# Tongji-MIC-Lab/TDVC

Measured on AMD Instinct MI355X. Metric: 1080p P-frames/sec (encode + reconstruct, lambda=2048 config), higher is better.
Workload: dtype f16; 1 GPU; 1x 1920x1080 (padded 1088x1920) 7-frame synthetic GOP (seed 1234), batch 1, P-frames coded in GOP order; gop=7, batch=1, parallelism=gop-sharded x1, weights=closed-form filler (no checkpoint ships)

## Files before the change

### include/tdvc_hip.h

```cpp
#ifndef TDVC_HIP_H
#define TDVC_HIP_H

#include <stdint.h>

#ifdef __cplusplus
extern "C" {
#endif

#define TDVC_OK 0
#define TDVC_EINVAL (-1)
#define TDVC_ENOSUP (-2)

typedef struct {
  void* p;
  int32_t N, H, W, C;
  int64_t sn;
  int32_t sp;
  int32_t dtype;
} tdvc_fmap;

enum { TDVC_F16 = 0, TDVC_F32 = 1 };
enum { TDVC_ACT_NONE = 0, TDVC_ACT_RELU = 1, TDVC_ACT_LRELU = 2, TDVC_ACT_CLAMP01 = 3, TDVC_ACT_SIGMOID = 4 };
enum { TDVC_GDN_NONE = 0, TDVC_GDN_FWD = 1, TDVC_GDN_INV = 2 };
enum { TDVC_OUT_NHWC = 0,
       TDVC_OUT_SHUFFLE2 = 1,
       TDVC_OUT_NCHW_F32 = 2 };

#define TDVC_MAX_TAPS 49

typedef struct {
  tdvc_fmap x;
  tdvc_fmap y;
  const void* w;
  const float* bias;
  int32_t cout;
  int32_t ntaps;
  int8_t tap_dy[TDVC_MAX_TAPS], tap_dx[TDVC_MAX_TAPS];
  int32_t kh, kw, stride, pad;
  int32_t ck;
  int32_t square_input;
  int32_t gdn;
  tdvc_fmap aux;
  int32_t act; float slope;
  int32_t round_before_act;
  tdvc_fmap res;
  tdvc_fmap res2;
  int32_t out_mode;
  int32_t s2d;
  int32_t bcast_T;
  float bcast_slope;
  float* chan_sum;
} tdvc_conv_desc;

int tdvc_abi_version(void);
const char* tdvc_last_error(void);
int tdvc_prepare_device(void);
const char* tdvc_last_conv_kernel(void);

int tdvc_set_predicate(const int* flag);
int tdvc_last_launch_predicated(void);
int tdvc_frame_changed(const tdvc_fmap* cur, tdvc_fmap* cache, int* flag, void* stream);


int tdvc_conv_plan(int cin, int kh, int kw, int stride);
int64_t tdvc_conv_packed_bytes(int cout, int cin, int ntaps, int ck);
int tdvc_pack_conv_weights(const float* w_oihw, int cout, int cin_real, int cin, int kh, int kw,
                           int ntaps, const int8_t* tap_dy, const int8_t* tap_dx, int ck, uint16_t* dst);
int tdvc_conv2d(const tdvc_conv_desc* d, void* stream);
int tdvc_conv_chan_sum_rows(const tdvc_conv_desc* d);
const char* tdvc_conv_select(const tdvc_conv_desc* d);
int tdvc_conv2d_f32(const tdvc_conv_desc* d, void* stream);

typedef struct {
  tdvc_fmap x, y;
  const void* w;
  const float* bias;
  int32_t act1; float slope1;
  int32_t act2; float slope2;
  int32_t add_input;
  tdvc_fmap res2;
} tdvc_conv_pair_desc;
int64_t tdvc_conv_pair_packed_bytes(void);
int tdvc_pack_conv_pair_weights(const float* w1_oihw, const float* w2_oihw, uint16_t* dst);
int tdvc_conv_pair_supported(const tdvc_conv_pair_desc* d);
int tdvc_conv_pair(const tdvc_conv_pair_desc* d, void* stream);

typedef struct {
  tdvc_fmap x, om, y;
  const void* w;
  const float* bias;
  int32_t groups;
  int32_t act; float slope; int32_t round_before_act;
  void* x_planar;
} tdvc_dcn_desc;
int tdvc_dcn_fused(const tdvc_dcn_desc* d, void* stream);

int tdvc_dcn_v2_forward_f32(const float* input, const float* weight, const float* bias,
                            const float* offset, const float* mask, float* output,
                            int B, int C, int H, int W, int Cout,
                            int kh, int kw, int sh, int sw, int ph, int pw, int dh, int dw,
                            int deformable_group, void* stream);
int tdvc_dcn_v2_backward_f32(const float* input, const float* weight, const float* bias,
                             const float* offset, const float* mask, const float* grad_output,
                             float* grad_input, float* grad_offset, float* grad_mask,
                             float* grad_weight, float* grad_bias, float* columns,
                             int B, int C, int H, int W, int Cout,
                             int kh, int kw, int sh, int sw, int ph, int pw, int dh, int dw,
                             int deformable_group, void* stream);

int tdvc_nchw_to_fmap(const float* src, int C, const tdvc_fmap* y, void* stream);
int tdvc_fmap_to_nchw(const tdvc_fmap* x, int C, float* dst, void* stream);
int tdvc_scale_act_res(const tdvc_fmap* a, const float* gate, int act, float slope,
                       const tdvc_fmap* r, float r_sign, const tdvc_fmap* y, const tdvc_fmap* y2, void* stream);
int tdvc_add_flow(const tdvc_fmap* off, const tdvc_fmap* flow, void* stream);
int tdvc_bcast_add_act(const tdvc_fmap* x, const tdvc_fmap* b, int T, float slope, void* stream);

int tdvc_channel_sum(const tdvc_fmap* x, float* partial, int nblocks, void* stream);
int tdvc_se_gate(const float* partial, int nblocks, float inv_count, int N, int C, int Cmid,
                 const float* w1, const float* b1, const float* w2, const float* b2,
                 float* gate, void* stream);

int tdvc_upsample2x(const tdvc_fmap* x, const tdvc_fmap* y, void* stream);
int tdvc_avgpool2(const tdvc_fmap* x, const tdvc_fmap* y, void* stream);
int tdvc_spynet_level_input(const tdvc_fmap* ref, const tdvc_fmap* supp, const tdvc_fmap* flow_lo,
                            const tdvc_fmap* flow_up, const tdvc_fmap* cat8, void* stream);
int tdvc_resize_bilinear(const tdvc_fmap* x, const tdvc_fmap* y, const float* chscale, void* stream);

int64_t tdvc_avgpool_k_work_floats(int N, int hp, int wp, int C, int scale);
int tdvc_avgpool_k(const tdvc_fmap* x, int scale, float* pooled, int hp, int wp, float* work, int64_t work_floats, void* stream);
int tdvc_patch_match(const float* pin, const float* pref, int N, int hp, int wp, int C,
                     int32_t* idx, void* stream);
int tdvc_match_gather(const tdvc_fmap* fin, const tdvc_fmap* fref, const int32_t* idx, int scale,
                      int hp, int wp, const tdvc_fmap* cat, void* stream);

int tdvc_eb_forward(const tdvc_fmap* z, const float* params, const tdvc_fmap* noise,
                    const tdvc_fmap* z_hat, double* bits_out, float* partial, int partial_cap, void* stream);
int tdvc_gc_forward(const tdvc_fmap* y, const tdvc_fmap* gp, const tdvc_fmap* noise,
                    double* bits_out, float* partial, int partial_cap, void* stream);
int tdvc_quantize(const tdvc_fmap* y, const tdvc_fmap* noise, const tdvc_fmap* y_hat, void* stream);

int64_t tdvc_rans_encode(const int32_t* symbols, const int32_t* indexes, int64_t n,
                         const int32_t* cdfs, int32_t cdf_stride, const int32_t* cdf_sizes,
                         const int32_t* offsets, uint8_t* out, int64_t cap);
int tdvc_rans_decode(const uint8_t* data, int64_t nbytes, const int32_t* indexes, int64_t n,
                     const int32_t* cdfs, int32_t cdf_stride, const int32_t* cdf_sizes,
                     const int32_t* offsets, int32_t* symbols_out);

void* tdvc_rans_decoder_create(const uint8_t* data, int64_t nbytes);
int tdvc_rans_decoder_decode(void* handle, const int32_t* indexes, int64_t n, const int32_t* cdfs,
                             int32_t cdf_stride, const int32_t* cdf_sizes, const int32_t* offsets,
                             int32_t* symbols_out);
void tdvc_rans_decoder_destroy(void* handle);

int64_t tdvc_rans_encode_lanes(const int32_t* symbols, const int32_t* indexes, int64_t npos, int M, int L,
                               const int32_t* cdfs, int32_t cdf_stride, const int32_t* cdf_sizes,
                               const int32_t* offsets, uint8_t* out, int64_t cap);
int tdvc_rans_decode_lanes(const uint8_t* data, int64_t nbytes, const int32_t* indexes, int64_t npos, int M,
                           const int32_t* cdfs, int32_t cdf_stride, const int32_t* cdf_sizes,
                           const int32_t* offsets, int32_t* symbols_out);

int tdvc_pmf_to_quantized_cdf(const float* pmf, int n, int precision, int32_t* cdf_out);

int tdvc_ar_gather(const tdvc_fmap* y_hat, const tdvc_fmap* params, const int32_t* pos, int npos,
                   const tdvc_fmap* x1, const tdvc_fmap* pc, void* stream);
int tdvc_ar_quantize(const tdvc_fmap* y, const tdvc_fmap* gp, const int32_t* pos, int npos,
                     const float* scale_table, int ntable, const int32_t* symbols_in,
                     const tdvc_fmap* y_hat, int32_t* symbols, int32_t* indexes, void* stream);
int tdvc_ar_indexes(const tdvc_fmap* gp, const int32_t* pos, int npos, const float* scale_table, int ntable,
                    int M, int W, int32_t* indexes, void* stream);
int tdvc_ar_decode_serial(const uint8_t* data, int64_t nbytes, const int32_t* cdfs, int32_t cdf_stride, const int32_t* cdf_sizes,
                          const int32_t* offsets, const tdvc_fmap* y_hat, const tdvc_fmap* params, const tdvc_fmap* x1,
                          const tdvc_fmap* pc, const tdvc_conv_desc* convs, int nconvs, const tdvc_fmap* gp,
                          const int32_t* pos_table, int npos_total, int M, int W, const float* scale_table, int ntable,
                          int32_t* idx_dev, int32_t* sym_dev, void* stream);
int tdvc_ar_wavefront(const uint8_t* data, int64_t nbytes, const int32_t* cdfs, int32_t cdf_stride, const int32_t* cdf_sizes,
                      const int32_t* offsets, const tdvc_fmap* y, const tdvc_fmap* y_hat, const tdvc_fmap* params,
                      const tdvc_fmap* x1, const tdvc_fmap* pc, const tdvc_conv_desc* convs, int nconvs, const tdvc_fmap* gp,
                      const int32_t* pos_dev, const int32_t* step_sizes, int nsteps, int M, int W,
                      const float* scale_table, int ntable, int32_t* idx_dev, int32_t* sym_dev, void* stream);
int64_t tdvc_ar_lanes_state_bytes(int L);
int tdvc_ar_lanes_init(const uint8_t* stream_dev, int64_t nbytes, int L, uint32_t* state_dev, void* stream);
int tdvc_ar_decode_lanes_step(const tdvc_fmap* gp, const int32_t* pos, int npos, const float* scale_table, int ntable,
                              const uint8_t* stream_dev, int64_t nbytes, int L, const uint16_t* cdf16_dev, int32_t n16,
                              const int32_t* cdf_starts_dev, const int32_t* cdf_sizes_dev, const int32_t* offsets_dev, int32_t ncdfs,
                              uint32_t* state_dev,
                              const tdvc_fmap* y_hat, int32_t* symbols, int32_t* indexes, int64_t cbase, void* stream);
int tdvc_ar_wavefront_lanes(const uint8_t* data, int64_t nbytes, uint8_t* stream_dev, int64_t stream_cap, uint32_t* state_dev,
                            const uint16_t* cdf16_dev, int32_t n16, const int32_t* cdf_starts_dev, const int32_t* cdf_sizes_dev,
                            const int32_t* offsets_dev, int32_t ncdfs, const tdvc_fmap* y_hat, const tdvc_fmap* params, const tdvc_fmap* x1,
                            const tdvc_fmap* pc, const tdvc_conv_desc* convs, int nconvs, const tdvc_fmap* gp,
                            const int32_t* pos_dev, const int32_t* step_sizes, int nsteps, int M, int W,
                            const float* scale_table, int ntable, int32_t* idx_dev, int32_t* sym_dev, void* stream);
int tdvc_round_symbols(const tdvc_fmap* z, const float* median, int32_t* out, void* stream);

int tdvc_pack_conv_weights_indexed(const float* w, const int32_t* row_off, const int32_t* chan_off, const int32_t* tap_off,
                                   const uint8_t* row_mask, const uint8_t* chan_mask, const uint8_t* tap_mask,
                                   int cout, int cin, int ntaps, int ck, void* dst, void* stream);
int tdvc_pack_conv_weights_indexed_f32(const float* w, const int32_t* row_off, const int32_t* chan_off, const int32_t* tap_off,
                                       const uint8_t* row_mask, const uint8_t* chan_mask, const uint8_t* tap_mask,
                                       int cout, int cin, int ntaps, int ck, float* dst, void* stream);
typedef struct tdvc_pack_job {
  const float* w;
  const int32_t *row_off, *chan_off, *tap_off;
  const uint8_t *row_mask, *chan_mask, *tap_mask;
  void* dst;
  const float* bias_src;
  float* bias_dst;
  const int32_t* bias_perm;
  int32_t cout, cin, ntaps, ck;
} tdvc_pack_job;
int64_t tdvc_pack_job_blocks(int cout, int cin, int ntaps, int ck);
int tdvc_pack_conv_weights_batch(const tdvc_pack_job* jobs, const int32_t* block_start, int njobs, int total_blocks, void* stream);
int64_t tdvc_conv_wgrad_work_floats(int cout, int cin, int ntaps, int N, int Ho, int Wo);
int tdvc_conv_wgrad(const tdvc_fmap* g, const tdvc_fmap* x, int cout, int kh, int kw, int stride, int pad,
// ... 84 lines not shown
```

### tdvc_amd/_lib.py

```python
from __future__ import annotations

import ctypes as C
import os

_HERE = os.path.dirname(os.path.abspath(__file__))
LIB_PATH = os.path.join(_HERE, "libtdvc_hip.so")

MAX_TAPS = 49
F16, F32 = 0, 1
ACT_NONE, ACT_RELU, ACT_LRELU, ACT_CLAMP01, ACT_SIGMOID = 0, 1, 2, 3, 4
GDN_NONE, GDN_FWD, GDN_INV = 0, 1, 2
OUT_NHWC, OUT_SHUFFLE2, OUT_NCHW_F32 = 0, 1, 2


class FMapDesc(C.Structure):
    _fields_ = [("p", C.c_void_p), ("N", C.c_int32), ("H", C.c_int32), ("W", C.c_int32), ("C", C.c_int32),
                ("sn", C.c_int64), ("sp", C.c_int32), ("dtype", C.c_int32)]


class ConvDesc(C.Structure):
    _fields_ = [("x", FMapDesc), ("y", FMapDesc), ("w", C.c_void_p), ("bias", C.c_void_p),
                ("cout", C.c_int32), ("ntaps", C.c_int32),
                ("tap_dy", C.c_int8 * MAX_TAPS), ("tap_dx", C.c_int8 * MAX_TAPS),
                ("kh", C.c_int32), ("kw", C.c_int32), ("stride", C.c_int32), ("pad", C.c_int32),
                ("ck", C.c_int32), ("square_input", C.c_int32), ("gdn", C.c_int32),
                ("aux", FMapDesc), ("act", C.c_int32), ("slope", C.c_float),
                ("round_before_act", C.c_int32), ("res", FMapDesc), ("res2", FMapDesc), ("out_mode", C.c_int32), ("s2d", C.c_int32),
                ("bcast_T", C.c_int32), ("bcast_slope", C.c_float), ("chan_sum", C.c_void_p)]


class DcnDesc(C.Structure):
    _fields_ = [("x", FMapDesc), ("om", FMapDesc), ("y", FMapDesc), ("w", C.c_void_p), ("bias", C.c_void_p),
                ("groups", C.c_int32), ("act", C.c_int32), ("slope", C.c_float), ("round_before_act", C.c_int32), ("x_planar", C.c_void_p)]


class ConvPairDesc(C.Structure):
    _fields_ = [("x", FMapDesc), ("y", FMapDesc), ("w", C.c_void_p), ("bias", C.c_void_p), ("act1", C.c_int32), ("slope1", C.c_float),
                ("act2", C.c_int32), ("slope2", C.c_float), ("add_input", C.c_int32), ("res2", FMapDesc)]


class WgradReduceJob(C.Structure):
    _fields_ = [("work", C.c_void_p), ("bwork", C.c_void_p), ("row_off", C.c_void_p), ("chan_off", C.c_void_p), ("tap_off", C.c_void_p),
                ("bias_index", C.c_void_p), ("dw", C.c_void_p), ("db", C.c_void_p), ("scale", C.c_float),
                ("nworkers", C.c_int32), ("cow", C.c_int32), ("ciw", C.c_int32), ("ntaps", C.c_int32), ("cout", C.c_int32), ("cin", C.c_int32),
                ("wblocks", C.c_int32), ("nblocks", C.c_int32)]


_P = C.c_void_p
_FM = C.POINTER(FMapDesc)
_i, _f, _i64 = C.c_int, C.c_float, C.c_int64

SIGNATURES = {
    "tdvc_abi_version": (_i, []),
    "tdvc_conv_chan_sum_rows": (_i, [C.POINTER(ConvDesc)]),
    "tdvc_conv_select": (C.c_char_p, [C.POINTER(ConvDesc)]),
    "tdvc_last_error": (C.c_char_p, []),
    "tdvc_last_conv_kernel": (C.c_char_p, []),
    "tdvc_prepare_device": (_i, []),
    "tdvc_set_predicate": (_i, [_P]),
    "tdvc_last_launch_predicated": (_i, []),
    "tdvc_frame_changed": (_i, [_FM, _FM, _P, _P]),
    "tdvc_conv_plan": (_i, [_i, _i, _i, _i]),
    "tdvc_conv_packed_bytes": (_i64, [_i, _i, _i, _i]),
    "tdvc_pack_conv_weights": (_i, [_P, _i, _i, _i, _i, _i, _i, _P, _P, _i, _P]),
    "tdvc_conv2d": (_i, [C.POINTER(ConvDesc), _P]),
    "tdvc_conv2d_f32": (_i, [C.POINTER(ConvDesc), _P]),
    "tdvc_pack_conv_weights_indexed": (_i, [_P] * 7 + [_i] * 4 + [_P, _P]),
    "tdvc_pack_conv_weights_indexed_f32": (_i, [_P] * 7 + [_i] * 4 + [_P, _P]),
    "tdvc_pack_job_blocks": (_i64, [_i, _i, _i, _i]),
    "tdvc_pack_conv_weights_batch": (_i, [_P, _P, _i, _i, _P]),
    "tdvc_act_backward": (_i, [_FM, _FM, _FM, _i, _f, _FM, _P]),
    "tdvc_pixel_unshuffle": (_i, [_FM, _FM, _P]),
    "tdvc_bias_grad_work_floats": (_i64, [_i, _i]),
    "tdvc_bias_grad": (_i, [_FM, _i, _P, _f, _P, _P, _i64, _P]),
    "tdvc_copy_cast": (_i, [_FM, _FM, _P]),
    "tdvc_clamp01_backward": (_i, [_FM, _FM, _P]),
    "tdvc_gate_backward_work_floats": (_i64, [_i, _i]),
    "tdvc_gate_backward": (_i, [_FM, _FM, _P, _FM, _P, _P, _i64, _P]),
    "tdvc_se_gate_backward": (_i, [_P, _i, _f, _i, _i, _i] + [_P] * 6 + [_f] + [_P] * 6),
    "tdvc_bcast_channel_add": (_i, [_FM, _P, _f, _P]),
    "tdvc_add_flow_backward": (_i, [_FM, _FM, _P]),
    "tdvc_bcast_add_act_backward": (_i, [_FM, _FM, _FM, _f, _P]),
    "tdvc_upsample2x_backward": (_i, [_FM, _FM, _P]),
    "tdvc_resize_bilinear_backward": (_i, [_FM, _FM, _P, _P]),
    "tdvc_spynet_level_input_backward": (_i, [_FM, _FM, _FM, _FM, _FM, _P]),
    "tdvc_sigmoid_f32": (_i, [_P, _P, _i64, _P]),
    "tdvc_sigmoid_backward_f32": (_i, [_P, _P, _i64, _P]),
    "tdvc_axpy_f32": (_i, [_P, _P, _f, _i64, _P]),
    "tdvc_match_gather_backward": (_i, [_FM, _FM, _P, _i, _i, _i, _FM, _FM, _FM, _P]),
    "tdvc_eb_backward": (_i, [_FM, _P, _FM, _f, _FM, _P, _P]),
    "tdvc_eb_pack": (_i, [_P, _P, _P, _i, _P]),
    "tdvc_eb_param_chain": (_i, [_P, _P, _P, _f, _i, _P]),
    "tdvc_eb_aux": (_i, [_P, _P, _f, _P, _P, _i, _P]),
    "tdvc_gc_backward": (_i, [_FM, _FM, _FM, _f, _FM, _FM, _P]),
    "tdvc_dcn_columns": (_i, [_FM, _FM, _i, _FM, _P]),
    "tdvc_ar_decode_serial": (_i, [_P, _i64, _P, _i, _P, _P, _FM, _FM, _FM, _FM, _P, _i, _FM, _P, _i, _i, _i, _P, _i, _P, _P, _P]),
    "tdvc_ar_wavefront": (_i, [_P, _i64, _P, _i, _P, _P, _FM, _FM, _FM, _FM, _FM, _P, _i, _FM, _P, _P, _i, _i, _i, _P, _i, _P, _P, _P]),
    "tdvc_ar_lanes_state_bytes": (_i64, [_i]),
    "tdvc_ar_lanes_init": (_i, [_P, _i64, _i, _P, _P]),
    "tdvc_ar_decode_lanes_step": (_i, [_FM, _P, _i, _P, _i, _P, _i64, _i, _P, C.c_int32, _P, _P, _P, C.c_int32, _P, _FM, _P, _P, _i64, _P]),
    "tdvc_ar_wavefront_lanes": (_i, [_P, _i64, _P, _i64, _P, _P, C.c_int32, _P, _P, _P, C.c_int32, _FM, _FM, _FM, _FM, _P, _i, _FM, _P, _P, _i, _i, _i,
                                     _P, _i, _P, _P, _P]),
    "tdvc_ssim_level_work_floats": (_i64, [_i] * 5),
    "tdvc_ssim_level": (_i, [_P, _P, _i, _i, _i, _i, _P, _i, _f, _f, _P, _P, _P, _i64, _P]),
    "tdvc_avgpool2_pad_f32": (_i, [_P, _i64, _i, _i, _P, _P]),
    "tdvc_ssim_level_backward": (_i, [_P, _P, _i, _i, _i, _i, _P, _i, _f, _f, _P, _P, _f, _P, _P, _P]),
    "tdvc_msssim_level_grads": (_i, [_P, _P, _P, _i, _i, _P, _P, _P, _P, _P]),
    "tdvc_dcn_col2im_work_floats": (_i64, [_i, _i, _i, _i]),
    "tdvc_dcn_col2im": (_i, [_FM, _FM, _FM, _i, _P, _FM, _P, _i64, _P]),
    "tdvc_dcn_col2im_det": (_i, [_FM, _FM, _FM, _i, _P, _FM, _P, _i64, _P, _P, _P, _i, _P]),
    "tdvc_dcn_far_apply": (_i, [_P, _P, _P, _i, _P, _P]),
    "tdvc_conv_wgrad_work_floats": (_i64, [_i] * 6),
    "tdvc_conv_wgrad": (_i, [_FM, _FM] + [_i] * 6 + [_P] * 5 + [_i, _f, _P, _P, _i64, _P]),
    "tdvc_conv_wgrad_bias": (_i, [_FM, _FM] + [_i] * 6 + [_P] * 5 + [_i, _f, _P, _P, _P, _P, _i64, _P]),
    "tdvc_conv_wgrad_partials": (_i, [_FM, _FM] + [_i] * 6 + [_P] * 5 + [_i, _f, _P, _P, _P, _P, _i64, C.POINTER(WgradReduceJob), _P]),
    "tdvc_wgrad_reduce_batch": (_i, [_P, _P, _i, _i, _P]),
    "tdvc_gdn_backward": (_i, [_FM, _FM, _FM, _i, _FM, _FM, _P]),
    "tdvc_mul2_accumulate": (_i, [_FM, _FM, _FM, _P]),
    "tdvc_dcn_fused": (_i, [C.POINTER(DcnDesc), _P]),
    "tdvc_conv_pair_packed_bytes": (_i64, []),
    "tdvc_pack_conv_pair_weights": (_i, [_P, _P, _P]),
    "tdvc_conv_pair_supported": (_i, [C.POINTER(ConvPairDesc)]),
    "tdvc_conv_pair": (_i, [C.POINTER(ConvPairDesc), _P]),
    "tdvc_dcn_v2_forward_f32": (_i, [_P] * 6 + [_i] * 14 + [_P]),
    "tdvc_dcn_v2_backward_f32": (_i, [_P] * 12 + [_i] * 14 + [_P]),
    "tdvc_nchw_to_fmap": (_i, [_P, _i, _FM, _P]),
    "tdvc_fmap_to_nchw": (_i, [_FM, _i, _P, _P]),
    "tdvc_scale_act_res": (_i, [_FM, _P, _i, _f, _FM, _f, _FM, _FM, _P]),
    "tdvc_add_flow": (_i, [_FM, _FM, _P]),
    "tdvc_bcast_add_act": (_i, [_FM, _FM, _i, _f, _P]),
    "tdvc_channel_sum": (_i, [_FM, _P, _i, _P]),
    "tdvc_se_gate": (_i, [_P, _i, _f, _i, _i, _i, _P, _P, _P, _P, _P, _P]),
    "tdvc_upsample2x": (_i, [_FM, _FM, _P]),
    "tdvc_avgpool2": (_i, [_FM, _FM, _P]),
    "tdvc_spynet_level_input": (_i, [_FM, _FM, _FM, _FM, _FM, _P]),
    "tdvc_resize_bilinear": (_i, [_FM, _FM, _P, _P]),
    "tdvc_avgpool_k_work_floats": (_i64, [_i, _i, _i, _i, _i]),
    "tdvc_avgpool_k": (_i, [_FM, _i, _P, _i, _i, _P, _i64, _P]),
    "tdvc_patch_match": (_i, [_P, _P, _i, _i, _i, _i, _P, _P]),
    "tdvc_match_gather": (_i, [_FM, _FM, _P, _i, _i, _i, _FM, _P]),
    "tdvc_eb_forward": (_i, [_FM, _P, _FM, _FM, _P, _P, _i, _P]),
    "tdvc_gc_forward": (_i, [_FM, _FM, _FM, _P, _P, _i, _P]),
    "tdvc_quantize": (_i, [_FM, _FM, _FM, _P]),
    "tdvc_rans_encode": (_i64, [_P, _P, _i64, _P, C.c_int32, _P, _P, _P, _i64]),
    "tdvc_rans_decode": (_i, [_P, _i64, _P, _i64, _P, C.c_int32, _P, _P, _P]),
    "tdvc_rans_encode_lanes": (_i64, [_P, _P, _i64, _i, _i, _P, C.c_int32, _P, _P, _P, _i64]),
    "tdvc_rans_decode_lanes": (_i, [_P, _i64, _P, _i64, _i, _P, C.c_int32, _P, _P, _P]),
    "tdvc_rans_decoder_create": (_P, [_P, _i64]),
    "tdvc_rans_decoder_decode": (_i, [_P, _P, _i64, _P, C.c_int32, _P, _P, _P]),
    "tdvc_rans_decoder_destroy": (None, [_P]),
    "tdvc_pmf_to_quantized_cdf": (_i, [_P, _i, _i, _P]),
    "tdvc_ar_gather": (_i, [_FM, _FM, _P, _i, _FM, _FM, _P]),
    "tdvc_ar_quantize": (_i, [_FM, _FM, _P, _i, _P, _i, _P, _FM, _P, _P, _P]),
    "tdvc_ar_indexes": (_i, [_FM, _P, _i, _P, _i, _i, _i, _P, _P]),
    "tdvc_round_symbols": (_i, [_FM, _P, _P, _P]),
}

_lib = None


class TdvcHipError(RuntimeError):
    pass


def lib():
    global _lib
    if _lib is None:
        if not os.path.exists(LIB_PATH):
            raise TdvcHipError(
                f"{LIB_PATH} is missing: build it with `python -c 'import __graft_entry__ as g; g.build()'` "
                "(hipcc --offload-arch=gfx950).  tdvc_amd has no CPU fallback.")
        l = C.CDLL(LIB_PATH)
        for name, (res, args) in SIGNATURES.items():
            fn = getattr(l, name)
            fn.restype = res
            fn.argtypes = args
        _lib = l
    return _lib


def check(rc: int, what: str = ""):
    if rc != 0:
        msg = lib().tdvc_last_error().decode("utf-8", "replace")
        raise TdvcHipError(f"{what}: rc={rc}: {msg}")
```

### tdvc_amd/csrc/common.h

```cpp
#pragma once
#include <hip/hip_runtime.h>
#include <stdint.h>
#include <stdio.h>
#include <string.h>

#include "../../include/tdvc_hip.h"

typedef _Float16 half_t;
typedef _Float16 half8 __attribute__((ext_vector_type(8)));
typedef _Float16 half4 __attribute__((ext_vector_type(4)));
typedef _Float16 half2v __attribute__((ext_vector_type(2)));
typedef float f32x16 __attribute__((ext_vector_type(16)));
typedef float f32x4 __attribute__((ext_vector_type(4)));

void tdvc_set_error(const char* fmt, ...);
int tdvc_scratch_pages(const void** zeros, void** dump);

const int* tdvc_launch_predicate();
void tdvc_note_launch();
#define TDVC_PREDICATE_RETURN(pred)                       \
  do {                                                    \
    if ((pred) != nullptr && *(pred) == 0) return;        \
  } while (0)

#define TDVC_CHECK(cond, ...)            \
  do {                                   \
    if (!(cond)) {                       \
      tdvc_set_error(__VA_ARGS__);       \
      return TDVC_EINVAL;                \
    }                                    \
  } while (0)

static inline int tdvc_launch_status(const char* what) {
  tdvc_note_launch();
  hipError_t e = hipGetLastError();
  if (e != hipSuccess) {
    tdvc_set_error("%s: launch failed: %s", what, hipGetErrorString(e));
    return (int)e;
  }
  return TDVC_OK;
}

static inline bool aligned16(const void* p) { return (((uintptr_t)p) & 15) == 0; }
struct TdvcPerDeviceFlag {
  bool done[64] = {};
  bool& flag() {
    int dev = 0;
    if (hipGetDevice(&dev) != hipSuccess || dev < 0 || dev >= 64) dev = 0;
    return done[dev];
  }
};

struct FMap {
  void* p;
  int N, H, W, C;
  long sn;
  int sp;
  int f32;
};
static inline FMap to_dev(const tdvc_fmap& f) {
  FMap m;
  m.p = f.p; m.N = f.N; m.H = f.H; m.W = f.W; m.C = f.C; m.sn = f.sn; m.sp = f.sp;
  m.f32 = (f.dtype == TDVC_F32);
  return m;
}
static inline FMap null_fmap() {
  FMap m; memset(&m, 0, sizeof(m)); return m;
}

static inline bool fmap_ok16(const tdvc_fmap& f) {
  return f.p && f.dtype == TDVC_F16 && (f.C % 8) == 0 && (f.sp % 8) == 0 && (f.sn % 8) == 0 && aligned16(f.p) &&
         f.sp >= f.C && f.N > 0 && f.H > 0 && f.W > 0;
}
static inline bool fmap_ok32(const tdvc_fmap& f) {
  return f.p && f.dtype == TDVC_F32 && f.sp >= f.C && f.N > 0 && f.H > 0 && f.W > 0 && (((uintptr_t)f.p) & 3) == 0;
}

__device__ __forceinline__ int tdvc_xcd_tile(int b) {
  const int gx = (int)gridDim.x;
  const bool planar = gridDim.y * gridDim.z == 1;
  if ((gx & 7) != 0 && !planar) return b;
  const int q = gx >> 3, r = gx & 7, c = b & 7;
  return c * q + min(c, r) + (b >> 3);
}

__device__ __forceinline__ float act_apply(float v, int act, float slope) {
  switch (act) {
    case TDVC_ACT_RELU: return v > 0.f ? v : 0.f;
    case TDVC_ACT_LRELU: return v > 0.f ? v : v * slope;
    case TDVC_ACT_CLAMP01: return fminf(fmaxf(v, 0.f), 1.f);
    case TDVC_ACT_SIGMOID: return 1.f / (1.f + __expf(-v));
    default: return v;
  }
}
```

### tdvc_amd/csrc/conv_c8.hip

```cpp
#include "conv_common.h"

using convk::ConvParams;

namespace {

constexpr int NW_C8 = 4, NTHR_C8 = 256;
constexpr int EW_C8 = 32 * 144;
constexpr int LDS_C8 = 256 + NW_C8 * EW_C8;

__global__ __launch_bounds__(NTHR_C8, 4) void conv_c8_kernel(const ConvParams p, int tiles_x, int total_tiles) {
  TDVC_PREDICATE_RETURN(p.pred);
  extern __shared__ __attribute__((aligned(16))) unsigned char smem[];
  float* bias_s = reinterpret_cast<float*>(smem);
  const int tid = threadIdx.x, lane = tid & 63;
  const int wave = __builtin_amdgcn_readfirstlane(tid >> 6);
  const int hh = lane >> 5, r = lane & 31;
  if (tid < 64) bias_s[tid] = p.bias[tid];
  unsigned char* ew = smem + 256 + wave * EW_C8;

  half8 wa[2][5];
#pragma unroll
  for (int mt = 0; mt < 2; ++mt)
#pragma unroll
    for (int s = 0; s < 5; ++s) wa[mt][s] = *reinterpret_cast<const half8*>(p.w + (((long)mt * 5 + s) * 64 + lane) * 8);

  int tdy[5], tdx[5];
#pragma unroll
  for (int s = 0; s < 5; ++s) {
    const int t = min(2 * s + hh, 8);
    tdy[s] = t / 3 - 1;
    tdx[s] = t % 3 - 1;
  }
  __syncthreads();

  const int nwaves = (int)gridDim.x * NW_C8;
  const int w0 = (int)blockIdx.x * NW_C8 + wave;
  const int per_img = tiles_x * p.Ho;
  const half8 zero8 = {0, 0, 0, 0, 0, 0, 0, 0};

  auto load_b = [&](int tile, half8 (&b)[5]) {
    const int n = tile / per_img, rem = tile - n * per_img;
    const int oy = rem / tiles_x, ox0 = (rem - oy * tiles_x) * 32;
    const half_t* xn = p.x + (long)n * p.x_sn;
#pragma unroll
    for (int s = 0; s < 5; ++s) {
      const int iy = oy + tdy[s], ix = ox0 + r + tdx[s];
      const bool ok = iy >= 0 && iy < p.H && ix >= 0 && ix < p.W;
      const half_t* src = xn + ((long)(ok ? iy : 0) * p.W + (ok ? ix : 0)) * p.x_sp;
      const half8 v = *reinterpret_cast<const half8*>(src);
      b[s] = ok ? v : zero8;
    }
  };

  half8 bcur[5], bnext[5];
  int tile = w0;
  if (tile < total_tiles) load_b(tile, bnext);
  for (; tile < total_tiles; tile += nwaves) {
#pragma unroll
    for (int s = 0; s < 5; ++s) bcur[s] = bnext[s];
    if (tile + nwaves < total_tiles) load_b(tile + nwaves, bnext);
    f32x16 acc[2][1];
#pragma unroll
    for (int mt = 0; mt < 2; ++mt)
#pragma unroll
      for (int i = 0; i < 16; ++i) acc[mt][0][i] = 0.f;
#pragma unroll
    for (int s = 0; s < 5; ++s)
#pragma unroll
      for (int mt = 0; mt < 2; ++mt) acc[mt][0] = __builtin_amdgcn_mfma_f32_32x32x16_f16(wa[mt][s], bcur[s], acc[mt][0], 0, 0, 0);
    const int n = tile / per_img, rem = tile - n * per_img;
    const int oy = rem / tiles_x, ox0 = (rem - oy * tiles_x) * 32;
    {
      constexpr int EPS = 144;
      const int chunk = lane & 7, prow = lane >> 3;
      const bool ch_ok = chunk * 8 < p.y.C;
      const half_t sl = (half_t)p.slope;
      const half2v sl2 = {sl, sl};
#pragma unroll
      for (int mt = 0; mt < 2; ++mt)
#pragma unroll
        for (int g = 0; g < 4; ++g) {
          const f32x4 b4 = *reinterpret_cast<const f32x4*>(bias_s + mt * 32 + 8 * g + 4 * hh);
          half2v lo = {(half_t)(acc[mt][0][4 * g + 0] + b4[0]), (half_t)(acc[mt][0][4 * g + 1] + b4[1])};
          half2v hi = {(half_t)(acc[mt][0][4 * g + 2] + b4[2]), (half_t)(acc[mt][0][4 * g + 3] + b4[3])};
          lo = __builtin_elementwise_max(lo, lo * sl2);
          hi = __builtin_elementwise_max(hi, hi * sl2);
          const half4 o = {lo[0], lo[1], hi[0], hi[1]};
          *reinterpret_cast<half4*>(ew + r * EPS + (mt * 32 + 8 * g + 4 * hh) * 2) = o;
        }
      half_t* yb = reinterpret_cast<half_t*>(p.y.p) + (long)n * p.y.sn + ((long)oy * p.Wo + ox0) * p.y.sp + chunk * 8;
#pragma unroll
      for (int k = 0; k < 4; ++k) {
        const int px = k * 8 + prow;
        const half8 v = *reinterpret_cast<const half8*>(ew + px * EPS + chunk * 16);
        if (ch_ok && ox0 + px < p.Wo) *reinterpret_cast<half8*>(yb + (long)px * p.y.sp) = v;
      }
    }
  }
}

}

bool conv_c8_eligible(const tdvc_conv_desc* d, const ConvParams& p, int Ho, int Wo) {
  return convk::taps_dense(d, 3, 3, 1) && d->ck == 8 && d->stride == 1 && d->cout == 64 && d->x.C == 8 && !d->s2d && !d->square_input &&
         (long)Ho * Wo >= convk::LARGE_MAP_PIXELS &&
         convk::conv_is_lean(p) && !p.res.p && !p.res2.p && p.y.C >= 64 && (long)d->x.N * Ho * ((Wo + 31) / 32) < (1L << 30);
}

int launch_conv_c8(const ConvParams& p, int N, hipStream_t st) {
  ConvParams q = p;
  q.slope = convk::conv_simple_slope(p);
  q.pred = tdvc_launch_predicate();
  const int tiles_x = (p.Wo + 31) / 32;
  const long total = (long)N * p.Ho * tiles_x;
  int grid = (int)((total + NW_C8 - 1) / NW_C8);
  if (grid > 256 * 4) grid = 256 * 4;
  hipLaunchKernelGGL(conv_c8_kernel, dim3(grid), dim3(NTHR_C8), LDS_C8, st, q, tiles_x, (int)total);
  return tdvc_launch_status("tdvc_conv2d(c8)");
}
```

### tdvc_amd/csrc/conv_common.h

```cpp
#pragma once
#include "common.h"

namespace convk {

struct ConvParams {
  const half_t* x; long x_sn; int x_sp; int H, W, Cin;
  const half_t* w; const float* bias;
  FMap y; int Ho, Wo; int cout;
  FMap aux; FMap res; FMap res2;
  int ntaps, kh, kw, pad;
  int in_stride;
  int nchunks, steps;
  int square, gdn, act; float slope; int round16, out_mode;
  int tiles_x;
  int simple;
  int s2d, Corig;
  int reverse;
  int bcast_T; float bcast_slope;
  float* csum;
  int8_t tap_dy[TDVC_MAX_TAPS], tap_dx[TDVC_MAX_TAPS];
  const int* pred;
};

enum ConvSwitch { SW_NONE = -1, SW_V2, SW_V3, SW_V5, SW_V7, SW_V9, SW_V10, SW_V11, SW_ROW, SW_C8, SW_N16, SW_GDN128, SW_COUNT };
// ... 137 lines not shown
  if (p.gdn ? p.act != TDVC_ACT_NONE : !(p.act == TDVC_ACT_NONE || p.act == TDVC_ACT_RELU || p.act == TDVC_ACT_LRELU)) return false;
  if (p.act == TDVC_ACT_LRELU && !(p.slope >= 0.f && p.slope <= 1.f)) return false;
  if (p.res.p && (p.res.f32 || p.res.C < p.y.C)) return false;
  if (p.res2.p && p.res2.C < p.y.C) return false;
  if (shuf && (((p.cout >> 2) % 64) != 0 || p.gdn)) return false;
  if (p.gdn && (p.aux.C < p.y.C || shuf)) return false;
  return true;
}
inline float conv_simple_slope(const ConvParams& p) {
  return p.act == TDVC_ACT_NONE ? 1.f : (p.act == TDVC_ACT_RELU ? 0.f : p.slope);
}

struct PackedRow { half4 v[8]; };

template <int NTX, bool BIAS_IN_ACC = false>
__device__ __forceinline__ void epilogue_pack(const ConvParams& p, f32x16 (&acc)[2][NTX], const float* bias64, int lane,
                                              PackedRow (&out)[NTX], bool zero_acc) {
  const int hh = lane >> 5;
#pragma unroll
  for (int nt = 0; nt < NTX; ++nt)
#pragma unroll
    for (int mt = 0; mt < 2; ++mt)
#pragma unroll
      for (int g = 0; g < 4; ++g) {
        const int cl = mt * 32 + 8 * g + 4 * hh;
        f32x4 b4 = {0.f, 0.f, 0.f, 0.f};
        if constexpr (!BIAS_IN_ACC) b4 = *reinterpret_cast<const f32x4*>(bias64 + cl);
        half4 o;
#pragma unroll
        for (int i = 0; i < 4; ++i) {
          float v = acc[mt][nt][4 * g + i];
          if constexpr (!BIAS_IN_ACC) {
            v += b4[i];
            if (zero_acc) acc[mt][nt][4 * g + i] = 0.f;
          }
          v = __builtin_fmaxf(v, v * p.slope);
          o[i] = (half_t)v;
        }
        out[nt].v[mt * 4 + g] = o;
      }
}

__device__ __forceinline__ void epilogue_store_row(const ConvParams& p, const PackedRow& row, unsigned char* ew, int n, int cbase,
                                                   int oy, int ox_first, int lane, bool full = false) {
  constexpr int EPS = 144;
  const int hh = lane >> 5, r = lane & 31;
  const int chunk = lane & 7, prow = lane >> 3;
  const int co = cbase + chunk * 8;
  const bool has1 = p.res.p != nullptr, has2 = p.res2.p != nullptr, gdn = p.gdn != 0;
  int pc = co, sub_y = 0, sub_x = 0, mul = 1, PW = p.Wo;
  if (p.out_mode == TDVC_OUT_SHUFFLE2) {
    const int cq = p.cout >> 2;
    const int sub = co / cq;
    pc = co - sub * cq;
    sub_y = sub >> 1; sub_x = sub & 1; mul = 2; PW = 2 * p.Wo;
  }
  const bool ch_ok = pc < p.y.C && co < ((p.cout + 63) & ~63);
  const bool row_ok = oy < p.Ho && ch_ok;
#pragma unroll
  for (int mt = 0; mt < 2; ++mt)
#pragma unroll
    for (int g = 0; g < 4; ++g)
      *reinterpret_cast<half4*>(ew + r * EPS + (mt * 32 + 8 * g + 4 * hh) * 2) = row.v[mt * 4 + g];
  const int pcc = ch_ok ? pc : 0;
  constexpr int KB = 4;
#pragma unroll
  for (int k0 = 0; k0 < 4; k0 += KB) {
    half8 r0[KB], r1[KB], r2[KB];
    int opix[KB], apix[KB];
    bool ok[KB];
#pragma unroll
    for (int k = 0; k < KB; ++k) {
      const int ox = ox_first + (k0 + k) * 8 + prow;
      ok[k] = full ? ch_ok : (row_ok && ox < p.Wo);
      opix[k] = ok[k] ? (mul * oy + sub_y) * PW + (mul * ox + sub_x) : 0;
      apix[k] = ok[k] ? oy * p.Wo + ox : 0;
    }
    if (gdn) {
      const half_t* ab = reinterpret_cast<const half_t*>(p.aux.p) + (long)n * p.aux.sn + (ch_ok ? co : 0);
#pragma unroll
      for (int k = 0; k < KB; ++k) r0[k] = *reinterpret_cast<const half8*>(ab + (long)apix[k] * p.aux.sp);
    }
    if (has1) {
      const half_t* rb = reinterpret_cast<const half_t*>(p.res.p) + (long)n * p.res.sn + pcc;
#pragma unroll
      for (int k = 0; k < KB; ++k) r1[k] = *reinterpret_cast<const half8*>(rb + (long)opix[k] * p.res.sp);
    }
    if (has2) {
      const half_t* rb = reinterpret_cast<const half_t*>(p.res2.p) + (long)n * p.res2.sn + pcc;
#pragma unroll
      for (int k = 0; k < KB; ++k) r2[k] = *reinterpret_cast<const half8*>(rb + (long)opix[k] * p.res2.sp);
    }
#pragma unroll
    for (int k = 0; k < KB; ++k) {
      half8 h = *reinterpret_cast<const half8*>(ew + ((k0 + k) * 8 + prow) * EPS + chunk * 16);
      if (gdn) {
        float v[8];
#pragma unroll
        for (int j = 0; j < 8; ++j) v[j] = (float)r0[k][j] * (p.gdn == TDVC_GDN_FWD ? rsqrtf((float)h[j]) : sqrtf((float)h[j]));
        if (has1) {
#pragma unroll
          for (int j = 0; j < 8; ++j) v[j] += (float)r1[k][j];
        }
        if (has2) {
#pragma unroll
          for (int j = 0; j < 8; ++j) v[j] += (float)r2[k][j];
        }
#pragma unroll
        for (int j = 0; j < 8; ++j) h[j] = (half_t)v[j];
      } else {
        if (has1) h = h + r1[k];
        if (has2) h = h + r2[k];
      }
      if (ok[k]) *reinterpret_cast<half8*>(reinterpret_cast<half_t*>(p.y.p) + (long)n * p.y.sn + (long)opix[k] * p.y.sp + pc) = h;
    }
  }
}

template <int NTX, bool BIAS_IN_ACC, bool BCAST = false, bool CSUM = false>
__device__ __forceinline__ void epilogue_lean_seq(const ConvParams& p, f32x16 (&acc)[2][NTX], const float* bias64, unsigned char* ew, int n,
                                                  int cbase, int oy_first, int ox_first, int lane, bool zero_acc, bool full, float* cs = nullptr) {
  constexpr int EPS = 144;
  const int hh = lane >> 5, r = lane & 31;
  const int chunk = lane & 7, prow = lane >> 3;
  const int co = cbase + chunk * 8;
  const bool ch_ok = co < p.y.C && co < ((p.cout + 63) & ~63);
  const int cc = ch_ok ? co : 0;
  const bool has1 = p.res.p != nullptr, has2 = p.res2.p != nullptr;
  const half_t sl = (half_t)p.slope;
  const half2v sl2 = {sl, sl}, zero2 = {(half_t)0.f, (half_t)0.f};
  const bool act = p.slope != 1.f, relu = p.slope == 0.f;
  half_t* yb = reinterpret_cast<half_t*>(p.y.p) + (long)n * p.y.sn + cc;
  const half_t* rb1 = reinterpret_cast<const half_t*>(p.res.p) + (long)n * p.res.sn + cc;
  const half_t* rb2 = reinterpret_cast<const half_t*>(p.res2.p) + (long)n * p.res2.sn + cc;
  f32x4 b4[2][4];
  if constexpr (!BIAS_IN_ACC) {
#pragma unroll
    for (int mt = 0; mt < 2; ++mt)
#pragma unroll
      for (int g = 0; g < 4; ++g) b4[mt][g] = *reinterpret_cast<const f32x4*>(bias64 + mt * 32 + 8 * g + 4 * hh);
  }
#pragma unroll
  for (int nt = 0; nt < NTX; ++nt) {
    const int oy = oy_first + nt;
    int opix[4];
    bool ok[4];
#pragma unroll
    for (int k = 0; k < 4; ++k) {
      const int ox = ox_first + k * 8 + prow;
      ok[k] = full ? ch_ok : (ch_ok && oy < p.Ho && ox < p.Wo);
      opix[k] = ok[k] ? oy * p.Wo + ox : 0;
    }
    half8 r1[4], r2[4];
    if (has1) {
#pragma unroll
      for (int k = 0; k < 4; ++k) r1[k] = *reinterpret_cast<const half8*>(rb1 + (long)opix[k] * p.res.sp);
    }
    if (has2) {
#pragma unroll
      for (int k = 0; k < 4; ++k) r2[k] = *reinterpret_cast<const half8*>(rb2 + (long)opix[k] * p.res2.sp);
    }
#pragma unroll
    for (int mt = 0; mt < 2; ++mt)
#pragma unroll
      for (int g = 0; g < 4; ++g) {
        float v[4];
#pragma unroll
        for (int i = 0; i < 4; ++i) {
          v[i] = acc[mt][nt][4 * g + i];
          if constexpr (!BIAS_IN_ACC) {
            v[i] += b4[mt][g][i];
            if (zero_acc) acc[mt][nt][4 * g + i] = 0.f;
          }
        }
        half2v lo = {(half_t)v[0], (half_t)v[1]}, hi = {(half_t)v[2], (half_t)v[3]};
        if (relu) {
          lo = __builtin_elementwise_max(lo, zero2);
          hi = __builtin_elementwise_max(hi, zero2);
        } else if (act) {
          lo = __builtin_elementwise_max(lo, lo * sl2);
          hi = __builtin_elementwise_max(hi, hi * sl2);
        }
        const half4 o = {lo[0], lo[1], hi[0], hi[1]};
        *reinterpret_cast<half4*>(ew + r * EPS + (mt * 32 + 8 * g + 4 * hh) * 2) = o;
      }
    if constexpr (BCAST) {
#pragma unroll
      for (int k = 0; k < 4; ++k) {
        const half8 v = *reinterpret_cast<const half8*>(ew + (k * 8 + prow) * EPS + chunk * 16);
        half_t* yp = yb + (long)opix[k] * p.y.sp;
        half8 xs[4];
#pragma unroll
        for (int t = 0; t < 4; ++t) xs[t] = *reinterpret_cast<const half8*>(yp + t * 64);
#pragma unroll
        for (int t = 0; t < 4; ++t) {
          half8 o;
#pragma unroll
          for (int j = 0; j < 8; ++j) {
            const float s = (float)xs[t][j] + (float)v[j];
            o[j] = (half_t)(s > 0.f ? s : s * p.bcast_slope);
          }
          if (ok[k]) *reinterpret_cast<half8*>(yp + t * 64) = o;
        }
      }
      continue;
    }
#pragma unroll
    for (int k = 0; k < 4; ++k) {
      half8 v = *reinterpret_cast<const half8*>(ew + (k * 8 + prow) * EPS + chunk * 16);
      if (has1) v = v + r1[k];
      if (has2) v = v + r2[k];
      if (ok[k]) *reinterpret_cast<half8*>(yb + (long)opix[k] * p.y.sp) = v;
      if constexpr (CSUM) {
#pragma unroll
        for (int j = 0; j < 8; ++j) cs[j] += ok[k] ? (float)v[j] : 0.f;
      }
    }
  }
}

template <int NTX, bool BIAS_IN_ACC = false, int MODE = 3>
__device__ __forceinline__ void epilogue_simple_rows(const ConvParams& p, f32x16 (&acc)[2][NTX], const float* bias64,
                                                     unsigned char* ew, int n, int cbase, int oy_first, int ox_first,
                                                     int lane, bool zero_acc, bool full = false) {
  if constexpr (MODE == 2) {
    epilogue_lean_seq<NTX, BIAS_IN_ACC>(p, acc, bias64, ew, n, cbase, oy_first, ox_first, lane, zero_acc, full);
    return;
  }
  if constexpr (MODE == 3) {
    if (p.simple == 2) {
      epilogue_lean_seq<NTX, BIAS_IN_ACC>(p, acc, bias64, ew, n, cbase, oy_first, ox_first, lane, zero_acc, full);
      return;
    }
  }
  PackedRow rows[NTX];
  epilogue_pack<NTX, BIAS_IN_ACC>(p, acc, bias64, lane, rows, zero_acc);
#pragma unroll
  for (int nt = 0; nt < NTX; ++nt) epilogue_store_row(p, rows[nt], ew, n, cbase, oy_first + nt, ox_first, lane, full);
}

inline bool conv_is_lean(const ConvParams& p) {
  return conv_is_simple(p) && p.out_mode == TDVC_OUT_NHWC && !p.gdn;
}

template <int NRES, int NR, bool STAMPED = false>
__device__ __forceinline__ void epilogue_lean_rows(const ConvParams& p, const f32x16 (&acc)[2][NR], unsigned char* ew, int n,
                                                   int cbase, int oy, int ox_first, int lane, bool full, long long* st = nullptr) {
#define EST(i) do { if constexpr (STAMPED) { if (st) st[i] = clock64(); } } while (0)
  static_assert(NR % 2 == 0, "two rows per round");
  constexpr int EPS = 144, EROW = 32 * EPS;
  const int hh = lane >> 5, r = lane & 31;
  const int chunk = lane & 7, prow = lane >> 3;
  const int co = cbase + chunk * 8;
  const bool ch_ok = co < p.y.C && co < ((p.cout + 63) & ~63);
  const int cc = ch_ok ? co : 0;
  int opix[NR][4];
  bool ok[NR][4];
#pragma unroll
  for (int j = 0; j < NR; ++j)
#pragma unroll
    for (int k = 0; k < 4; ++k) {
      const int ox = ox_first + k * 8 + prow;
      ok[j][k] = full ? ch_ok : (ch_ok && oy + j < p.Ho && ox < p.Wo);
      opix[j][k] = ok[j][k] ? (oy + j) * p.Wo + ox : 0;
    }
  half8 r1[NR][4], r2[NR][4];
  if constexpr (NRES >= 1) {
    const half_t* rb = reinterpret_cast<const half_t*>(p.res.p) + (long)n * p.res.sn + cc;
#pragma unroll
    for (int j = 0; j < NR; ++j)
#pragma unroll
      for (int k = 0; k < 4; ++k) r1[j][k] = *reinterpret_cast<const half8*>(rb + (long)opix[j][k] * p.res.sp);
  }
  if constexpr (NRES >= 2) {
    const half_t* rb = reinterpret_cast<const half_t*>(p.res2.p) + (long)n * p.res2.sn + cc;
#pragma unroll
    for (int j = 0; j < NR; ++j)
#pragma unroll
      for (int k = 0; k < 4; ++k) r2[j][k] = *reinterpret_cast<const half8*>(rb + (long)opix[j][k] * p.res2.sp);
  }
  const half_t sl = (half_t)p.slope;
  const half2v sl2 = {sl, sl};
  const bool act = p.slope != 1.f;
  half_t* yb = reinterpret_cast<half_t*>(p.y.p) + (long)n * p.y.sn + cc;
  EST(0);
#pragma unroll
  for (int j0 = 0; j0 < NR; j0 += 2) {
#pragma unroll
    for (int j = j0; j < j0 + 2; ++j)
#pragma unroll
      for (int mt = 0; mt < 2; ++mt)
#pragma unroll
        for (int g = 0; g < 4; ++g) {
          half2v lo = {(half_t)acc[mt][j][4 * g + 0], (half_t)acc[mt][j][4 * g + 1]};
          half2v hi = {(half_t)acc[mt][j][4 * g + 2], (half_t)acc[mt][j][4 * g + 3]};
          if (act) {
            lo = __builtin_elementwise_max(lo, lo * sl2);
            hi = __builtin_elementwise_max(hi, hi * sl2);
          }
          half4 o = {lo[0], lo[1], hi[0], hi[1]};
          *reinterpret_cast<half4*>(ew + (j & 1) * EROW + r * EPS + (mt * 32 + 8 * g + 4 * hh) * 2) = o;
        }
    EST(1 + 3 * (j0 / 2));
    half8 h[2][4];
#pragma unroll
    for (int j = 0; j < 2; ++j)
#pragma unroll
      for (int k = 0; k < 4; ++k) h[j][k] = *reinterpret_cast<const half8*>(ew + j * EROW + (k * 8 + prow) * EPS + chunk * 16);
    EST(2 + 3 * (j0 / 2));
#pragma unroll
    for (int j = 0; j < 2; ++j)
#pragma unroll
      for (int k = 0; k < 4; ++k) {
        half8 v = h[j][k];
        if constexpr (NRES >= 1) v = v + r1[j0 + j][k];
        if constexpr (NRES >= 2) v = v + r2[j0 + j][k];
        if (ok[j0 + j][k]) *reinterpret_cast<half8*>(yb + (long)opix[j0 + j][k] * p.y.sp) = v;
      }
    EST(3 + 3 * (j0 / 2));
  }
#undef EST
}

}
```

### tdvc_amd/csrc/conv_dispatch.hip

```cpp
#include <stdlib.h>

#include "conv_common.h"

using convk::ConvParams;
bool conv_v2_eligible(const tdvc_conv_desc* d, int Ho, int Wo); int launch_conv_v2(const ConvParams& p, int cout_blocks, int N, hipStream_t st);
bool conv_v3_eligible(const tdvc_conv_desc* d, int Ho, int Wo); int launch_conv_v3(const ConvParams& p, int cout_blocks, int N, hipStream_t st);
bool conv_v5_eligible(const tdvc_conv_desc* d, int Ho, int Wo); int launch_conv_v5(const ConvParams& p, int cout_blocks, int N, hipStream_t st); int conv_v5_chan_sum_rows(int Ho, int Wo, int cout_blocks, int N);
bool conv_v7_eligible(const tdvc_conv_desc* d, const ConvParams& p, int Ho, int Wo); int launch_conv_v7(const ConvParams& p, int cout_blocks, int N, hipStream_t st);
bool conv_v9_eligible(const tdvc_conv_desc* d, int Ho, int Wo, bool v3_ok); int launch_conv_v9(const ConvParams& p, int ck8, int cout_tiles32, int N, hipStream_t st);
bool conv_v10_eligible(const tdvc_conv_desc* d, const ConvParams& p, int Ho, int Wo); int launch_conv_v10(const ConvParams& p, int cout_blocks, int N, hipStream_t st);
bool conv_v11_eligible(const tdvc_conv_desc* d, const ConvParams& p, int Ho, int Wo); int launch_conv_v11(const ConvParams& p, int cout_blocks, int N, hipStream_t st);
int conv_row_geometry(const tdvc_conv_desc* d, const ConvParams& p, int Ho, int Wo); int launch_conv_row(int geo, const ConvParams& p, int N, hipStream_t st);
bool conv_c8_eligible(const tdvc_conv_desc* d, const ConvParams& p, int Ho, int Wo); int launch_conv_c8(const ConvParams& p, int N, hipStream_t st);
bool conv_n16_eligible(const tdvc_conv_desc* d, int Ho, int Wo); int launch_conv_n16(const ConvParams& p, int N, hipStream_t st);
bool gdn128_eligible(const tdvc_conv_desc* d, const ConvParams& p, int Ho, int Wo); int launch_gdn128(const ConvParams& p, int N, hipStream_t st);
int conv_direct_lds_bytes(const tdvc_conv_desc* d);
int conv_cout_tiles(int cout);
int launch_conv_direct(const ConvParams& p, int ck8, int stride, int N, hipStream_t st);
int conv_f32_validate(const tdvc_conv_desc* d, int& Ho, int& Wo);

namespace {
const char* const kSwitchEnv[convk::SW_COUNT] = {nullptr, "TDVC_CONV_NO_V3", "TDVC_CONV_NO_V5", "TDVC_CONV_NO_V7", "TDVC_CONV_NO_V9", "TDVC_CONV_NO_V10",
                                                 "TDVC_CONV_NO_V11", "TDVC_CONV_NO_ROW", "TDVC_CONV_NO_C8", "TDVC_CONV_NO_N16", "TDVC_CONV_NO_GDN128"};
int g_enabled[convk::SW_COUNT] = {1, 1, 1, 1, 1, 1, 1, 15, 1, 1, 1};
long g_v9_work_limit = 1L << 20;
}

int convk::conv_on(int id) {
  static const struct EnvOff {
    bool off[convk::SW_COUNT];
    EnvOff() {
      const bool v1 = getenv("TDVC_CONV_V1") != nullptr;
      for (int i = 0; i < convk::SW_COUNT; ++i) off[i] = v1 || (kSwitchEnv[i] && getenv(kSwitchEnv[i]) != nullptr);
    }
  } env;
  return id == convk::SW_NONE ? 1 : (env.off[id] ? 0 : g_enabled[id]);
}
long convk::conv_v9_work_limit() { return g_v9_work_limit; }

extern "C" void tdvc_debug_enable_conv_v9(int enable) { g_enabled[convk::SW_V9] = enable != 0; }
extern "C" void tdvc_debug_enable_conv_v10(int enable) { g_enabled[convk::SW_V10] = enable != 0; }
extern "C" void tdvc_debug_enable_conv_v11(int enable) { g_enabled[convk::SW_V11] = enable != 0; }
extern "C" void tdvc_debug_enable_conv_row(int mask) { g_enabled[convk::SW_ROW] = mask; }
extern "C" void tdvc_debug_enable_conv_c8(int enable) { g_enabled[convk::SW_C8] = enable != 0; }
extern "C" void tdvc_debug_enable_conv_n16(int enable) { g_enabled[convk::SW_N16] = enable != 0; }
extern "C" void tdvc_debug_enable_gdn128(int enable) { g_enabled[convk::SW_GDN128] = enable != 0; }
extern "C" void tdvc_debug_set_conv_v9_work_limit(long v) { g_v9_work_limit = v; }

namespace {

struct Pick {
  const tdvc_conv_desc* d;
  int Ho, Wo;
  int geo;
  int ck8() const { return d->ck / 8; }
  int N() const { return d->x.N; }
  int cout_blocks() const { return conv_cout_tiles(d->cout) / 2; }
};

struct Entry {
  const char* name;
  int sw;
  bool (*eligible)(Pick& k, const ConvParams& p);
  int (*launch)(const Pick& k, const ConvParams& p, hipStream_t st);
  bool (*only)(const tdvc_conv_desc* d);
  const char* only_msg;
};

bool v3_on_and_eligible(const Pick& k) { return convk::conv_on(convk::SW_V3) && conv_v3_eligible(k.d, k.Ho, k.Wo); }

bool bcast_eligible(Pick& k, const ConvParams& p) {
  const tdvc_conv_desc* d = k.d;
  return d->bcast_T == 4 && d->kh == 1 && d->kw == 1 && d->stride == 1 && d->pad == 0 && d->cout == 64 && d->y.C == 64 && d->y.sp >= 4 * 64 &&
         d->y.dtype == TDVC_F16 && d->out_mode == TDVC_OUT_NHWC && d->act == TDVC_ACT_NONE && !d->gdn && !d->res.p && !d->res2.p &&
         !d->square_input && !d->round_before_act && d->bias && d->bcast_slope >= 0.f && d->bcast_slope <= 1.f && conv_v5_eligible(d, k.Ho, k.Wo) &&
         convk::conv_is_lean(p);
}
int bcast_launch(const Pick& k, const ConvParams& p, hipStream_t st) {
  ConvParams q = p;
  q.simple = 2;
  q.slope = 1.f;
  return launch_conv_v5(q, 1, k.N(), st);
}
bool row_eligible(Pick& k, const ConvParams& p) { return (k.geo = conv_row_geometry(k.d, p, k.Ho, k.Wo)) >= 0; }

constexpr char kNameV5[] = "conv_mfma_v5", kNameDirect[] = "conv_mfma<%d,%d,%d>";

const Entry kTable[] = {
    {"conv_mfma_v5(bcast)", convk::SW_V5, bcast_eligible, bcast_launch, [](const tdvc_conv_desc* d) { return d->bcast_T != 0; },
     "tdvc_conv2d: bcast_T needs a plain 1x1 / stride 1 conv to 64 channels of >= 8192 pixels, y a 64-channel window of a buffer with >= 4 slices, bcast_T == 4"},
    {"conv_row(s2d)", convk::SW_ROW, [](Pick& k, const ConvParams& p) { return k.d->s2d && row_eligible(k, p); },
     [](const Pick& k, const ConvParams& p, hipStream_t st) { return launch_conv_row(k.geo, p, k.N(), st); }, nullptr, nullptr},
    {"conv_mfma_v3(s2d)", convk::SW_V3, [](Pick& k, const ConvParams&) { return k.d->s2d && conv_v3_eligible(k.d, k.Ho, k.Wo); },
     [](const Pick& k, const ConvParams& p, hipStream_t st) { return launch_conv_v3(p, k.cout_blocks(), k.N(), st); },
     [](const tdvc_conv_desc* d) { return d->s2d != 0; }, "tdvc_conv2d: s2d conv not eligible for the stage-pipelined kernel"},
    {"conv_mfma_v9", convk::SW_V9, [](Pick& k, const ConvParams&) { return conv_v9_eligible(k.d, k.Ho, k.Wo, v3_on_and_eligible(k)); },
     [](const Pick& k, const ConvParams& p, hipStream_t st) { return launch_conv_v9(p, k.ck8(), conv_cout_tiles(k.d->cout), k.N(), st); }, nullptr, nullptr},
    {"gdn128", convk::SW_GDN128, [](Pick& k, const ConvParams& p) { return gdn128_eligible(k.d, p, k.Ho, k.Wo); },
     [](const Pick& k, const ConvParams& p, hipStream_t st) { return launch_gdn128(p, k.N(), st); }, nullptr, nullptr},
    {kNameV5, convk::SW_V5, [](Pick& k, const ConvParams&) { return conv_v5_eligible(k.d, k.Ho, k.Wo); },
     [](const Pick& k, const ConvParams& p, hipStream_t st) { return launch_conv_v5(p, k.cout_blocks(), k.N(), st); }, nullptr, nullptr},
    {"conv_c8", convk::SW_C8, [](Pick& k, const ConvParams& p) { return conv_c8_eligible(k.d, p, k.Ho, k.Wo); },
     [](const Pick& k, const ConvParams& p, hipStream_t st) { return launch_conv_c8(p, k.N(), st); }, nullptr, nullptr},
    {"conv_n16", convk::SW_N16, [](Pick& k, const ConvParams&) { return conv_n16_eligible(k.d, k.Ho, k.Wo); },
     [](const Pick& k, const ConvParams& p, hipStream_t st) { return launch_conv_n16(p, k.N(), st); }, nullptr, nullptr},
    {"conv_row", convk::SW_ROW, row_eligible,
     [](const Pick& k, const ConvParams& p, hipStream_t st) { return launch_conv_row(k.geo, p, k.N(), st); }, nullptr, nullptr},
    {"conv_mfma_v10", convk::SW_V10, [](Pick& k, const ConvParams& p) { return conv_v10_eligible(k.d, p, k.Ho, k.Wo); },
     [](const Pick& k, const ConvParams& p, hipStream_t st) { return launch_conv_v10(p, k.cout_blocks(), k.N(), st); }, nullptr, nullptr},
    {"conv_mfma_v7", convk::SW_V7, [](Pick& k, const ConvParams& p) { return conv_v7_eligible(k.d, p, k.Ho, k.Wo); },
     [](const Pick& k, const ConvParams& p, hipStream_t st) { return launch_conv_v7(p, k.cout_blocks(), k.N(), st); }, nullptr, nullptr},
    {"conv_mfma_v11", convk::SW_V11, [](Pick& k, const ConvParams& p) { return conv_v11_eligible(k.d, p, k.Ho, k.Wo); },
     [](const Pick& k, const ConvParams& p, hipStream_t st) { return launch_conv_v11(p, k.cout_blocks(), k.N(), st); }, nullptr, nullptr},
    {"conv_mfma_v3", convk::SW_V3, [](Pick& k, const ConvParams&) { return conv_v3_eligible(k.d, k.Ho, k.Wo); },
     [](const Pick& k, const ConvParams& p, hipStream_t st) { return launch_conv_v3(p, k.cout_blocks(), k.N(), st); }, nullptr, nullptr},
    {"conv_mfma_v2", convk::SW_V2, [](Pick& k, const ConvParams&) { return conv_v2_eligible(k.d, k.Ho, k.Wo); },
     [](const Pick& k, const ConvParams& p, hipStream_t st) { return launch_conv_v2(p, k.cout_blocks(), k.N(), st); }, nullptr, nullptr},
    {kNameDirect, convk::SW_NONE, [](Pick& k, const ConvParams&) { return conv_direct_lds_bytes(k.d) <= 64 * 1024; },
     [](const Pick& k, const ConvParams& p, hipStream_t st) { return launch_conv_direct(p, k.ck8(), k.d->stride, k.N(), st); },
     [](const tdvc_conv_desc*) { return true; }, nullptr},
};

const Entry* select(Pick& k, const ConvParams& p) {
  for (const Entry& e : kTable) {
    if (convk::conv_on(e.sw) && e.eligible(k, p)) return &e;
    if (e.only && e.only(k.d)) {
      if (e.only_msg) tdvc_set_error("%s", e.only_msg);
      else tdvc_set_error("tdvc_conv2d: LDS plan %d bytes too large for the direct kernel (use tdvc_conv_plan)", conv_direct_lds_bytes(k.d));
      return nullptr;
    }
  }
  return nullptr;
}

void kernel_name(const Entry* e, const Pick& k, char (&out)[48]) {
  if (e->name == kNameDirect) snprintf(out, sizeof(out), kNameDirect, k.ck8(), conv_cout_tiles(k.d->cout) == 1 ? 1 : 2, k.d->stride);
  else snprintf(out, sizeof(out), "%s", e->name);
}

int prepare(const tdvc_conv_desc* d, ConvParams& p, int& Ho, int& Wo) {
  TDVC_CHECK(fmap_ok16(d->x), "tdvc_conv2d: input must be an fp16 fmap with C,sp %% 8 == 0 and 16-byte aligned");
  TDVC_CHECK(d->w && aligned16(d->w), "tdvc_conv2d: weights null/unaligned");
  TDVC_CHECK(d->stride == 1 || d->stride == 2, "tdvc_conv2d: stride %d unsupported", d->stride);
  TDVC_CHECK(d->ntaps >= 1 && d->ntaps <= TDVC_MAX_TAPS && d->kh >= 1 && d->kh <= 7 && d->kw >= 1 && d->kw <= 7,
             "tdvc_conv2d: bad kernel %dx%d ntaps=%d", d->kh, d->kw, d->ntaps);
  TDVC_CHECK(d->ck == 8 || d->ck == 16 || d->ck == 32 || d->ck == 64, "tdvc_conv2d: bad ck %d", d->ck);
  TDVC_CHECK(d->cout >= 1, "tdvc_conv2d: cout");
  for (int t = 0; t < d->ntaps; ++t)
    TDVC_CHECK(d->tap_dy[t] >= 0 && d->tap_dy[t] < d->kh && d->tap_dx[t] >= 0 && d->tap_dx[t] < d->kw,
               "tdvc_conv2d: tap %d out of the %dx%d window", t, d->kh, d->kw);
  Ho = (d->x.H + 2 * d->pad - d->kh) / d->stride + 1;
  Wo = (d->x.W + 2 * d->pad - d->kw) / d->stride + 1;
  if (d->s2d) {
    TDVC_CHECK(d->kh == 2 && d->kw == 2 && d->stride == 1 && d->pad == 1 && d->ntaps == 4 && d->ck == 32 && !d->square_input && !d->gdn,
               "tdvc_conv2d: s2d expects the virtual 2x2 / stride 1 / pad 1 conv packed with ck=32");
    TDVC_CHECK((d->x.H % 2) == 0 && (d->x.W % 2) == 0 && (d->x.C % 32) == 0 && d->cout >= 64,
               "tdvc_conv2d: s2d needs even H, W, C %% 32 == 0 and cout >= 64 (got %dx%dx%d, cout %d)", d->x.H, d->x.W, d->x.C, d->cout);
    Ho = d->x.H / 2;
    Wo = d->x.W / 2;
  }
  TDVC_CHECK(Ho > 0 && Wo > 0, "tdvc_conv2d: empty output");
  TDVC_CHECK((long)Ho * Wo * 4 < 2147483647L && (long)d->x.H * d->x.W < 2147483647L, "tdvc_conv2d: image too large (pixel indices are 32-bit)");

  const int shuf = d->out_mode == TDVC_OUT_SHUFFLE2;
  if (d->out_mode == TDVC_OUT_NCHW_F32) {
    TDVC_CHECK(d->y.p && d->y.N == d->x.N, "tdvc_conv2d: NCHW output null / batch mismatch");
  } else {
    TDVC_CHECK(d->y.dtype == TDVC_F32 ? fmap_ok32(d->y) : fmap_ok16(d->y), "tdvc_conv2d: bad output fmap");
    TDVC_CHECK(d->y.N == d->x.N && d->y.H == (shuf ? 2 * Ho : Ho) && d->y.W == (shuf ? 2 * Wo : Wo),
               "tdvc_conv2d: output geometry %dx%d does not match conv result %dx%d%s", d->y.H, d->y.W, Ho, Wo,
               shuf ? " (x2 shuffle)" : "");
    if (shuf) TDVC_CHECK((d->cout % 128) == 0, "tdvc_conv2d: SHUFFLE2 needs cout %% 128 == 0");
    if (d->y.dtype == TDVC_F16) TDVC_CHECK((d->y.C % 8) == 0, "tdvc_conv2d: fp16 output C %% 8");
  }
  if (d->gdn) {
    TDVC_CHECK(fmap_ok16(d->aux) && d->aux.H == Ho && d->aux.W == Wo && d->aux.N == d->x.N && d->aux.C >= d->cout &&
                   !shuf && (d->cout % 64) == 0,
               "tdvc_conv2d: GDN aux fmap mismatch");
  }
  if (d->res.p) {
    TDVC_CHECK(d->res.dtype == TDVC_F32 ? fmap_ok32(d->res) : fmap_ok16(d->res), "tdvc_conv2d: bad residual fmap");
    TDVC_CHECK(d->res.N == d->x.N && d->res.H == (shuf ? 2 * Ho : Ho) && d->res.W == (shuf ? 2 * Wo : Wo),
               "tdvc_conv2d: residual geometry mismatch");
  }
  if (d->res2.p) {
    TDVC_CHECK(fmap_ok16(d->res2) && d->res2.N == d->x.N && d->res2.H == (shuf ? 2 * Ho : Ho) && d->res2.W == (shuf ? 2 * Wo : Wo),
               "tdvc_conv2d: bad second residual fmap");
  }
  if (d->bias) TDVC_CHECK(aligned16(d->bias), "tdvc_conv2d: bias unaligned");

  memset(&p, 0, sizeof(p));
  p.x = reinterpret_cast<const half_t*>(d->x.p); p.x_sn = d->x.sn; p.x_sp = d->x.sp;
  p.H = d->x.H; p.W = d->x.W; p.Cin = d->x.C;
  p.w = reinterpret_cast<const half_t*>(d->w); p.bias = d->bias;
  p.y = to_dev(d->y); p.Ho = Ho; p.Wo = Wo; p.cout = d->cout;
  p.aux = d->gdn ? to_dev(d->aux) : null_fmap();
  p.res = d->res.p ? to_dev(d->res) : null_fmap();
  p.res2 = d->res2.p ? to_dev(d->res2) : null_fmap();
  p.ntaps = d->ntaps; p.kh = d->kh; p.kw = d->kw; p.pad = d->pad;
  p.in_stride = d->stride;
  p.s2d = d->s2d; p.Corig = d->x.C;
  p.bcast_T = d->bcast_T; p.bcast_slope = d->bcast_slope;
  p.nchunks = d->s2d ? (4 * d->x.C) / d->ck : (d->x.C + d->ck - 1) / d->ck;
  p.steps = (d->ntaps * (d->ck / 8) + 1) / 2;
  p.square = d->square_input; p.gdn = d->gdn; p.act = d->act; p.slope = d->slope;
  p.round16 = d->round_before_act; p.out_mode = d->out_mode;
  memcpy(p.tap_dy, d->tap_dy, sizeof(p.tap_dy));
  memcpy(p.tap_dx, d->tap_dx, sizeof(p.tap_dx));
  p.tiles_x = (Wo + 31) / 32;
  if (conv_cout_tiles(d->cout) > 1 && convk::conv_is_simple(p)) {
    p.simple = convk::conv_is_lean(p) ? 2 : 1;
    p.slope = convk::conv_simple_slope(p);
  }
  return TDVC_OK;
}

thread_local char g_last_kernel[48] = "";

thread_local unsigned g_walk_parity = 0;
int g_walk_mode = -1;
int next_walk_reverse() {
  if (g_walk_mode < 0) { const char* e = getenv("TDVC_CONV_WALK"); g_walk_mode = e ? atoi(e) : 1; }
  return g_walk_mode == 1 ? (int)(g_walk_parity++ & 1u) : 0;
}

int conv2d_impl(const tdvc_conv_desc* d, void* stream, bool query_rows) {
  TDVC_CHECK(d, "tdvc_conv2d: null descriptor");
  if (d->x.dtype == TDVC_F32) {
    if (query_rows) return 0;
    TDVC_CHECK(!d->chan_sum, "tdvc_conv2d: chan_sum is not available on the fp32 path (tdvc_conv_chan_sum_rows() == 0)");
    snprintf(g_last_kernel, sizeof(g_last_kernel), "conv_f32");
    return tdvc_conv2d_f32(d, stream);
  }
  ConvParams p;
  Pick k = {d, 0, 0, -1};
  if (const int rc = prepare(d, p, k.Ho, k.Wo)) return rc;
  p.reverse = query_rows ? 0 : next_walk_reverse();
  const Entry* e = select(k, p);
  const bool csum_ok = e && e->name == kNameV5 && k.cout_blocks() == 1 && p.simple == 2;
  if (query_rows) return csum_ok ? conv_v5_chan_sum_rows(k.Ho, k.Wo, 1, k.N()) : 0;
  TDVC_CHECK(!d->chan_sum || (csum_ok && (reinterpret_cast<uintptr_t>(d->chan_sum) & 15) == 0),
             "tdvc_conv2d: chan_sum on a conv whose kernel has no fused channel sum (tdvc_conv_chan_sum_rows() == 0) or unaligned");
  p.csum = d->chan_sum;
// ... 28 lines not shown
```

### tdvc_amd/csrc/conv_pair.hip

```cpp
#include <type_traits>

#include "conv_common.h"

namespace {

constexpr int BI = 2;
constexpr int TRING = 2 * BI;
constexpr int SRING = 2 * BI;
constexpr int T_LAG = 1 + BI;
constexpr int ID_LAG = 2 + BI;
template <int NCB> struct PairGeoBase;
template <> struct PairGeoBase<2> { static constexpr int PIECES = 5, XRING = 16, PF = 8, HD = 4; };
template <> struct PairGeoBase<4> { static constexpr int PIECES = 9, XRING = 10, PF = 4, HD = 2; };
template <int NCB> struct PairGeo : PairGeoBase<NCB> {
  using G = PairGeoBase<NCB>;
  static constexpr int PW = 16 * NCB - 2;
  static constexpr int NPX = PW + 4;
  static constexpr int ROWB = G::PIECES * 1024;
  static constexpr int TROWB = ROWB;
  static constexpr int SROW = 16 * NCB * 128;
  static constexpr int X0 = 0, T0 = G::XRING * ROWB, S0 = T0 + TRING * TROWB;
  static constexpr int LDS = S0 + SRING * SROW;
  static_assert(NPX * 128 <= ROWB, "ring row holds the strip's input pixels");
  static_assert(G::PF - G::XRING < -(BI - 1) - ID_LAG, "input ring: a DMA would land on a row whose identity a conv2 wave BI - 1 steps behind has not read (needs PF + 2 BI + 2 <= XRING)");
  static_assert(G::PF >= G::HD + BI, "landing: row r must be past land_wait()'s history window before the last barrier in front of step r");
  static_assert((NCB == 2 && G::HD == 4) || (NCB == 4 && G::HD == 2), "land_wait(): constant counts for these two histories");
  static_assert(ID_LAG >= 1 && ID_LAG <= G::XRING - G::PF - BI, "identity row inside the input ring");
  static_assert(LDS <= 160 * 1024, "rings inside 160 KB of LDS");
};
static_assert(T_LAG == 1 + BI && TRING >= 2 * BI && (TRING & (TRING - 1)) == 0, "t ring: BI rows being written + BI rows being read");
static_assert(SRING >= 2 * BI && (SRING & (SRING - 1)) == 0, "staging ring: BI rows being written + BI rows being stored");
static_assert((BI & (BI - 1)) == 0, "power-of-two barrier interval");
constexpr int NTHR = 512;
#ifndef PAIR_DMA_MID
#define PAIR_DMA_MID 1
#endif
#ifndef PAIR_FBN
#define PAIR_FBN 2
#endif
#ifndef PAIR_MID_G
#define PAIR_MID_G 1
#endif

struct PairParams {
  const half_t* x; long x_sn; int x_sp;
  half_t* y; long y_sn; int y_sp;
  const half_t* res2; long r2_sn; int r2_sp;
  const half_t* w;
  const float* bias;
  const half_t* zeros;
  half_t* dump;
  int N, H, W;
  int strips, segs, seg_rows, jobs;
  float slope1, slope2;
  int experiment;
  const int* pred;
};

__device__ __forceinline__ int swz(int q) { return (int)((0x62654210u >> (4 * ((q >> 1) & 7))) & 7u); }

__device__ __forceinline__ void glds16(const half_t* gsrc, unsigned lds_dst) {
  unsigned keep;
  asm volatile("s_mov_b32 %0, m0\n\ts_mov_b32 m0, %2\n\ts_nop 0\n\tglobal_load_lds_dwordx4 %1, off\n\ts_mov_b32 m0, %0"
               : "=&s"(keep) : "v"(gsrc), "s"(lds_dst) : "memory");
}
__device__ __forceinline__ void pair_barrier(bool skip = false) {
  asm volatile("s_waitcnt lgkmcnt(0)" ::: "memory");
  if (!skip) __builtin_amdgcn_s_barrier();
  asm volatile("" ::: "memory");
}
template <int A>
__device__ __forceinline__ half4 actk(half4 v, half4 sl) {
  if constexpr (A == 1) {
    const half4 z = {(half_t)0.f, (half_t)0.f, (half_t)0.f, (half_t)0.f};
    return __builtin_elementwise_max(v, z);
  } else if constexpr (A == 2) {
    return __builtin_elementwise_max(v, v * sl);
  } else {
    return v;
  }
}

template <int XRING> __device__ __forceinline__ int pair_slot(int kk) {
  if constexpr ((XRING & (XRING - 1)) == 0) return kk & (XRING - 1);
  else return __builtin_amdgcn_readfirstlane(kk) % XRING;
}

template <int NCB, int A1, int A2, bool ADDX, bool RES2, bool STAMP = false>
__global__ __launch_bounds__(NTHR, 1) void conv_pair_kernel(const PairParams p, long long* stamps = nullptr, int stamp_cap = 0) {
  TDVC_PREDICATE_RETURN(p.pred);
  using G = PairGeo<NCB>;
  constexpr int PW = G::PW, ROWB = G::ROWB, TROWB = G::TROWB, SROW = G::SROW, XRING = G::XRING, PF = G::PF, X0 = G::X0, T0 = G::T0, S0 = G::S0;
  constexpr int NF = 6 * NCB;
  constexpr int NIT = NCB / 2;
  long long st_busy = 0, st_vm = 0, st_bar = 0, st_n = 0;
  extern __shared__ __attribute__((aligned(1024))) unsigned char smem[];
  const unsigned lds0 = static_cast<unsigned>(reinterpret_cast<uintptr_t>(smem));
  const int tid = threadIdx.x, lane = tid & 63;
  const int wave = __builtin_amdgcn_readfirstlane(tid >> 6);
  const int grp = wave >> 2, wq = wave & 3;
  const int r16 = lane & 15, kb = lane >> 4;

  half8 wf[18];
#pragma unroll
  for (int f = 0; f < 18; ++f) wf[f] = *reinterpret_cast<const half8*>(p.w + ((((long)(grp * 4 + wq) * 18 + f) * 64 + lane) * 8));
  const f32x4 bias4 = *reinterpret_cast<const f32x4*>(p.bias + 64 * grp + 16 * wq + 4 * kb);

  int foff[3][2];
#pragma unroll
  for (int dx = 0; dx < 3; ++dx) {
    const int q = dx + r16, sw = swz(q);
#pragma unroll
    for (int kc = 0; kc < 2; ++kc) foff[dx][kc] = q * 128 + (((4 * kc + kb) ^ sw) << 4);
  }
  const int cdc = 2 * wq + (kb >> 1);
  const int doff = r16 * 128 + ((cdc ^ swz(r16)) << 4) + 8 * (kb & 1);
  const int roff = (r16 + 2) * 128 + ((cdc ^ swz(r16 + 2)) << 4) + 8 * (kb & 1);
  constexpr int PLAST = G::PIECES - 1;
  int soff_own, soff_hi = 0, soff_last;
  {
    const int q = 8 * wq + (lane >> 3), c = (lane & 7) ^ swz(q);
    soff_own = q * p.x_sp + c * 8;
    if constexpr (NCB == 4) {
      const int qh = 32 + q, ch = (lane & 7) ^ swz(qh);
      soff_hi = qh * p.x_sp + ch * 8;
    }
    const int ql = 8 * PLAST + (lane >> 3), cl = (lane & 7) ^ swz(ql);
    soff_last = ql * p.x_sp + cl * 8;
  }
  const int s_t = tid & 255;
  const int s_yi = s_t >> 3, s_c = (s_t & 7) ^ swz(s_yi);

  const int nwg = (int)gridDim.x, b = (int)blockIdx.x;
  int jfirst, jstep, jend;
  if ((nwg & 7) == 0) {
    const int per = (p.jobs + 7) >> 3;
    jfirst = (b & 7) * per + (b >> 3);
    jstep = nwg >> 3;
    jend = min(p.jobs, ((b & 7) + 1) * per);
  } else {
    jfirst = b; jstep = nwg; jend = p.jobs;
  }

  const half_t hs1 = (half_t)p.slope1, hs2 = (half_t)p.slope2;
  const half4 sl1 = {hs1, hs1, hs1, hs1}, sl2 = {hs2, hs2, hs2, hs2};
  auto run = [&](auto ROLEc) __attribute__((always_inline)) {
  constexpr int ROLE = decltype(ROLEc)::value;
  f32x4 acc[3][NCB];
  half8 fb[NF];
  half8 r2v[NIT] = {};

  for (int job = jfirst; job < jend; job += jstep) {
    const int n = job / (p.strips * p.segs);
    const int rem = job - n * (p.strips * p.segs);
    const int seg = rem / p.strips, strip = rem - seg * p.strips;
    const int c0 = strip * PW, ra = seg * p.seg_rows, rb = min(p.H, ra + p.seg_rows);
    const int rows = rb - ra;
    const half_t* xn = p.x + (long)n * p.x_sn;
    half_t* yn = p.y + (long)n * p.y_sn;

    bool col_own, col_hi = false, col_last;
    {
      const int q = 8 * wq + (lane >> 3), ql = 8 * PLAST + (lane >> 3);
      col_own = c0 - 2 + q >= 0 && c0 - 2 + q < p.W;
      if constexpr (NCB == 4) col_hi = c0 - 2 + 32 + q < p.W;
      col_last = ql < G::NPX && c0 - 2 + ql < p.W;
    }
    unsigned tmask[NCB];
#pragma unroll
    for (int cb = 0; cb < NCB; ++cb) {
      const int col = c0 - 1 + 16 * cb + r16;
      tmask[cb] = (col >= 0 && col < p.W) ? 0xFFFFFFFFu : 0u;
    }
    bool s_ok[NIT];
#pragma unroll
    for (int u = 0; u < NIT; ++u) s_ok[u] = s_yi + 32 * u < PW && c0 + s_yi + 32 * u < p.W && !(p.experiment & 2);
#pragma unroll
    for (int s3 = 0; s3 < 3; ++s3)
#pragma unroll
      for (int cb = 0; cb < NCB; ++cb) acc[s3][cb] = f32x4{0.f, 0.f, 0.f, 0.f};

    auto issue_row = [&](int kk) __attribute__((always_inline)) -> int {
      const int row = ra - 2 + kk;
      const bool rowok = row >= 0 && row < p.H;
      const half_t* base = xn + ((long)row * p.W + (c0 - 2)) * p.x_sp;
      const unsigned dst = lds0 + X0 + pair_slot<XRING>(kk) * ROWB;
      glds16((rowok && col_own) ? base + soff_own : p.zeros, dst + wq * 1024);
      if constexpr (NCB == 4) {
        glds16((rowok && col_hi) ? base + soff_hi : p.zeros, dst + (wq + 4) * 1024);
        if (wq == 0) glds16((rowok && col_last) ? base + soff_last : p.zeros, dst + PLAST * 1024);
      } else {
        if (wq == (kk & 3)) glds16((rowok && col_last) ? base + soff_last : p.zeros, dst + PLAST * 1024);
      }
      return 1;
    };
    auto load_frags = [&](unsigned rowbase) __attribute__((always_inline)) {
#pragma unroll
      for (int dx = 0; dx < 3; ++dx)
#pragma unroll
        for (int kc = 0; kc < 2; ++kc) {
          const unsigned char* b0 = smem + (rowbase + foff[dx][kc]);
#pragma unroll
          for (int cb = 0; cb < NCB; ++cb) fb[(cb * 3 + dx) * 2 + kc] = *reinterpret_cast<const half8*>(b0 + cb * 2048);
        }
    };
    auto row_mfmas = [&](unsigned rowbase, auto SNc, auto SMc, auto SDc, auto fin, auto mid) __attribute__((always_inline)) {
      constexpr int SN = decltype(SNc)::value, SM = decltype(SMc)::value, SD = decltype(SDc)::value;
      if constexpr (NCB == 4) {
        half8 fg[PAIR_FBN][NCB];
        auto loadg = [&](int g, half8 (&dst)[NCB]) __attribute__((always_inline)) {
          const unsigned char* b0 = smem + (rowbase + foff[g >> 1][g & 1]);
#pragma unroll
          for (int cb = 0; cb < NCB; ++cb) dst[cb] = *reinterpret_cast<const half8*>(b0 + cb * 2048);
        };
#pragma unroll
        for (int g = 0; g < PAIR_FBN - 1; ++g) loadg(g, fg[g]);
#pragma unroll
        for (int g = 0; g < 6; ++g) {
          const int dx = g >> 1, kc = g & 1;
          if (g + PAIR_FBN - 1 < 6) loadg(g + PAIR_FBN - 1, fg[(g + PAIR_FBN - 1) % PAIR_FBN]);
#pragma unroll
          for (int dyo = 0; dyo < 3; ++dyo) {
            const int dy = 2 - dyo;
            const int slot = dy == 2 ? SD : (dy == 1 ? SM : SN);
            const bool first = dy == 0 && g == 0;
#pragma unroll
            for (int cb = 0; cb < NCB; ++cb)
              acc[slot][cb] = __builtin_amdgcn_mfma_f32_16x16x32_f16(wf[(dy * 3 + dx) * 2 + kc], fg[g % PAIR_FBN][cb], first ? bias4 : acc[slot][cb], 0, 0, 0);
          }
          if (g == PAIR_MID_G) mid();
        }
        fin();
      } else {
        load_frags(rowbase);
#pragma unroll
        for (int dyo = 0; dyo < 3; ++dyo) {
          const int dy = 2 - dyo;
#pragma unroll
          for (int dx = 0; dx < 3; ++dx)
#pragma unroll
            for (int kc = 0; kc < 2; ++kc)
#pragma unroll
              for (int cb = 0; cb < NCB; ++cb) {
                const int slot = dy == 2 ? SD : (dy == 1 ? SM : SN);
                const bool first = dy == 0 && dx == 0 && kc == 0;
                acc[slot][cb] = __builtin_amdgcn_mfma_f32_16x16x32_f16(wf[(dy * 3 + dx) * 2 + kc], fb[(cb * 3 + dx) * 2 + kc],
                                                                       first ? bias4 : acc[slot][cb], 0, 0, 0);
              }
          if (dy == 2) fin();
          if (dyo == 0) mid();
        }
      }
    };

    if constexpr (ROLE == 0) {
#pragma unroll
      for (int kk = 0; kk < PF; ++kk)
        if (kk <= rows + 3) issue_row(kk);
    }
    asm volatile("s_waitcnt vmcnt(0)" ::: "memory");
    pair_barrier();

    const int K = (rows + 4 + 2 * BI + BI - 1) & ~(BI - 1);
    auto land_wait = [&](int nvm) __attribute__((always_inline)) {
      if (!nvm) asm volatile("s_waitcnt vmcnt(0)" ::: "memory");
      else if constexpr (NCB == 2) asm volatile("s_waitcnt vmcnt(5)" ::: "memory");
      else if (wq == 0) asm volatile("s_waitcnt vmcnt(6)" ::: "memory");
      else asm volatile("s_waitcnt vmcnt(4)" ::: "memory");
    };
    auto step = [&](auto PHc, auto FULLc, int k) __attribute__((always_inline)) {
      constexpr int PH = decltype(PHc)::value;
      constexpr bool FULL = decltype(FULLc)::value;
      using S0c = std::integral_constant<int, PH>;
      using S1c = std::integral_constant<int, (PH + 1) % 3>;
      using S2c = std::integral_constant<int, (PH + 2) % 3>;
      const int i = ra - 2 + k;
      long long t0 = 0, t1 = 0, t2 = 0;
      if constexpr (STAMP && FULL) t0 = clock64();
      if constexpr (ROLE == 0) {
        int nvm = 0;
        if (FULL || k <= rows + 3) {
          row_mfmas(X0 + pair_slot<XRING>(k) * ROWB, S1c{}, S0c{}, S2c{}, [&]() __attribute__((always_inline)) {
            const int trow = i - 1;
            const unsigned rowm = (trow >= 0 && trow < p.H) ? 0xFFFFFFFFu : 0u;
            unsigned char* tb = smem + T0 + ((k - 1) & (TRING - 1)) * TROWB + doff;
#pragma unroll
            for (int cb = 0; cb < NCB; ++cb) {
              const f32x4 v = acc[(PH + 2) % 3][cb];
              half4 h = {(half_t)v[0], (half_t)v[1], (half_t)v[2], (half_t)v[3]};
              h = actk<A1>(h, sl1);
              typedef unsigned u32x2 __attribute__((ext_vector_type(2)));
              u32x2 u = __builtin_bit_cast(u32x2, h);
              const unsigned m = rowm & tmask[cb];
              u[0] &= m; u[1] &= m;
              *reinterpret_cast<u32x2*>(tb + cb * 2048) = u;
            }
          }, [&]() __attribute__((always_inline)) {
            if (k + PF <= rows + 3 && !(p.experiment & 1)) nvm = issue_row(k + PF);
          });
        }
        if constexpr (STAMP && FULL) {
          asm volatile("s_waitcnt lgkmcnt(0)" ::: "memory");
          t1 = clock64();
        }
        land_wait(nvm);
      } else {
        const int srow = ra + k - 4 - 2 * BI;
        if (FULL || (srow >= ra && srow < rb)) {
#pragma unroll
// ... 4 lines not shown
            *reinterpret_cast<half8*>(dst) = yv;
          }
        }
        if constexpr (RES2) {
          const int nrow = srow + 1;
#pragma unroll
          for (int u = 0; u < NIT; ++u) {
            const bool ok = s_ok[u] && (FULL || (nrow >= ra && nrow < rb));
            const half_t* src = ok ? p.res2 + (long)n * p.r2_sn + ((long)nrow * p.W + c0 + s_yi + 32 * u) * p.r2_sp + s_c * 8 : p.zeros;
            r2v[u] = *reinterpret_cast<const half8*>(src);
          }
        }
        if (FULL || (k >= BI + 2 && k <= rows + 3 + BI)) {
          row_mfmas(T0 + ((k - T_LAG) & (TRING - 1)) * TROWB, S2c{}, S1c{}, S0c{}, [&]() __attribute__((always_inline)) {
            unsigned char* sb = smem + S0 + (k & (SRING - 1)) * SROW + doff;
            const unsigned char* xb = smem + X0 + pair_slot<XRING>(k - ID_LAG) * ROWB + roff;
#pragma unroll
            for (int cb = 0; cb < NCB; ++cb) {
              const f32x4 v = acc[PH][cb];
              half4 h = {(half_t)v[0], (half_t)v[1], (half_t)v[2], (half_t)v[3]};
              h = actk<A2>(h, sl2);
              if constexpr (ADDX) h = h + *reinterpret_cast<const half4*>(xb + cb * 2048);
              *reinterpret_cast<half4*>(sb + cb * 2048) = h;
            }
          }, []() {});
        }
        if constexpr (STAMP && FULL) {
          asm volatile("s_waitcnt lgkmcnt(0)" ::: "memory");
          t1 = clock64();
        }
      }
      if constexpr (STAMP && FULL) t2 = clock64();
      pair_barrier((k & (BI - 1)) != BI - 1 || (p.experiment & 4) != 0);
      if constexpr (STAMP && FULL) {
        const long long t3 = clock64();
        st_busy += t1 - t0; st_vm += t2 - t1; st_bar += t3 - t2; st_n += 1;
      }
    };
    using I0 = std::integral_constant<int, 0>;
    using I1 = std::integral_constant<int, 1>;
    using I2 = std::integral_constant<int, 2>;
    auto edge_steps = [&](int k, int kend) __attribute__((always_inline)) {
      for (; k < kend; k += 3) {
        step(I0{}, std::false_type{}, k);
        if (k + 1 < kend) step(I1{}, std::false_type{}, k + 1);
        if (k + 2 < kend) step(I2{}, std::false_type{}, k + 2);
      }
    };
    constexpr int KF = ((4 + 2 * BI + 2) / 3) * 3;
    edge_steps(0, KF);
    int k = KF;
    for (; k + 2 <= rows + 2; k += 3) {
      step(I0{}, std::true_type{}, k);
      step(I1{}, std::true_type{}, k + 1);
      step(I2{}, std::true_type{}, k + 2);
    }
    edge_steps(k, K);
  }
  };
  if (grp == 0) run(std::integral_constant<int, 0>{});
  else run(std::integral_constant<int, 1>{});
  if constexpr (STAMP) {
    if (lane == 0 && (int)blockIdx.x < stamp_cap) {
      long long* o = stamps + ((long)blockIdx.x * 8 + wave) * 8;
      o[0] = st_busy; o[1] = st_vm; o[2] = st_bar; o[3] = 0; o[4] = st_n;
    }
  }
}

}

static bool g_pair_enabled = true;
static int g_pair_experiment = 0;
static int g_pair_geometry = 0;
static long long* g_pair_stamps = nullptr;
static int g_pair_stamp_cap = 0;
extern "C" void tdvc_debug_set_stamp_buffer_pair(void* buf, int cap_blocks) { g_pair_stamps = (long long*)buf; g_pair_stamp_cap = cap_blocks; }
extern "C" void tdvc_debug_set_pair_experiment(int e) { g_pair_experiment = e; }
extern "C" void tdvc_debug_set_pair_geometry(int ncb) { g_pair_geometry = ncb; }
extern "C" void tdvc_debug_enable_conv_pair(int enable) { g_pair_enabled = enable != 0; }

extern "C" int64_t tdvc_conv_pair_packed_bytes(void) { return 2L * 4 * 18 * 64 * 8 * 2; }

extern "C" int tdvc_pack_conv_pair_weights(const float* w1_oihw, const float* w2_oihw, uint16_t* dst) {
  TDVC_CHECK(w1_oihw && w2_oihw && dst, "tdvc_pack_conv_pair_weights: null argument");
  for (int cv = 0; cv < 2; ++cv) {
    const float* w = cv ? w2_oihw : w1_oihw;
    for (int wv = 0; wv < 4; ++wv)
      for (int f = 0; f < 18; ++f)
        for (int ln = 0; ln < 64; ++ln)
          for (int j = 0; j < 8; ++j) {
            const int co = 16 * wv + (ln & 15), ci = 32 * (f & 1) + 8 * (ln >> 4) + j, t = f >> 1;
            const _Float16 h = (_Float16)w[((long)co * 64 + ci) * 9 + t];
            uint16_t bits;
            memcpy(&bits, &h, 2);
            dst[((((long)(cv * 4 + wv) * 18 + f) * 64) + ln) * 8 + j] = bits;
          }
  }
  return TDVC_OK;
}

static bool pair_buffers_ok(const tdvc_fmap& x, const tdvc_fmap& y) {
  const uintptr_t xa = (uintptr_t)x.p, ya = (uintptr_t)y.p;
  const uintptr_t xe = xa + 2 * ((uintptr_t)(x.N - 1) * x.sn + ((uintptr_t)x.H * x.W - 1) * x.sp + 64);
  const uintptr_t ye = ya + 2 * ((uintptr_t)(y.N - 1) * y.sn + ((uintptr_t)y.H * y.W - 1) * y.sp + 64);
  if (!(xa < ye && ya < xe)) return true;
  const uintptr_t gap = xa > ya ? xa - ya : ya - xa;
  return x.sp == y.sp && x.sn == y.sn && gap >= 128 && gap + 128 <= 2 * (uintptr_t)x.sp;
}

extern "C" int tdvc_conv_pair_supported(const tdvc_conv_pair_desc* d) {
  static const bool off = getenv("TDVC_NO_CONV_PAIR") != nullptr;
  if (off || !g_pair_enabled || !d) return 0;
  const tdvc_fmap &x = d->x, &y = d->y;
  const bool ok = fmap_ok16(x) && fmap_ok16(y) && x.C == 64 && y.C == 64 && x.N == y.N && x.H == y.H && x.W == y.W && d->w && d->bias &&
                  (!d->res2.p || (fmap_ok16(d->res2) && d->res2.C == 64 && d->res2.N == x.N && d->res2.H == x.H && d->res2.W == x.W)) &&
                  (long)x.H * x.W >= 8192 && x.H >= 16 && (x.p == y.p  || pair_buffers_ok(x, y)) &&
                  (d->act1 != TDVC_ACT_LRELU || (d->slope1 >= 0.f && d->slope1 <= 1.f)) && (d->act2 != TDVC_ACT_LRELU || (d->slope2 >= 0.f && d->slope2 <= 1.f));
  return ok ? 1 : 0;
}

extern "C" int tdvc_conv_pair(const tdvc_conv_pair_desc* d, void* stream) {
  TDVC_CHECK(d, "tdvc_conv_pair: null descriptor");
  TDVC_CHECK(fmap_ok16(d->x) && fmap_ok16(d->y) && d->x.C == 64 && d->y.C == 64, "tdvc_conv_pair: x and y must be fp16 maps of 64 channels");
  TDVC_CHECK(d->x.N == d->y.N && d->x.H == d->y.H && d->x.W == d->y.W, "tdvc_conv_pair: x / y geometry mismatch");
  TDVC_CHECK(d->w && d->bias, "tdvc_conv_pair: weights / bias missing");
  TDVC_CHECK(!d->res2.p || (fmap_ok16(d->res2) && d->res2.C == 64 && d->res2.N == d->x.N && d->res2.H == d->x.H && d->res2.W == d->x.W),
             "tdvc_conv_pair: res2 must be an fp16 map of the output geometry");
  TDVC_CHECK(pair_buffers_ok(d->x, d->y), "tdvc_conv_pair: x and y overlap (in-place operation is not supported: rows of x are re-read as halo)");
  TDVC_CHECK((d->act1 != TDVC_ACT_LRELU || (d->slope1 >= 0.f && d->slope1 <= 1.f)) && (d->act2 != TDVC_ACT_LRELU || (d->slope2 >= 0.f && d->slope2 <= 1.f)),
             "tdvc_conv_pair: LeakyReLU is computed as max(v, v * slope) and needs 0 <= slope <= 1");
  auto slope_of = [](int act, float slope) { return act == TDVC_ACT_NONE ? 1.f : (act == TDVC_ACT_RELU ? 0.f : slope); };
  TDVC_CHECK((d->act1 == TDVC_ACT_NONE || d->act1 == TDVC_ACT_RELU || d->act1 == TDVC_ACT_LRELU) &&
             (d->act2 == TDVC_ACT_NONE || d->act2 == TDVC_ACT_RELU || d->act2 == TDVC_ACT_LRELU), "tdvc_conv_pair: activations are none / ReLU / LeakyReLU");
  const void* zeros = nullptr;
  void* dump = nullptr;
  if (const int zrc = tdvc_scratch_pages(&zeros, &dump)) return zrc;
  PairParams p;
  p.x = reinterpret_cast<const half_t*>(d->x.p); p.x_sn = d->x.sn; p.x_sp = d->x.sp;
  p.y = reinterpret_cast<half_t*>(d->y.p); p.y_sn = d->y.sn; p.y_sp = d->y.sp;
  p.res2 = reinterpret_cast<const half_t*>(d->res2.p); p.r2_sn = d->res2.p ? d->res2.sn : 0; p.r2_sp = d->res2.p ? d->res2.sp : 0;
  p.w = reinterpret_cast<const half_t*>(d->w);
  p.bias = d->bias;
  p.zeros = reinterpret_cast<const half_t*>(zeros);
  p.experiment = g_pair_experiment;
  p.dump = reinterpret_cast<half_t*>(dump);
  p.N = d->x.N; p.H = d->x.H; p.W = d->x.W;
  p.slope1 = slope_of(d->act1, d->slope1);
  p.slope2 = slope_of(d->act2, d->slope2);
  auto waste = [&](int pw) { return (double)(((p.W + pw - 1) / pw) * (pw + 2)) / (double)p.W; };
  const int ncb = g_pair_geometry == 2 || g_pair_geometry == 4 ? g_pair_geometry : (waste(62) <= 1.12 * waste(30) ? 4 : 2);
  const int PWsel = 16 * ncb - 2;
  p.strips = (p.W + PWsel - 1) / PWsel;
  const long base = (long)p.N * p.strips;
  int best = 1;
  double best_eff = 0.;
  for (int sg = 1; sg <= 64 && (p.H + sg - 1) / sg >= 16; ++sg) {
    const int sr = (p.H + sg - 1) / sg, nseg = (p.H + sr - 1) / sr;
    const long jobs = base * nseg;
    const double eff = (double)jobs / (double)(((jobs + 255) / 256) * 256) * sr / (sr + 5.0);
    if (eff > best_eff + 1e-9) { best_eff = eff; best = sg; }
  }
  p.seg_rows = (p.H + best - 1) / best;
  p.segs = (p.H + p.seg_rows - 1) / p.seg_rows;
  p.jobs = (int)(base * p.segs);
  const int grid = p.jobs < 256 ? p.jobs : 256;
  p.pred = tdvc_launch_predicate();
  auto go = [&](auto kern, int lds) -> int {
    hipError_t err = hipFuncSetAttribute(reinterpret_cast<const void*>(kern), hipFuncAttributeMaxDynamicSharedMemorySize, lds);
    if (err != hipSuccess) { tdvc_set_error("tdvc_conv_pair: hipFuncSetAttribute failed: %s", hipGetErrorString(err)); return (int)err; }
    hipLaunchKernelGGL(kern, dim3(grid), dim3(NTHR), lds, reinterpret_cast<hipStream_t>(stream), p, g_pair_stamps, g_pair_stamp_cap);
    return 0;
  };
  const bool resblock = d->act1 == TDVC_ACT_RELU && d->act2 == TDVC_ACT_NONE;
  const int sel = (resblock ? 4 : 0) + (d->add_input ? 2 : 0) + (d->res2.p ? 1 : 0);
  auto launch = [&](auto ncbc) -> int {
    constexpr int NCB = decltype(ncbc)::value;
    constexpr int lds = PairGeo<NCB>::LDS;
    switch (sel) {
      case 0: return go(&conv_pair_kernel<NCB, 2, 2, false, false>, lds);
      case 1: return go(&conv_pair_kernel<NCB, 2, 2, false, true>, lds);
      case 2: return go(&conv_pair_kernel<NCB, 2, 2, true, false>, lds);
      case 3: return go(&conv_pair_kernel<NCB, 2, 2, true, true>, lds);
      case 4: return go(&conv_pair_kernel<NCB, 1, 0, false, false>, lds);
      case 5: return go(&conv_pair_kernel<NCB, 1, 0, false, true>, lds);
      case 6: return g_pair_stamps ? go(&conv_pair_kernel<NCB, 1, 0, true, false, true>, lds) : go(&conv_pair_kernel<NCB, 1, 0, true, false>, lds);
      default: return go(&conv_pair_kernel<NCB, 1, 0, true, true>, lds);
    }
  };
  const int rc = ncb == 4 ? launch(std::integral_constant<int, 4>{}) : launch(std::integral_constant<int, 2>{});
  if (rc) return rc;
  return tdvc_launch_status("tdvc_conv_pair");
}
```

### tdvc_amd/csrc/lib.cpp

```cpp
#include <hip/hip_runtime.h>
#include <stdarg.h>
#include <stdio.h>

#include <mutex>

#include "../../include/tdvc_hip.h"

static thread_local char g_err[512] = "";

void tdvc_set_error(const char* fmt, ...) {
  va_list ap;
  va_start(ap, fmt);
  vsnprintf(g_err, sizeof(g_err), fmt, ap);
  va_end(ap);
}

extern "C" int tdvc_abi_version(void) { return 7; }
extern "C" const char* tdvc_last_error(void) { return g_err; }

static thread_local const int* g_pred = nullptr;
static thread_local int g_pred_taken = 0, g_pred_last = 0;

extern "C" int tdvc_set_predicate(const int* flag) {
  if (reinterpret_cast<uintptr_t>(flag) & 3) { tdvc_set_error("tdvc_set_predicate: flag must be 4-byte aligned"); return TDVC_EINVAL; }
  g_pred = flag;
  return TDVC_OK;
}
extern "C" int tdvc_last_launch_predicated(void) { return g_pred_last; }
const int* tdvc_launch_predicate() {
  g_pred_taken = g_pred != nullptr;
  return g_pred;
}
void tdvc_note_launch() {
  g_pred_last = g_pred_taken;
  g_pred_taken = 0;
}

namespace {
constexpr int kMaxDev = 64;
constexpr size_t kZeroBytes = 4096, kDumpBytes = 16384;
std::mutex g_scratch_mu;
unsigned char* g_scratch[kMaxDev] = {};
}

int tdvc_scratch_pages(const void** zeros, void** dump) {
  int dev = 0;
  hipError_t err = hipGetDevice(&dev);
  if (err != hipSuccess || dev < 0 || dev >= kMaxDev) {
    tdvc_set_error("scratch pages: hipGetDevice failed or device index %d out of range: %s", dev, hipGetErrorString(err));
    return err != hipSuccess ? (int)err : TDVC_EINVAL;
  }
  std::lock_guard<std::mutex> lk(g_scratch_mu);
  if (!g_scratch[dev]) {
    unsigned char* p = nullptr;
    err = hipMalloc(reinterpret_cast<void**>(&p), kZeroBytes + kDumpBytes);
    if (err == hipSuccess) err = hipMemset(p, 0, kZeroBytes + kDumpBytes);
    if (err == hipSuccess) err = hipDeviceSynchronize();
    if (err != hipSuccess) {
      if (p) (void)hipFree(p);
      tdvc_set_error("scratch pages: allocation on device %d failed: %s", dev, hipGetErrorString(err));
      return (int)err;
    }
    g_scratch[dev] = p;
  }
  if (zeros) *zeros = g_scratch[dev];
  if (dump) *dump = g_scratch[dev] + kZeroBytes;
  return TDVC_OK;
}

extern "C" int tdvc_prepare_device(void) { return tdvc_scratch_pages(nullptr, nullptr); }
```

### tdvc_amd/csrc/pointwise.hip

```cpp
#include "pointwise_common.h"

namespace {

__global__ void nchw_to_fmap_kernel(const float* src, int C, FMap y) {
  const long npix = (long)y.H * y.W;
  const long i = (long)blockIdx.x * blockDim.x + threadIdx.x;
  if (i >= npix * y.N) return;
  const int n = (int)(i / npix);
  const long pix = i % npix;
  for (int c0 = 0; c0 < y.C; c0 += 8) {
    float v[8];
#pragma unroll
    for (int j = 0; j < 8; ++j) v[j] = (c0 + j < C) ? src[((long)n * C + c0 + j) * npix + pix] : 0.f;
    store8(y, n, pix, c0, v);
  }
}

__global__ void fmap_to_nchw_kernel(FMap x, int C, float* dst) {
  const long npix = (long)x.H * x.W;
  const long i = (long)blockIdx.x * blockDim.x + threadIdx.x;
  if (i >= npix * x.N) return;
  const int n = (int)(i / npix);
  const long pix = i % npix;
  for (int c0 = 0; c0 < C; c0 += 8) {
// ... 306 lines not shown
  ix = fminf((float)(W - 1), fmaxf(ix, 0.f));
  iy = fminf((float)(H - 1), fmaxf(iy, 0.f));
  const float xw = floorf(ix), yn = floorf(iy);
  const int ix0 = (int)xw, iy0 = (int)yn, ix1 = ix0 + 1, iy1 = iy0 + 1;
  const float w_nw = ((float)ix1 - ix) * ((float)iy1 - iy), w_ne = (ix - (float)ix0) * ((float)iy1 - iy);
  const float w_sw = ((float)ix1 - ix) * (iy - (float)iy0), w_se = (ix - (float)ix0) * (iy - (float)iy0);
  const float* sp = reinterpret_cast<const float*>(supp.p) + (long)n * supp.sn;
  float wv[3] = {0.f, 0.f, 0.f};
  const bool x0ok = ix0 >= 0 && ix0 < W, x1ok = ix1 >= 0 && ix1 < W, y0ok = iy0 >= 0 && iy0 < H, y1ok = iy1 >= 0 && iy1 < H;
  const float* rp = reinterpret_cast<const float*>(ref.p) + (long)n * ref.sn + pix * ref.sp;
  float r3[3];
  if constexpr (VEC) {
    const int cx0 = min(max(ix0, 0), W - 1), cx1 = min(max(ix1, 0), W - 1), cy0 = min(max(iy0, 0), H - 1), cy1 = min(max(iy1, 0), H - 1);
    const f32x4 nw = *reinterpret_cast<const f32x4*>(sp + ((long)cy0 * W + cx0) * supp.sp);
    const f32x4 ne = *reinterpret_cast<const f32x4*>(sp + ((long)cy0 * W + cx1) * supp.sp);
    const f32x4 sw = *reinterpret_cast<const f32x4*>(sp + ((long)cy1 * W + cx0) * supp.sp);
    const f32x4 se = *reinterpret_cast<const f32x4*>(sp + ((long)cy1 * W + cx1) * supp.sp);
    const f32x4 rr = *reinterpret_cast<const f32x4*>(rp);
#pragma unroll
    for (int c = 0; c < 3; ++c) {
      float s = 0.f;
      if (y0ok && x0ok) s += nw[c] * w_nw;
      if (y0ok && x1ok) s += ne[c] * w_ne;
      if (y1ok && x0ok) s += sw[c] * w_sw;
      if (y1ok && x1ok) s += se[c] * w_se;
      wv[c] = s;
      r3[c] = rr[c];
    }
  } else {
#pragma unroll
    for (int c = 0; c < 3; ++c) {
      float s = 0.f;
      if (y0ok && x0ok) s += sp[((long)iy0 * W + ix0) * supp.sp + c] * w_nw;
      if (y0ok && x1ok) s += sp[((long)iy0 * W + ix1) * supp.sp + c] * w_ne;
      if (y1ok && x0ok) s += sp[((long)iy1 * W + ix0) * supp.sp + c] * w_sw;
      if (y1ok && x1ok) s += sp[((long)iy1 * W + ix1) * supp.sp + c] * w_se;
      wv[c] = s;
      r3[c] = rp[c];
    }
  }
  float v[8] = {r3[0], r3[1], r3[2], wv[0], wv[1], wv[2], fx, fy};
  store8(cat8, n, pix, 0, v);
  float* fu = reinterpret_cast<float*>(flow_up.p) + (long)n * flow_up.sn + pix * flow_up.sp;
  if constexpr (VEC) {
    *reinterpret_cast<f32x2*>(fu) = f32x2{fx, fy};
  } else {
    fu[0] = fx;
    fu[1] = fy;
  }
}

__global__ void resize_bilinear_kernel(FMap x, FMap y, const float* chscale) {
  const long npix = (long)y.H * y.W;
  const long i = (long)blockIdx.x * blockDim.x + threadIdx.x;
  if (i >= npix * y.N) return;
  const int n = (int)(i / npix);
  const long pix = i % npix;
  const int oy = (int)(pix / y.W), ox = (int)(pix % y.W);
  const float rh = (float)x.H / (float)y.H, rw = (float)x.W / (float)y.W;
  const float sy = fmaxf(rh * (oy + 0.5f) - 0.5f, 0.f), sx = fmaxf(rw * (ox + 0.5f) - 0.5f, 0.f);
  const int y0 = (int)sy < x.H - 1 ? (int)sy : x.H - 1, x0 = (int)sx < x.W - 1 ? (int)sx : x.W - 1;
  const int y1 = y0 + (y0 < x.H - 1), x1 = x0 + (x0 < x.W - 1);
  const float ly1 = sy - y0, lx1 = sx - x0, ly0 = 1.f - ly1, lx0 = 1.f - lx1;
  const float* xp = reinterpret_cast<const float*>(x.p) + (long)n * x.sn;
  float* yp = reinterpret_cast<float*>(y.p) + (long)n * y.sn + pix * y.sp;
  for (int c = 0; c < y.C; ++c) {
    const float a = xp[((long)y0 * x.W + x0) * x.sp + c], b = xp[((long)y0 * x.W + x1) * x.sp + c];
    const float cc = xp[((long)y1 * x.W + x0) * x.sp + c], d = xp[((long)y1 * x.W + x1) * x.sp + c];
    float v = ly0 * (lx0 * a + lx1 * b) + ly1 * (lx0 * cc + lx1 * d);
    if (chscale) v *= chscale[c];
    yp[c] = v;
  }
}

constexpr int POOL_ROWS = 8;
__global__ __launch_bounds__(256) void avgpool_k_strip_kernel(FMap x, int scale, float* work, int wp, int nsplit, const int* pred) {
  __shared__ float red[256][9];
  TDVC_PREDICATE_RETURN(pred);
  const int chunks = x.C / 8;
  const int lanes = 256 / chunks;
  const int tid = threadIdx.x;
  const int ck = tid % chunks, pl = tid / chunks;
  const int cell = blockIdx.x / nsplit, strip = blockIdx.x - cell * nsplit, n = blockIdx.y;
  const int py = cell / wp, px = cell % wp;
  const int r0 = strip * POOL_ROWS, rows = min(POOL_ROWS, scale - r0);
  float acc[8];
#pragma unroll
  for (int j = 0; j < 8; ++j) acc[j] = 0.f;
  const int area = rows * scale;
  if (pl < lanes) {
    int k = pl;
    for (; k + 3 * lanes < area; k += 4 * lanes) {
      float v[4][8];
#pragma unroll
      for (int u = 0; u < 4; ++u) {
        const int kk = k + u * lanes;
        load8(x, n, (long)(py * scale + r0 + kk / scale) * x.W + (px * scale + kk % scale), ck * 8, v[u]);
      }
#pragma unroll
      for (int u = 0; u < 4; ++u)
#pragma unroll
        for (int j = 0; j < 8; ++j) acc[j] += v[u][j];
    }
    for (; k < area; k += lanes) {
      float v[8];
      load8(x, n, (long)(py * scale + r0 + k / scale) * x.W + (px * scale + k % scale), ck * 8, v);
#pragma unroll
      for (int j = 0; j < 8; ++j) acc[j] += v[j];
    }
  }
#pragma unroll
  for (int j = 0; j < 8; ++j) red[tid][j] = (pl < lanes) ? acc[j] : 0.f;
  __syncthreads();
  if (tid < x.C) {
    const int cc = tid / 8, j = tid % 8;
    float s = 0.f;
    for (int l = 0; l < lanes; ++l) s += red[l * chunks + cc][j];
    work[(((long)n * gridDim.x) + blockIdx.x) * x.C + tid] = s;
  }
}

__global__ void avgpool_k_final_kernel(const float* work, float* pooled, long total, int C_, int nsplit, float area, const int* pred) {
  TDVC_PREDICATE_RETURN(pred);
  const long i = (long)blockIdx.x * blockDim.x + threadIdx.x;
  if (i >= total) return;
  const long cell = i / C_;
  const int c = (int)(i - cell * C_);
  float s = 0.f;
  for (int k = 0; k < nsplit; ++k) s += work[(cell * nsplit + k) * C_ + c];
  pooled[i] = s / area;
}

typedef unsigned int u32x4 __attribute__((ext_vector_type(4)));
__device__ __forceinline__ u32x4* frame_word(const FMap& f, long i) {
  const int c8 = f.C / 8;
  const long per_img = (long)f.H * f.W * c8;
  const long n = i / per_img, rem = i - n * per_img;
  const long pix = rem / c8;
  const int ck = (int)(rem - pix * c8);
  return reinterpret_cast<u32x4*>(reinterpret_cast<half_t*>(f.p) + n * f.sn + pix * f.sp + ck * 8);
}
__global__ __launch_bounds__(EW_BLOCK) void frame_compare_kernel(FMap cur, FMap cache, long words, int* flag) {
  const long i = (long)blockIdx.x * blockDim.x + threadIdx.x;
  if (i >= words) return;
  const u32x4 a = *frame_word(cur, i), b = *frame_word(cache, i);
  if (((a[0] ^ b[0]) | (a[1] ^ b[1]) | (a[2] ^ b[2]) | (a[3] ^ b[3])) != 0u) flag[0] = 1;
}
__global__ __launch_bounds__(EW_BLOCK) void frame_refresh_kernel(FMap cur, FMap cache, long words, const int* flag) {
  if (flag[0] == 0) return;
  const long i = (long)blockIdx.x * blockDim.x + threadIdx.x;
  if (i >= words) return;
  *frame_word(cache, i) = *frame_word(cur, i);
}

__device__ __forceinline__ float block_sum(float v, float* sh) {
  const int tid = threadIdx.x;
#pragma unroll
  for (int o = 32; o > 0; o >>= 1) v += __shfl_xor(v, o);
  __syncthreads();
  if ((tid & 63) == 0) sh[tid >> 6] = v;
  __syncthreads();
  return sh[0] + sh[1] + sh[2] + sh[3];
}

__device__ __forceinline__ float patch_elem(const float* pm, int hp, int wp, int C, int pi, int pj, int d) {
  const int c = d / 9, k = d % 9;
  const int yy = 3 * pi - 3 + k / 3, xx = 3 * pj - 3 + k % 3;
  if (yy < 0 || yy >= hp || xx < 0 || xx >= wp) return 0.f;
  return pm[((long)yy * wp + xx) * C + c];
}

__global__ __launch_bounds__(256) void patch_match_kernel(const float* pin, const float* pref, int hp, int wp, int C,
                                                           int nph, int npw, int32_t* idx) {
  extern __shared__ float sm[];
  float* a = sm;
  __shared__ float sh[4];
  const int D = C * 9, L = nph * npw;
  const int l = blockIdx.x, n = blockIdx.y, tid = threadIdx.x;
  const float* pa = pin + (long)n * hp * wp * C;
  const float* pb = pref + (long)n * hp * wp * C;
  float ss = 0.f;
  for (int d = tid; d < D; d += 256) {
    const float v = patch_elem(pa, hp, wp, C, l / npw, l % npw, d);
    a[d] = v;
    ss += v * v;
  }
  const float na = fmaxf(sqrtf(block_sum(ss, sh)), 1e-12f);
  for (int d = tid; d < D; d += 256) a[d] = a[d] / na;
  __syncthreads();
  float best = -INFINITY;
  int besti = 0;
  for (int m = 0; m < L; ++m) {
    float sb = 0.f;
    for (int d = tid; d < D; d += 256) {
      const float v = patch_elem(pb, hp, wp, C, m / npw, m % npw, d);
      sb += v * v;
    }
    const float nb = fmaxf(sqrtf(block_sum(sb, sh)), 1e-12f);
    float dot = 0.f;
    for (int d = tid; d < D; d += 256) dot += a[d] * (patch_elem(pb, hp, wp, C, m / npw, m % npw, d) / nb);
    const float s = block_sum(dot, sh);
    if (s > best) { best = s; besti = m; }
  }
  if (tid == 0) idx[(long)n * L + l] = besti;
}

__global__ __launch_bounds__(256) void match_gather_kernel(FMap fin, FMap fref, const int32_t* idx, int ks, int nbh, int nbw, FMap cat) {
  const int lanes = fin.C / 8;
  const long npix = (long)fin.H * fin.W;
  const long i = (long)blockIdx.x * blockDim.x + threadIdx.x;
  const long t = i / lanes;
  const int c = (int)(i % lanes) * 8;
  const bool valid = t < npix * fin.N;
  const long tc = valid ? t : 0;
  const int n = (int)(tc / npix);
  const long pix = tc % npix;
  const int y = (int)(pix / fin.W), x = (int)(pix % fin.W);
  const int bi = y / ks + 1, bj = x / ks + 1;
  const int m = idx[(long)n * nbh * nbw + bi * nbw + bj];
  const int sy = (m / nbw - 1) * ks + y % ks, sx = (m % nbw - 1) * ks + x % ks;
  float a[8], b[8];
  load8(fin, n, pix, c, a);
  if (sy >= 0 && sy < fref.H && sx >= 0 && sx < fref.W) {
    load8(fref, n, (long)sy * fref.W + sx, c, b);
  } else {
#pragma unroll
    for (int j = 0; j < 8; ++j) b[j] = 0.f;
  }
  float w12 = 0.f, w1 = 0.f, w2 = 0.f;
#pragma unroll
  for (int j = 0; j < 8; ++j) { w12 += a[j] * b[j]; w1 += a[j] * a[j]; w2 += b[j] * b[j]; }
  for (int o = 1; o < lanes; o <<= 1) {
    w12 += __shfl_xor(w12, o);
    w1 += __shfl_xor(w1, o);
    w2 += __shfl_xor(w2, o);
  }
  const float cor = w12 / fmaxf(sqrtf(w1) * sqrtf(w2), 1e-8f);
  if (!valid) return;
#pragma unroll
  for (int j = 0; j < 8; ++j) { a[j] *= cor; b[j] *= cor; }
  store8(cat, n, pix, c, a);
  store8(cat, n, pix, fin.C + c, b);
}

__device__ __forceinline__ float sigmoidf_(float x) { return 1.f / (1.f + expf(-x)); }

__global__ __launch_bounds__(256) void eb_forward_kernel(FMap z, const float* params, FMap noise, FMap z_hat, float* partial) {
  __shared__ float sh[4];
  const long npix = (long)z.H * z.W;
  const long total = npix * z.C * z.N;
  const long i = (long)blockIdx.x * blockDim.x + threadIdx.x;
  float bits = 0.f;
  if (i < total) {
    const int c = (int)(i % z.C);
    const long t = i / z.C;
    const long pix = t % npix;
    const int n = (int)(t / npix);
    const float* P = params + (long)c * EB_NP;
    const float zv = reinterpret_cast<const float*>(z.p)[(long)n * z.sn + pix * z.sp + c];
    float v;
    if (noise.p) {
      v = zv + reinterpret_cast<const float*>(noise.p)[(long)n * noise.sn + pix * noise.sp + c];
    } else {
      const float med = P[58];
      v = rintf(zv - med) + med;
    }
    const float lower = eb_logits(P, v - 0.5f), upper = eb_logits(P, v + 0.5f);
    const float s = lower + upper;
    const float sign = s > 0.f ? -1.f : (s < 0.f ? 1.f : 0.f);
    float lik = fabsf(sigmoidf_(sign * upper) - sigmoidf_(sign * lower));
    lik = fmaxf(lik, 1e-9f);
    bits = -log2f(lik);
    if (z_hat.f32)
      reinterpret_cast<float*>(z_hat.p)[(long)n * z_hat.sn + pix * z_hat.sp + c] = v;
    else
      reinterpret_cast<half_t*>(z_hat.p)[(long)n * z_hat.sn + pix * z_hat.sp + c] = (half_t)v;
  }
  const float s = block_sum(bits, sh);
  if (threadIdx.x == 0) partial[blockIdx.x] = s;
}

__global__ __launch_bounds__(256) void gc_forward_kernel(FMap y, FMap gp, FMap noise, float* partial) {
  __shared__ float sh[4];
  const long npix = (long)y.H * y.W;
  const long total = npix * y.C * y.N;
  const long i = (long)blockIdx.x * blockDim.x + threadIdx.x;
  float bits = 0.f;
  if (i < total) {
    const int c = (int)(i % y.C);
    const long t = i / y.C;
    const long pix = t % npix;
    const int n = (int)(t / npix);
    const float yv = reinterpret_cast<const float*>(y.p)[(long)n * y.sn + pix * y.sp + c];
    const float* g = reinterpret_cast<const float*>(gp.p) + (long)n * gp.sn + pix * gp.sp;
    const float scale = fmaxf(g[c], 0.11f), mean = g[y.C + c];
    float v;
    if (noise.p)
      v = yv + reinterpret_cast<const float*>(noise.p)[(long)n * noise.sn + pix * noise.sp + c] - mean;
    else
      v = rintf(yv - mean);
    v = fabsf(v);
    const float k = 0.70710678118654752440f;
    const float upper = 0.5f * erfcf(-k * ((0.5f - v) / scale));
    const float lower = 0.5f * erfcf(-k * ((-0.5f - v) / scale));
    const float lik = fmaxf(upper - lower, 1e-9f);
    bits = -log2f(lik);
// ... 30 lines not shown
    float q[8];
    load8(noise, n, pix, c, q);
#pragma unroll
    for (int j = 0; j < 8; ++j) v[j] += q[j];
  } else {
#pragma unroll
    for (int j = 0; j < 8; ++j) v[j] = rintf(v[j]);
  }
  store8(y_hat, n, pix, c, v);
}

}

extern "C" int tdvc_nchw_to_fmap(const float* src, int C, const tdvc_fmap* y, void* stream) {
  TDVC_CHECK(src && y && fmap_any(*y) && C >= 1 && C <= y->C, "tdvc_nchw_to_fmap: bad arguments");
  const long total = (long)y->N * y->H * y->W;
  hipLaunchKernelGGL(nchw_to_fmap_kernel, grid1d(total), dim3(EW_BLOCK), 0, ST(stream), src, C, to_dev(*y));
  return tdvc_launch_status("tdvc_nchw_to_fmap");
}

extern "C" int tdvc_fmap_to_nchw(const tdvc_fmap* x, int C, float* dst, void* stream) {
  TDVC_CHECK(dst && x && fmap_any(*x) && C >= 1 && C <= x->C, "tdvc_fmap_to_nchw: bad arguments");
  const long total = (long)x->N * x->H * x->W;
  hipLaunchKernelGGL(fmap_to_nchw_kernel, grid1d(total), dim3(EW_BLOCK), 0, ST(stream), to_dev(*x), C, dst);
  return tdvc_launch_status("tdvc_fmap_to_nchw");
}

extern "C" int tdvc_scale_act_res(const tdvc_fmap* a, const float* gate, int act, float slope,
                                  const tdvc_fmap* r, float r_sign, const tdvc_fmap* y, const tdvc_fmap* y2, void* stream) {
  TDVC_CHECK(a && y && fmap_any(*a) && fmap_any(*y) && same_geom(*a, *y) && y->C == a->C, "tdvc_scale_act_res: bad a/y");
  if (r) TDVC_CHECK(fmap_any(*r) && same_geom(*a, *r) && r->C == a->C, "tdvc_scale_act_res: bad residual");
  if (y2) TDVC_CHECK(fmap_any(*y2) && same_geom(*a, *y2) && y2->C == a->C, "tdvc_scale_act_res: bad y2");
  const long total = (long)a->N * a->H * a->W * ((a->C + 7) / 8);
  const bool all16 = a->dtype == TDVC_F16 && y->dtype == TDVC_F16 && (!r || r->dtype == TDVC_F16) && (!y2 || y2->dtype == TDVC_F16) &&
                     (!gate || aligned16(gate)) && total < (1L << 31) - (1L << 23);
  if (all16) {
    constexpr int U = 4;
    long blocks = (total + 256 * U - 1) / (256 * U);
    if (blocks > 4096) blocks = 4096;
    hipLaunchKernelGGL(scale_act_res16_kernel<U>, dim3((unsigned)blocks), dim3(256), 0, ST(stream), to_dev(*a), gate, act, slope,
                       r ? to_dev(*r) : null_fmap(), r_sign, to_dev(*y), y2 ? to_dev(*y2) : null_fmap(), (unsigned)total, (unsigned)(a->C / 8),
                       (unsigned)((long)a->H * a->W));
    return tdvc_launch_status("tdvc_scale_act_res");
  }
  hipLaunchKernelGGL(scale_act_res_kernel, grid1d(total), dim3(EW_BLOCK), 0, ST(stream), to_dev(*a), gate, act, slope,
                     r ? to_dev(*r) : null_fmap(), r_sign, to_dev(*y), y2 ? to_dev(*y2) : null_fmap());
  return tdvc_launch_status("tdvc_scale_act_res");
}

extern "C" int tdvc_add_flow(const tdvc_fmap* off, const tdvc_fmap* flow, void* stream) {
  TDVC_CHECK(off && flow && fmap_ok16(*off) && fmap_ok32(*flow) && flow->C >= 2 && same_geom(*off, *flow), "tdvc_add_flow: bad arguments");
  const long total = (long)off->N * off->H * off->W * (off->C / 8);
  hipLaunchKernelGGL(add_flow_kernel, grid1d(total), dim3(EW_BLOCK), 0, ST(stream), to_dev(*off), to_dev(*flow));
  return tdvc_launch_status("tdvc_add_flow");
}

extern "C" int tdvc_bcast_add_act(const tdvc_fmap* x, const tdvc_fmap* b, int T, float slope, void* stream) {
  TDVC_CHECK(x && b && fmap_ok16(*x) && fmap_ok16(*b) && same_geom(*x, *b) && x->C == T * b->C, "tdvc_bcast_add_act: bad arguments");
  const long total = (long)x->N * x->H * x->W * (x->C / 8);
  if (T == 4 && total / 4 < (1L << 31)) {
    const long items = total / 4;
    hipLaunchKernelGGL(bcast_add_act_t_kernel<4>, grid1d(items), dim3(256), 0, ST(stream), to_dev(*x), to_dev(*b), slope, (unsigned)items,
                       (unsigned)(b->C / 8), (unsigned)((long)x->H * x->W));
    return tdvc_launch_status("tdvc_bcast_add_act");
  }
  hipLaunchKernelGGL(bcast_add_act_kernel, grid1d(total), dim3(EW_BLOCK), 0, ST(stream), to_dev(*x), to_dev(*b), slope);
  return tdvc_launch_status("tdvc_bcast_add_act");
}

extern "C" int tdvc_channel_sum(const tdvc_fmap* x, float* partial, int nblocks, void* stream) {
  TDVC_CHECK(x && partial && fmap_any(*x) && (x->C % 8) == 0 && x->C <= 256 && nblocks >= 1 && nblocks <= 4096, "tdvc_channel_sum: bad arguments");
  hipLaunchKernelGGL(channel_sum_kernel, dim3(nblocks, x->N), dim3(256), 0, ST(stream), to_dev(*x), partial, nblocks);
  return tdvc_launch_status("tdvc_channel_sum");
}

extern "C" int tdvc_se_gate(const float* partial, int nblocks, float inv_count, int N, int C, int Cmid,
                            const float* w1, const float* b1, const float* w2, const float* b2, float* gate, void* stream) {
  TDVC_CHECK(partial && w1 && b1 && w2 && b2 && gate && C <= 256 && Cmid <= 32 && N >= 1, "tdvc_se_gate: bad arguments");
  hipLaunchKernelGGL(se_gate_kernel, dim3(N), dim3(1024), 0, ST(stream), partial, nblocks, inv_count, C, Cmid, w1, b1, w2, b2, gate);
  return tdvc_launch_status("tdvc_se_gate");
}

extern "C" int tdvc_upsample2x(const tdvc_fmap* x, const tdvc_fmap* y, void* stream) {
  TDVC_CHECK(x && y && fmap_ok16(*x) && fmap_ok16(*y) && y->H == 2 * x->H && y->W == 2 * x->W && y->C == x->C && y->N == x->N,
             "tdvc_upsample2x: bad arguments");
  const long total = (long)y->N * y->H * y->W * (y->C / 8);
  hipLaunchKernelGGL(upsample2x_kernel, grid1d(total), dim3(EW_BLOCK), 0, ST(stream), to_dev(*x), to_dev(*y));
  return tdvc_launch_status("tdvc_upsample2x");
}

extern "C" int tdvc_avgpool2(const tdvc_fmap* x, const tdvc_fmap* y, void* stream) {
  TDVC_CHECK(x && y && fmap_ok32(*x) && fmap_ok32(*y) && y->H == x->H / 2 && y->W == x->W / 2 && y->C <= x->C && y->N == x->N,
             "tdvc_avgpool2: bad arguments");
  const long total = (long)y->N * y->H * y->W;
  hipLaunchKernelGGL(avgpool2_kernel, grid1d(total), dim3(EW_BLOCK), 0, ST(stream), to_dev(*x), to_dev(*y));
  return tdvc_launch_status("tdvc_avgpool2");
}

extern "C" int tdvc_spynet_level_input(const tdvc_fmap* ref, const tdvc_fmap* supp, const tdvc_fmap* flow_lo,
                                       const tdvc_fmap* flow_up, const tdvc_fmap* cat8, void* stream) {
  TDVC_CHECK(ref && supp && flow_up && cat8, "tdvc_spynet_level_input: null");
  TDVC_CHECK(fmap_ok32(*ref) && fmap_ok32(*supp) && ref->C >= 3 && supp->C >= 3 && same_geom(*ref, *supp), "tdvc_spynet_level_input: bad ref/supp");
  TDVC_CHECK(fmap_ok32(*flow_up) && flow_up->C >= 2 && same_geom(*ref, *flow_up), "tdvc_spynet_level_input: bad flow_up");
  TDVC_CHECK(fmap_ok16(*cat8) && cat8->C == 8 && same_geom(*ref, *cat8), "tdvc_spynet_level_input: bad cat8");
  if (flow_lo) TDVC_CHECK(fmap_ok32(*flow_lo) && flow_lo->C >= 2 && flow_lo->N == ref->N && flow_lo->H * 2 == ref->H && flow_lo->W * 2 == ref->W,
                          "tdvc_spynet_level_input: bad flow_lo");
  const long total = (long)ref->N * ref->H * ref->W;
  auto pix16 = [](const tdvc_fmap& f) { return f.C >= 4 && (f.sp % 4) == 0 && (f.sn % 4) == 0 && aligned16(f.p); };
  auto pix8 = [](const tdvc_fmap& f) { return (f.sp % 2) == 0 && (f.sn % 2) == 0 && (((uintptr_t)f.p) & 7) == 0; };
  const bool vec = pix16(*ref) && pix16(*supp) && pix8(*flow_up) && (!flow_lo || pix8(*flow_lo));
  if (vec)
    hipLaunchKernelGGL(spynet_level_input_kernel<true>, grid1d(total), dim3(EW_BLOCK), 0, ST(stream), to_dev(*ref), to_dev(*supp),
                       flow_lo ? to_dev(*flow_lo) : null_fmap(), to_dev(*flow_up), to_dev(*cat8));
  else
    hipLaunchKernelGGL(spynet_level_input_kernel<false>, grid1d(total), dim3(EW_BLOCK), 0, ST(stream), to_dev(*ref), to_dev(*supp),
                       flow_lo ? to_dev(*flow_lo) : null_fmap(), to_dev(*flow_up), to_dev(*cat8));
  return tdvc_launch_status("tdvc_spynet_level_input");
}

extern "C" int tdvc_resize_bilinear(const tdvc_fmap* x, const tdvc_fmap* y, const float* chscale, void* stream) {
  TDVC_CHECK(x && y && fmap_ok32(*x) && fmap_ok32(*y) && y->C <= x->C && y->N == x->N, "tdvc_resize_bilinear: bad arguments");
  const long total = (long)y->N * y->H * y->W;
  hipLaunchKernelGGL(resize_bilinear_kernel, grid1d(total), dim3(EW_BLOCK), 0, ST(stream), to_dev(*x), to_dev(*y), chscale);
  return tdvc_launch_status("tdvc_resize_bilinear");
}

extern "C" int64_t tdvc_avgpool_k_work_floats(int N, int hp, int wp, int C_, int scale) {
  return (int64_t)N * hp * wp * ((scale + POOL_ROWS - 1) / POOL_ROWS) * C_;
}

extern "C" int tdvc_avgpool_k(const tdvc_fmap* x, int scale, float* pooled, int hp, int wp, float* work, int64_t work_floats, void* stream) {
  TDVC_CHECK(x && pooled && work && fmap_ok16(*x) && x->C <= 256 && scale >= 1 && hp == x->H / scale && wp == x->W / scale && hp >= 1 && wp >= 1,
             "tdvc_avgpool_k: bad arguments");
  const int nsplit = (scale + POOL_ROWS - 1) / POOL_ROWS;
  TDVC_CHECK(work_floats >= tdvc_avgpool_k_work_floats(x->N, hp, wp, x->C, scale), "tdvc_avgpool_k: workspace too small (tdvc_avgpool_k_work_floats)");
  const int* pred = tdvc_launch_predicate();
  hipLaunchKernelGGL(avgpool_k_strip_kernel, dim3(hp * wp * nsplit, x->N), dim3(256), 0, ST(stream), to_dev(*x), scale, work, wp, nsplit, pred);
  const long total = (long)x->N * hp * wp * x->C;
  hipLaunchKernelGGL(avgpool_k_final_kernel, grid1d(total), dim3(256), 0, ST(stream), work, pooled, total, x->C, nsplit, (float)scale * (float)scale, pred);
  return tdvc_launch_status("tdvc_avgpool_k");
}

extern "C" int tdvc_frame_changed(const tdvc_fmap* cur, tdvc_fmap* cache, int* flag, void* stream) {
  TDVC_CHECK(cur && cache && flag && fmap_ok16(*cur) && fmap_ok16(*cache) && same_geom(*cur, *cache) && cur->C == cache->C &&
             (reinterpret_cast<uintptr_t>(flag) & 3) == 0, "tdvc_frame_changed: fp16 maps of one geometry and a 4-byte aligned flag");
  const hipError_t err = hipMemsetAsync(flag, 0, sizeof(int), ST(stream));
  if (err != hipSuccess) { tdvc_set_error("tdvc_frame_changed: hipMemsetAsync failed: %s", hipGetErrorString(err)); return (int)err; }
  const long words = (long)cur->N * cur->H * cur->W * (cur->C / 8);
  hipLaunchKernelGGL(frame_compare_kernel, grid1d(words), dim3(EW_BLOCK), 0, ST(stream), to_dev(*cur), to_dev(*cache), words, flag);
  hipLaunchKernelGGL(frame_refresh_kernel, grid1d(words), dim3(EW_BLOCK), 0, ST(stream), to_dev(*cur), to_dev(*cache), words, flag);
  return tdvc_launch_status("tdvc_frame_changed");
}

extern "C" int tdvc_patch_match(const float* pin, const float* pref, int N, int hp, int wp, int C, int32_t* idx, void* stream) {
  TDVC_CHECK(pin && pref && idx && N >= 1 && hp >= 1 && wp >= 1 && C >= 1 && C * 9 * 4 <= 60000, "tdvc_patch_match: bad arguments");
  const int nph = (hp + 3) / 3 + 1, npw = (wp + 3) / 3 + 1;
  hipLaunchKernelGGL(patch_match_kernel, dim3(nph * npw, N), dim3(256), (size_t)C * 9 * 4, ST(stream), pin, pref, hp, wp, C, nph, npw, idx);
  return tdvc_launch_status("tdvc_patch_match");
}

extern "C" int tdvc_match_gather(const tdvc_fmap* fin, const tdvc_fmap* fref, const int32_t* idx, int scale, int hp, int wp,
                                 const tdvc_fmap* cat, void* stream) {
  TDVC_CHECK(fin && fref && idx && cat && fmap_ok16(*fin) && fmap_ok16(*fref) && fmap_ok16(*cat), "tdvc_match_gather: bad fmaps");
  TDVC_CHECK(fin->C == 64 && fref->C == 64 && cat->C == 128 && same_geom(*fin, *fref) && same_geom(*fin, *cat), "tdvc_match_gather: needs C=64 / cat C=128");
  const int ks = 3 * scale;
  const int nbh = (fin->H + ks) / ks + 1, nbw = (fin->W + ks) / ks + 1;
  TDVC_CHECK(nbh == (hp + 3) / 3 + 1 && nbw == (wp + 3) / 3 + 1,
             "tdvc_match_gather: fold grid %dx%d != patch grid %dx%d (F.fold would raise, pnet.py:252)", nbh, nbw, (hp + 3) / 3 + 1, (wp + 3) / 3 + 1);
  const long total = (long)fin->N * fin->H * fin->W * 8;
  hipLaunchKernelGGL(match_gather_kernel, grid1d(total), dim3(256), 0, ST(stream), to_dev(*fin), to_dev(*fref), idx, ks, nbh, nbw, to_dev(*cat));
  return tdvc_launch_status("tdvc_match_gather");
}

extern "C" int tdvc_eb_forward(const tdvc_fmap* z, const float* params, const tdvc_fmap* noise,
                               const tdvc_fmap* z_hat, double* bits_out, float* partial, int partial_cap, void* stream) {
  TDVC_CHECK(z && params && z_hat && bits_out && partial && fmap_ok32(*z) && fmap_any(*z_hat) && same_geom(*z, *z_hat) && z_hat->C >= z->C,
             "tdvc_eb_forward: bad arguments");
  if (noise) TDVC_CHECK(fmap_ok32(*noise) && same_geom(*z, *noise) && noise->C >= z->C, "tdvc_eb_forward: bad noise");
  const long total = (long)z->N * z->H * z->W * z->C;
  const int nb = (int)((total + 255) / 256);
  TDVC_CHECK(nb <= partial_cap, "tdvc_eb_forward: partial buffer too small (%d < %d)", partial_cap, nb);
  hipLaunchKernelGGL(eb_forward_kernel, dim3(nb), dim3(256), 0, ST(stream), to_dev(*z), params, noise ? to_dev(*noise) : null_fmap(), to_dev(*z_hat), partial);
  hipLaunchKernelGGL(final_sum_kernel, dim3(1), dim3(256), 0, ST(stream), partial, nb, bits_out);
  return tdvc_launch_status("tdvc_eb_forward");
}

extern "C" int tdvc_gc_forward(const tdvc_fmap* y, const tdvc_fmap* gp, const tdvc_fmap* noise,
                               double* bits_out, float* partial, int partial_cap, void* stream) {
  TDVC_CHECK(y && gp && bits_out && partial && fmap_ok32(*y) && fmap_ok32(*gp) && same_geom(*y, *gp) && gp->C >= 2 * y->C, "tdvc_gc_forward: bad arguments");
  if (noise) TDVC_CHECK(fmap_ok32(*noise) && same_geom(*y, *noise) && noise->C >= y->C, "tdvc_gc_forward: bad noise");
  const long total = (long)y->N * y->H * y->W * y->C;
  const int nb = (int)((total + 255) / 256);
  TDVC_CHECK(nb <= partial_cap, "tdvc_gc_forward: partial buffer too small (%d < %d)", partial_cap, nb);
  hipLaunchKernelGGL(gc_forward_kernel, dim3(nb), dim3(256), 0, ST(stream), to_dev(*y), to_dev(*gp), noise ? to_dev(*noise) : null_fmap(), partial);
  hipLaunchKernelGGL(final_sum_kernel, dim3(1), dim3(256), 0, ST(stream), partial, nb, bits_out);
  return tdvc_launch_status("tdvc_gc_forward");
}

extern "C" int tdvc_quantize(const tdvc_fmap* y, const tdvc_fmap* noise, const tdvc_fmap* y_hat, void* stream) {
  TDVC_CHECK(y && y_hat && fmap_any(*y) && fmap_any(*y_hat) && same_geom(*y, *y_hat) && y_hat->C >= y->C, "tdvc_quantize: bad arguments");
  if (noise) TDVC_CHECK(fmap_any(*noise) && same_geom(*y, *noise) && noise->C >= y->C, "tdvc_quantize: bad noise");
  const long total = (long)y->N * y->H * y->W * ((y->C + 7) / 8);
  hipLaunchKernelGGL(quantize_kernel, grid1d(total), dim3(EW_BLOCK), 0, ST(stream), to_dev(*y), noise ? to_dev(*noise) : null_fmap(), to_dev(*y_hat));
  return tdvc_launch_status("tdvc_quantize");
}
```

### tdvc_amd/model/modules.py

```python
from __future__ import annotations

import torch
import torch.nn as nn

from .. import ops
from ..ops import ACT_LRELU, ACT_NONE, ACT_RELU, FM


class PackCache:

    def _pk(self, key, fn):
        c = self.__dict__.setdefault("_packed", {})
        if key not in c:
            c[key] = fn()
        return c[key]


def _dev(m: nn.Module):
    return next(m.parameters()).device


def pk_conv(owner: PackCache, name: str, conv: nn.Module, **kw) -> ops.PackedConv:
    def build():
        w = conv.weight
        if w.dim() == 5:
            co, ci, kt, kh, kw_ = w.shape
            if kt == 1:
                return ops.pack_conv(w.view(co, ci, kh, kw_), conv.bias, stride=1, pad=conv.padding[-1], device=w.device,
                                     param_w=conv.weight, param_b=conv.bias, **kw)
            return ops.pack_conv(w, conv.bias, stride=1, pad=0, device=w.device,
                                 layout=ops.convpack.WeightLayout.conv3d_temporal(co, ci, kt), param_w=conv.weight, param_b=conv.bias, **kw)
        return ops.pack_conv(w, conv.bias, stride=conv.stride[0], pad=conv.padding[0], device=w.device, **kw)
    return owner._pk(name, build)


class ConvAct(nn.Module):

    def __init__(self, cin, cout, k, stride=1, padding=0):
        super().__init__()
        self.conv = nn.Conv2d(cin, cout, k, stride, padding, bias=True)


class SELayer(nn.Module, PackCache):

    def __init__(self, channels, ratio=16):
        super().__init__()
        self.channels = channels
        self.conv1 = ConvAct(channels, int(channels / ratio), 1)
        self.conv2 = ConvAct(int(channels / ratio), channels, 1)

    def params(self) -> ops.SEParams:
        def build():
            c, m = self.channels, self.conv1.conv.out_channels
            f = lambda t: t.detach().float().contiguous()
            return ops.SEParams(f(self.conv1.conv.weight.view(m, c)), f(self.conv1.conv.bias),
                                f(self.conv2.conv.weight.view(c, m)), f(self.conv2.conv.bias), c, m,
                                params=(self.conv1.conv.weight, self.conv1.conv.bias, self.conv2.conv.weight, self.conv2.conv.bias))
        return self._pk("se", build)

    def gate(self, x: FM, partial=None) -> torch.Tensor:
        return ops.se_gate(x, self.params(), partial=partial)

    def run(self, x: FM, out: FM | None = None, act=ACT_NONE, slope=0.0, res: FM | None = None, out2: FM | None = None, sums: list | None = None):
        out = FM.empty(x.N, x.H, x.W, x.C, dtype=x.t.dtype, device=x.t.device) if out is None else out
        return ops.scale_act_res(x, out, gate=self.gate(x, sums[0] if sums else None), act=act, slope=slope, res=res, out2=out2)


class Res_Block(nn.Module, PackCache):

    def __init__(self, channels=64):
        super().__init__()
        self.conv1 = nn.Conv2d(channels, channels, 3, 1, 1)
        self.conv2 = nn.Conv2d(channels, channels, 3, 1, 1)

    def run(self, x: FM, out: FM | None = None, res2: FM | None = None) -> FM:
        if self.conv1.in_channels == 64 and ops.conv_pair_supported(x, out, res2) and (out is None or out.desc().p != x.desc().p):
            pp = self._pk("pair", lambda: ops.pack_conv_pair(self.conv1.weight, self.conv1.bias, self.conv2.weight, self.conv2.bias))
            return ops.conv_pair(x, pp, out=out, act1=ACT_RELU, act2=ACT_NONE, add_input=True, res2=res2)
        t = ops.conv(x, pk_conv(self, "c1", self.conv1), act=ACT_RELU)
        return ops.conv(t, pk_conv(self, "c2", self.conv2), out=out, res=x, res2=res2)


def res_stack(n, ch=64):
    return nn.Sequential(*[Res_Block(ch) for _ in range(n)])


def run_stack(stack, x: FM, out: FM | None = None, res2: FM | None = None) -> FM:
    n = len(stack)
    for i, blk in enumerate(stack):
        last = i == n - 1
        x = blk.run(x, out=out if last else None, res2=res2 if last else None)
    return x


class SPyNetBasicModule(nn.Module):
    def __init__(self):
        super().__init__()
        ch = [8, 32, 64, 32, 16, 2]
        self.basic_module = nn.Sequential(*[ConvAct(ch[i], ch[i + 1], 7, 1, 3) for i in range(5)])


class SPyNet(nn.Module, PackCache):

    def __init__(self):
        super().__init__()
        self.basic_module = nn.ModuleList([SPyNetBasicModule() for _ in range(6)])
        self.register_buffer("mean", torch.tensor([0.485, 0.456, 0.406]).view(1, 3, 1, 1))
        self.register_buffer("std", torch.tensor([0.229, 0.224, 0.225]).view(1, 3, 1, 1))

    def compute_flow(self, ref: FM, supp: FM) -> FM:
        refs, supps = [ref], [supp]
        for _ in range(5):
            refs.append(ops.avgpool2(refs[-1]))
            supps.append(ops.avgpool2(supps[-1]))
        refs, supps = refs[::-1], supps[::-1]
        dev = ref.t.device
        flow = None
        for lvl in range(6):
            r, s = refs[lvl], supps[lvl]
            up = FM.empty(r.N, r.H, r.W, 2, dtype=torch.float32, device=dev)
            x = FM.empty(r.N, r.H, r.W, 8, device=dev)
            ops.spynet_level_input(r, s, flow, up, x)
            bm = self.basic_module[lvl].basic_module
            for i in range(4):
                x = ops.conv(x, pk_conv(self, f"l{lvl}c{i}", bm[i].conv), act=ACT_RELU)
            flow = ops.conv(x, pk_conv(self, f"l{lvl}c4", bm[4].conv), res=up, out_dtype=torch.float32)
        return flow

    def run(self, ref: FM, supp: FM) -> FM:
        H, W = ref.H, ref.W
        Hu = H if H % 32 == 0 else 32 * (H // 32 + 1)
        Wu = W if W % 32 == 0 else 32 * (W // 32 + 1)
        if (Hu, Wu) != (H, W):
            ref, supp = ops.resize_bilinear(ref, Hu, Wu), ops.resize_bilinear(supp, Hu, Wu)
        flow = self.compute_flow(ref, supp)
        if (Hu, Wu) != (H, W):
            sc = torch.tensor([float(W) / float(Wu), float(H) / float(Hu)], dtype=torch.float32, device=flow.t.device)
            flow = ops.resize_bilinear(flow, H, W, sc)
        return flow


class FeaExtra(nn.Module, PackCache):

    def __init__(self, num_block):
        super().__init__()
        self.conv_first = nn.Conv2d(3, 64, 3, 1, 1)
        self.residual_layer = res_stack(num_block)

    def run(self, img8: FM, out: FM) -> FM:
        x = ops.conv(img8, pk_conv(self, "first", self.conv_first), act=ACT_LRELU, slope=0.1)
        return run_stack(self.residual_layer, x, out=out)


class OffsetGen(nn.Module, PackCache):

    def __init__(self, nf=64):
        super().__init__()
        self.offset_conv11 = nn.ModuleDict()
        self.offset_conv11_1 = nn.ModuleDict()
        self.offset_conv12 = nn.ModuleDict()
        self.feat_fusion = nn.ModuleDict()
        for i in (3, 2, 1):
            lv = f"l{i}"
            self.offset_conv11[lv] = nn.Conv2d(nf * 2, nf, 3, 1, 1)
            self.offset_conv11_1[lv] = nn.Conv2d(nf, nf, 3, 1, 1)
            self.offset_conv12[lv] = nn.Conv2d(nf, nf, 3, 1, 1)
            if i < 3:
                self.feat_fusion[lv] = nn.Conv2d(nf * 2, nf, 1, 1, 0)
        self.upsample_conv = nn.Conv2d(nf, nf, 3, 1, 1)
        self.conv_l2_1 = nn.Conv2d(nf, nf, 3, 2, 1)
        self.conv_l2_2 = nn.Conv2d(nf, nf, 3, 1, 1)
        self.conv_l3_1 = nn.Conv2d(nf, nf, 3, 2, 1)
        self.conv_l3_2 = nn.Conv2d(nf, nf, 3, 1, 1)
        self.spynet = SPyNet()
        self.attn = SELayer(64)
        self.feat_fusion_ = nn.Conv2d(nf, nf, 3, 1, 1)

    def run(self, feats: FM, cur32: FM, ref32: FM) -> FM:
        B, H, W = feats.N, feats.H, feats.W
        dev = feats.t.device
        lr = dict(act=ACT_LRELU, slope=0.1)
        cat1 = feats.ch(0, 128)
        cat2 = FM.empty(B, H // 2, W // 2, 128, device=dev)
        cat3 = FM.empty(B, H // 4, W // 4, 128, device=dev)
        for k in (0, 1):
            t = ops.conv(cat1.ch(64 * k, 64), pk_conv(self, "l2_1", self.conv_l2_1), **lr)
            ops.conv(t, pk_conv(self, "l2_2", self.conv_l2_2), out=cat2.ch(64 * k, 64), **lr)
            t = ops.conv(cat2.ch(64 * k, 64), pk_conv(self, "l3_1", self.conv_l3_1), **lr)
            ops.conv(t, pk_conv(self, "l3_2", self.conv_l3_2), out=cat3.ch(64 * k, 64), **lr)
        cats = {1: cat1, 2: cat2, 3: cat3}
        up_o1 = None
        off = None
        for i in (3, 2, 1):
            lv = f"l{i}"
            c = cats[i]
            o1 = ops.conv(c, pk_conv(self, "c11" + lv, self.offset_conv11[lv]), **lr)
            if i == 3:
                if ops.conv_pair_supported(o1):
                    c1_, c2_ = self.offset_conv11_1[lv], self.offset_conv12[lv]
                    pp = self._pk("pair_l3", lambda: ops.pack_conv_pair(c1_.weight, c1_.bias, c2_.weight, c2_.bias))
                    off = ops.conv_pair(o1, pp, act1=ACT_LRELU, slope1=0.1, act2=ACT_LRELU, slope2=0.1, add_input=False)
                else:
                    o1 = ops.conv(o1, pk_conv(self, "c11_1" + lv, self.offset_conv11_1[lv]), **lr)
                    off = ops.conv(o1, pk_conv(self, "c12" + lv, self.offset_conv12[lv]), **lr)
            else:
                ops.conv(o1, pk_conv(self, "c11_1" + lv, self.offset_conv11_1[lv]), out=up_o1.ch(64, 64), **lr)
                off = ops.conv(up_o1, pk_conv(self, "ff" + lv, self.feat_fusion[lv]), **lr)
            if i > 1:
                up = ops.upsample2x(off)
                up_o1 = FM.empty(B, up.H, up.W, 128, device=dev)
                ops.conv(up, pk_conv(self, "upc", self.upsample_conv), out=up_o1.ch(0, 64))
        flow = self.spynet.run(cur32, ref32)
        if ops.TAPE is not None:
            off = ops.clone(off)
        ops.add_flow(off, flow)
        sums = []
        e = ops.conv(off, pk_conv(self, "ff_", self.feat_fusion_), chan_sum=sums)
        return self.attn.run(e, sums=sums)


class DCN(nn.Module, PackCache):

    def __init__(self, cin, cout, k, stride, padding, dilation=1, deformable_groups=1):
        super().__init__()
        assert k == 3 and stride == 1 and padding == 1 and dilation == 1
        self.deformable_groups = deformable_groups
        self.weight = nn.Parameter(torch.zeros(cout, cin, k, k))
        self.bias = nn.Parameter(torch.zeros(cout))
        self.conv_offset_mask = nn.Conv2d(cin, deformable_groups * 3 * k * k, k, stride, padding)

    def run(self, x: FM, y: FM, out: FM, act=ACT_NONE, slope=0.0) -> FM:
        om = ops.conv(y, pk_conv(self, "om", self.conv_offset_mask))
        pc = self._pk("w", lambda: ops.pack_conv(self.weight, self.bias, stride=1, pad=1, ck=8 * self.deformable_groups,
                                                 device=self.weight.device))
        return ops.dcn_fused(x, om, pc, out, groups=self.deformable_groups, act=act, slope=slope, round16=True)


class MCNet(nn.Module, PackCache):

    def __init__(self, num_block):
        super().__init__()
        self.dconv = DCN(64, 64, 3, stride=1, padding=1, deformable_groups=8)
        self.recon_layer = res_stack(num_block)
        self.feat_down = nn.Conv2d(64, 3, 3, 1, 1)
        self.conv = nn.Conv2d(128, 64, 3, 1, 1)

    def run(self, offset: FM, feats: FM, out: FM) -> FM:
        ref = feats.ch(64, 64)
        dcn_out = feats.ch(128, 64)
        self.dconv.run(ref, offset, dcn_out, act=ACT_LRELU, slope=0.1)
        perm = list(range(64, 128)) + list(range(0, 64))
        pc = self._pk("conv", lambda: ops.pack_conv(self.conv.weight, self.conv.bias, stride=1, pad=1, cin_perm=perm,
                                                    device=self.conv.weight.device))
        o2 = ops.conv(feats.ch(64, 128), pc, act=ACT_LRELU, slope=0.1)
        return run_stack(self.recon_layer, o2, out=out, res2=dcn_out)


class Bottleneck3D(nn.Module):
    def __init__(self):
        super().__init__()
        self.conv1 = nn.Conv3d(64, 64, (1, 3, 3), padding=(0, 1, 1))
        self.spatial_conv3d = nn.Conv3d(64, 64, (1, 3, 3), padding=(0, 1, 1))
        self.temporal_conv3d = nn.Conv3d(64, 64, (3, 1, 1), stride=(3, 1, 1), bias=False)
        self.conv3 = nn.Conv3d(64, 64, (1, 3, 3), padding=(0, 1, 1))


LOOPFILTER_PAIR = True
LOOPFILTER_BCAST = True


class LoopFilter(nn.Module, PackCache):

    def __init__(self):
        super().__init__()
        self.conv01 = nn.Conv2d(3, 64, 3, 1, 1)
        self.conv02 = nn.Conv2d(64, 64, 3, 1, 1)
        self.conv1 = nn.Conv3d(64, 64, (1, 3, 3), padding=(0, 1, 1))
        self.layer1 = Bottleneck3D()
        self.attn = SELayer(64)
        self.feat_fusion = nn.Conv2d(256, 64, 1, 1)

    def _slices(self, name, conv, src: FM, dst: FM, res_buf: FM | None = None, **kw):
        pc = pk_conv(self, name, conv)
        for b in range(src.N):
            ops.conv(src.as_slices(b, 4, 64), pc, out=dst.as_slices(b, 4, 64),
                     res=res_buf.as_slices(b, 4, 64) if res_buf is not None else None, **kw)

    def run(self, xt: FM, refs8: FM, out: FM) -> FM:
        B, H, W = xt.N, xt.H, xt.W
        dev = xt.t.device
        lr = dict(act=ACT_LRELU, slope=0.1)
        p01, p02 = pk_conv(self, "c01", self.conv01), pk_conv(self, "c02", self.conv02)
        a = FM.empty(B, H, W, 256, device=dev)
        fuse = LOOPFILTER_PAIR and ops.conv_pair_supported(a.as_slices(0, 4, 64).batch(0, 3))
        if fuse:
            pp = self._pk("pair_c02_c1", lambda: ops.pack_conv_pair(self.conv02.weight, self.conv02.bias,
                                                                     self.conv1.weight.view(64, 64, 3, 3), self.conv1.bias))
            pc1 = pk_conv(self, "c1", self.conv1)
        for b in range(B):
            t = ops.conv(refs8.batch(4 * b + 1, 3), p01, **lr)
            if fuse:
                ops.conv_pair(t, pp, out=a.as_slices(b, 4, 64).batch(0, 3), act1=ACT_NONE, act2=ACT_LRELU, slope2=0.1, add_input=False)
                ops.conv(xt.as_slices(b, 4, 64).batch(3, 1), pc1, out=a.as_slices(b, 4, 64).batch(3, 1), **lr)
            else:
                ops.conv(t, p02, out=xt.as_slices(b, 4, 64).batch(0, 3))
        if not fuse:
            self._slices("c1", self.conv1, xt, a, **lr)
        l1 = self.layer1
        bf = FM.empty(B, H, W, 256, device=dev)
        s = FM.empty(B, H, W, 256, device=dev)
        if LOOPFILTER_PAIR and ops.conv_pair_supported(a.as_slices(0, 4, 64), s.as_slices(0, 4, 64)):
            pp = self._pk("pair_b1_bs", lambda: ops.pack_conv_pair(l1.conv1.weight.view(64, 64, 3, 3), l1.conv1.bias,
                                                                    l1.spatial_conv3d.weight.view(64, 64, 3, 3), l1.spatial_conv3d.bias))
            for b in range(B):
                ops.conv_pair(a.as_slices(b, 4, 64), pp, out=s.as_slices(b, 4, 64), act1=ACT_LRELU, slope1=0.1, act2=ACT_NONE,
                              add_input=False)
        else:
            self._slices("b1", l1.conv1, a, bf, **lr)
            self._slices("bs", l1.spatial_conv3d, bf, s)
        if ops.TAPE is None and LOOPFILTER_BCAST and H * W >= 8192:
            ops.conv(s.ch(0, 192), pk_conv(self, "bt", l1.temporal_conv3d), out=s.ch(0, 64), bcast_T=4, bcast_slope=0.1)
        else:
            tm = ops.conv(s.ch(0, 192), pk_conv(self, "bt", l1.temporal_conv3d))
            if ops.TAPE is not None:
                s = ops.clone(s)
            ops.bcast_add_act(s, tm, 4, 0.1)
        o = bf if ops.TAPE is None else FM.empty(B, H, W, 256, device=dev)
        self._slices("b3", l1.conv3, s, o, res_buf=a)
        sums = []
        f = ops.conv(o, pk_conv(self, "ff", self.feat_fusion), chan_sum=sums, **lr)
        return self.attn.run(f, out=out, res=xt.ch(192, 64), sums=sums)


class FeatureExtract(nn.Module, PackCache):

    def __init__(self, cin, mid, nblocks):
        super().__init__()
        self.conv_first = nn.Conv2d(cin, mid, 3, 1, 1)
        self.body = res_stack(nblocks, mid)
        self.conv_last = nn.Conv2d(mid, mid, 3, 1, 1)

    def run(self, x: FM, out: FM | None = None) -> FM:
        x1 = ops.conv(x, pk_conv(self, "first", self.conv_first), act=ACT_LRELU, slope=0.01)
        t = run_stack(self.body, x1)
        return ops.conv(t, pk_conv(self, "last", self.conv_last), out=out, res=x1)


FEATUREFIX_REUSE = True


class IFrameReuse:

    __slots__ = ("key", "y", "iframe", "pref", "flag", "usable", "log")

    def __init__(self, key):
        self.key, self.usable, self.log = key, None, []
        self.y = self.iframe = self.pref = self.flag = None


class FeatureFix(nn.Module, PackCache):

    def __init__(self):
        super().__init__()
        self.FeatureExtract_input = FeatureExtract(64, 64, 2)
        self.FeatureExtract_ref = FeatureExtract(3, 64, 2)
        self.recon_layer = res_stack(2)
        self.conv_10 = nn.Conv2d(64, 64, 3, 2, 1)
        self.conv_11 = nn.Conv2d(64, 64, 3, 1, 1)
        self.conv_12 = nn.Conv2d(64, 64, 3, 2, 1)
        self.conv_13 = nn.Conv2d(64, 64, 3, 1, 1)
        self.featfusion = nn.Conv2d(128, 64, 3, 1, 1)
        self.featfusion2 = nn.Conv2d(128, 64, 3, 1, 1)
        self.featdown = nn.Conv2d(64, 3, 3, 1, 1)
        self.attn = SELayer(64)

    def run(self, x: FM, iframe8: FM, training: bool, trace=None) -> torch.Tensor:
        B, H, W = x.N, x.H, x.W
        dev = x.t.device
        lr = dict(act=ACT_LRELU, slope=0.1)
        fin = self.FeatureExtract_input.run(x)
        scale = 8 if training else int(H / 8)
        if FEATUREFIX_REUSE and not training and ops.TAPE is None and ops.PROFILE is None and trace is None and not iframe8.f32:
            y, pref = self._iframe_features(iframe8, scale)
            fref = y.ch(64, 64)
        else:
            y = FM.empty(B, H, W, 128, device=dev)
            fref = self.FeatureExtract_ref.run(iframe8, out=y.ch(64, 64))
            pref = ops.avgpool_k(fref, scale)
        pin = ops.avgpool_k(fin, scale)
        idx = ops.patch_match(pin, pref)
        cat = FM.empty(B, H, W, 128, device=dev)
        ops.match_gather(fin, fref, idx, scale, cat)
        ops.conv(cat, pk_conv(self, "ff", self.featfusion), out=y.ch(0, 64), **lr)
        sums = []
        o2 = ops.conv(y, pk_conv(self, "ff2", self.featfusion2), chan_sum=sums)
        o2 = self.attn.run(o2, sums=sums, **lr)
        o = run_stack(self.recon_layer, o2, res2=x)
        rgb = torch.empty((B, 3, H, W), dtype=torch.float32, device=dev)
        ops.conv(o, pk_conv(self, "down", self.featdown), act=ops.ACT_CLAMP01, nchw_out=rgb)
        if trace is not None:
            trace.update(ff_idx=idx, ff_fin=fin, ff_fref=fref)
        return rgb

    def reuse_state(self) -> IFrameReuse | None:
        return self.__dict__.get("_packed", {}).get("iframe_reuse")

    def _iframe_features(self, iframe8: FM, scale: int):
        B, H, W = iframe8.N, iframe8.H, iframe8.W
        dev = iframe8.t.device
        key = (dev.index, ops._stream().value, B, H, W, scale)
        cache = self.__dict__.setdefault("_packed", {})
        st = cache.get("iframe_reuse")
        if st is None or st.key != key:
            st = cache["iframe_reuse"] = IFrameReuse(key)

        def chain(y, pref):
            fref = self.FeatureExtract_ref.run(iframe8, out=y.ch(64, 64))
            ops.avgpool_k(fref, scale, out=pref)

        def fresh():
            return (FM.empty(B, H, W, 128, device=dev),
                    torch.empty((B, H // scale, W // scale, 64), dtype=torch.float32, device=dev))

        if st.usable is False:
            y, pref = fresh()
            chain(y, pref)
            return y, pref
        if st.usable is None:
            st.y, st.pref = fresh()
            st.iframe = FM.empty(B, H, W, iframe8.C, device=dev)
            st.flag = torch.ones(1, dtype=torch.int32, device=dev)
            ops.copy_cast(iframe8, st.iframe)
        else:
            ops.frame_changed(iframe8, st.iframe, st.flag)
        with ops.predicate(st.flag) as log:
            chain(st.y, st.pref)
        st.log = list(log)
        y, pref = st.y, st.pref
        if not all(log):
            if st.usable is not None:
                chain(y, pref)
# ... 6 lines not shown
```

### tdvc_amd/ops.py

```python
from __future__ import annotations

import ctypes as C
from dataclasses import dataclass

import numpy as np
import torch

from . import _lib as L
from . import convpack
from ._lib import (ACT_CLAMP01, ACT_LRELU, ACT_NONE, ACT_RELU, GDN_FWD, GDN_INV, GDN_NONE, OUT_NCHW_F32,
                   OUT_NHWC, OUT_SHUFFLE2)


_raw_stream = torch._C._cuda_getCurrentRawStream
_cur_dev = torch._C._cuda_getDevice
FORCE_STREAM = None
FORCE_KEEP = None


def _stream():
    if FORCE_STREAM is not None:
        return C.c_void_p(FORCE_STREAM)
    return C.c_void_p(_raw_stream(_cur_dev()))


PROFILE = None
TAPE = None
_IN_BACKWARD = False


_PRED_LOG = None


class predicate:

    def __init__(self, flag: torch.Tensor):
        assert flag.dtype == torch.int32 and flag.is_cuda and flag.numel() >= 1
        self.flag = flag

    def __enter__(self):
        global _PRED_LOG
        if _PRED_LOG is not None:
            raise L.TdvcHipError("ops.predicate does not nest")
        L.check(L.lib().tdvc_set_predicate(self.flag.data_ptr()), "set_predicate")
        _PRED_LOG = []
        return _PRED_LOG

    def __exit__(self, *exc):
        global _PRED_LOG
        _PRED_LOG = None
        L.lib().tdvc_set_predicate(None)
        return False


def _log_predicated(kernels=1):
    if _PRED_LOG is not None:
        _PRED_LOG.extend([bool(L.lib().tdvc_last_launch_predicated())] * kernels)


def frame_changed(cur: FM, cache: FM, flag: torch.Tensor) -> None:
    dc, dk = cur.desc(), cache.desc()
    L.check(L.lib().tdvc_frame_changed(C.byref(dc), C.byref(dk), flag.data_ptr(), _stream()), "frame_changed")


def _rec(name, *args):
    if TAPE is not None and not _IN_BACKWARD:
        from . import autograd
        getattr(autograd, "record_" + name)(TAPE, *args)


def pad8(c: int) -> int:
    return (c + 7) // 8 * 8


class FM:

    __slots__ = ("t", "off", "N", "C", "H", "W", "sn", "sp", "_d")

    def __init__(self, t: torch.Tensor, off: int = 0, N: int | None = None, C_: int | None = None, sn: int | None = None):
        assert t.dim() == 4 and (t.shape[3] == 1 or t.stride(3) == 1)
        self.t, self.off = t, off
        self._d = None
        self.N = t.shape[0] if N is None else N
        self.C = t.shape[3] if C_ is None else C_
        self.H, self.W = t.shape[1], t.shape[2]
        if self.W > 1:
            self.sp = t.stride(2)
        elif self.H > 1:
            self.sp = t.stride(1)
        else:
            self.sp = t.shape[3]
        assert self.H == 1 or t.stride(1) == self.W * self.sp, "rows of a feature map must be dense (row stride = W * pixel stride)"
        self.sn = (t.stride(0) if t.shape[0] > 1 else self.H * self.W * self.sp) if sn is None else sn

    @staticmethod
    def empty(N, H, W, C_, dtype=torch.float16, device="cuda"):
        return FM(torch.empty((N, H, W, C_), dtype=dtype, device=device))

    @staticmethod
    def zeros(N, H, W, C_, dtype=torch.float16, device="cuda"):
        return FM(torch.zeros((N, H, W, C_), dtype=dtype, device=device))

    @property
    def f32(self):
        return self.t.dtype == torch.float32

    def ch(self, c0, C_):
        assert 0 <= c0 and c0 + C_ <= self.C
        return FM(self.t, self.off + c0, self.N, C_, self.sn)

    def batch(self, n0, N):
        assert 0 <= n0 and n0 + N <= self.N
        return FM(self.t, self.off + n0 * self.sn, N, self.C, self.sn)

    def as_slices(self, b, T, Cs):
        assert self.C == T * Cs and 0 <= b < self.N
        return FM(self.t, self.off + b * self.sn, T, Cs, Cs)

    def desc(self) -> L.FMapDesc:
        d = self._d
        if d is None:
            p = self.t.data_ptr() + self.off * self.t.element_size()
            d = self._d = L.FMapDesc(p, self.N, self.H, self.W, self.C, self.sn, self.sp, L.F32 if self.f32 else L.F16)
        return d

    def to_nchw(self, C_=None) -> torch.Tensor:
        C_ = self.C if C_ is None else C_
        out = torch.empty((self.N, C_, self.H, self.W), dtype=torch.float32, device=self.t.device)
        d = self.desc()
        L.check(L.lib().tdvc_fmap_to_nchw(C.byref(d), C_, out.data_ptr(), _stream()), "fmap_to_nchw")
        return out


_NULL_FM = L.FMapDesc(None, 0, 0, 0, 0, 0, 0, 0)


def from_nchw(x: torch.Tensor, Cpad: int | None = None, dtype=torch.float16, out: FM | None = None) -> FM:
    assert x.is_cuda and x.dtype == torch.float32
    x = x.contiguous()
    N, Cc, H, W = x.shape
    if out is None:
        out = FM.empty(N, H, W, pad8(Cc) if Cpad is None else Cpad, dtype=dtype, device=x.device)
    d = out.desc()
    L.check(L.lib().tdvc_nchw_to_fmap(x.data_ptr(), Cc, C.byref(d), _stream()), "nchw_to_fmap")
    return out


FORMS_CREATED = 0


@dataclass
class PackedConv:
    w: torch.Tensor
    bias: torch.Tensor
    cout: int
    cin: int
    kh: int
    kw: int
    stride: int
    pad: int
    ck: int
    taps: list
    shuffle: bool = False
    cin_real: int = 0
    s2d: bool = False
    flops_per_px: float = 0.0
    wsrc: torch.Tensor | None = None
    bsrc: torch.Tensor | None = None
    layout: convpack.WeightLayout | None = None
    tables: convpack.PackTables | None = None
    orig: dict | None = None
    dgrad: "PackedConv | None" = None
    param_w: torch.Tensor | None = None
    param_b: torch.Tensor | None = None
    owner: object | None = None
    w32: torch.Tensor | None = None
    w32_buf: torch.Tensor | None = None

    def __post_init__(self):
        global FORMS_CREATED
        FORMS_CREATED += 1

    def packed_f32(self) -> torch.Tensor:
        if self.w32 is None:
            self.w32, self.w32_buf = _pack_from_tables_f32(self.wsrc, self.tables, self.w32_buf), None
        return self.w32

    def stale_f32(self):
        if self.w32 is not None:
            self.w32_buf, self.w32 = self.w32, None

    def repack(self):
        _pack_from_tables(self.wsrc, self.tables, self.w)
        self.stale_f32()
        if self.bsrc is not None:
            b = self.bsrc.detach().float()
            self.bias[:self.cout] = b[torch.from_numpy(convpack.shuffle_perm(self.cout)).to(b.device)] if self.shuffle else b
        if self.dgrad is not None:
            self.dgrad.repack()
        for key in ("_colpc", "_plain"):
            aux = self.__dict__.get(key)
            if aux is not None:
                aux.repack()


def _cout_pad(cout):
    return 32 if cout <= 32 else 64 * ((cout + 63) // 64)


def _s2d_weights(w: torch.Tensor) -> torch.Tensor:
    cout, C_, kh, kw = w.shape
    assert (kh, kw) == (3, 3)
    w2 = torch.zeros(cout, 4 * C_, 2, 2)
    for py in range(2):
        for px in range(2):
# ... 1033 lines not shown
```

### tdvc_amd/train.py

```python
from __future__ import annotations

import gc
from collections.abc import Mapping

import torch
import torch.distributed as dist

from . import autograd, ops
from .synth import split_optim_params


def refresh_packed(model: torch.nn.Module) -> None:
    pcs = []
    mods = model.__dict__.get("_mods_list")
    if mods is None:
        mods = model.__dict__["_mods_list"] = list(model.modules())
    from .model.coder import GDN, gdn_refresh_batched
    pcs += gdn_refresh_batched([m for m in mods if isinstance(m, GDN)])
    for m in mods:
        m.__dict__.pop("_ar_cache", None)
        if isinstance(m, GDN):
            continue
        if hasattr(m, "refresh_packed"):
            m.refresh_packed()
            continue
        pk = m.__dict__.get("_packed", {})
        pk.pop("iframe_reuse", None)
        pcs += [pc for pc in pk.values() if isinstance(pc, ops.PackedConv)]
        for key in [k for k, v in pk.items() if isinstance(v, ops.PackedConvPair)]:
            del pk[key]
    batch = model.__dict__.get("_pack_batch")
    if batch is None or batch.forms != ops.FORMS_CREATED or [id(pc) for pc in batch.roots] != [id(pc) for pc in pcs]:
        batch = ops.PackBatch(pcs)
        batch.roots = pcs
        model.__dict__["_pack_batch"] = batch
    batch.run()


class GradBuckets:

    def __init__(self, params, bucket_bytes: int = 16 << 20):
        self.params = [p for p in params if p.requires_grad]
        self.bucket_bytes = int(bucket_bytes)
        self._layout([(p, -1) for p in self.params], keep=False)

    def _layout(self, order, keep: bool):
        old = {id(p): p.grad for p, _ in order} if keep else {}
        self.buckets, self.ready_at, self._works = [], [], {}
        cur, cur_n = [], 0
        for p, r in order:
            if cur and (cur_n + p.numel()) * 4 > self.bucket_bytes:
                self._close(cur, cur_n, old)
                cur, cur_n = [], 0
            cur.append((p, r))
            cur_n += p.numel()
        if cur:
            self._close(cur, cur_n, old)
        self._by_ready = {}
        for i, r in enumerate(self.ready_at):
            self._by_ready.setdefault(r, []).append(i)

    def _close(self, ps, n, old):
        flat = torch.zeros(n, dtype=torch.float32, device=ps[0][0].device)
        off = 0
        for p, _ in ps:
            v = flat[off:off + p.numel()].view_as(p)
            if old.get(id(p)) is not None:
                v.copy_(old[id(p)])
            p.grad = v
            off += p.numel()
        self.buckets.append(flat)
        self.ready_at.append(max(r for _, r in ps))

    def reorder(self, ready: dict, n_nodes: int):
        self.n_nodes = int(n_nodes)
        order = sorted(((p, ready.get(id(p), -1)) for p in self.params), key=lambda t: t[1])
        self._layout(order, keep=True)

    def zero(self):
        for b in self.buckets:
            b.zero_()

    force_async = False

    def _distributed(self) -> bool:
        return dist.is_available() and dist.is_initialized() and (dist.get_world_size() > 1 or self.force_async)

    def node_done(self, k: int):
        for i in self._by_ready.get(k, ()):
            if self._distributed() and i not in self._works:
                self._works[i] = dist.all_reduce(self.buckets[i], op=dist.ReduceOp.SUM, async_op=True)

    def all_reduce_mean(self):
        if not self._distributed():
            return
        world = dist.get_world_size()
        for i, b in enumerate(self.buckets):
            if i not in self._works:
                self._works[i] = dist.all_reduce(b, op=dist.ReduceOp.SUM, async_op=True)
        for i, b in enumerate(self.buckets):
            self._works[i].wait()
            b.mul_(1.0 / world)
        self._works = {}


class StepLog(Mapping):
    KEYS = ("rd_loss", "mse", "bpp_res", "bpp_mv", "aux_loss", "grad_norm", "loss_scale", "skipped")

    def __init__(self, owner, vals):
        self._owner, self._d, self._scale_after = owner, None, None
        self._keys = self.KEYS + (("distortion",) if vals.numel() == 8 else ())
        if vals.is_cuda:
            self._host = torch.empty(vals.numel(), dtype=torch.float32, pin_memory=True)
            self._host.copy_(vals, non_blocking=True)
            self._ev = torch.cuda.Event()
            self._ev.record()
        else:
            self._host, self._ev = vals.detach().float(), None

    def _arrived(self, block):
        if self._ev is not None:
            if not block and not self._ev.query():
                return False
            self._ev.synchronize()
            self._ev = None
        return True

    def _vals(self):
        if self._d is None:
            if self._scale_after is None:
                self._owner._settle(self)
            v = self._host.tolist()
            skipped = v[6] != 0.0
            self._d = dict(rd_loss=v[0], mse=v[1], bpp_res=v[2], bpp_mv=v[3], aux_loss=v[4],
                           grad_norm=float("nan") if skipped else v[5], loss_scale=self._scale_after, skipped=skipped)
            if len(v) == 8:
                self._d["distortion"] = v[7]
            self._owner = None
        return self._d

    def __getitem__(self, k):
        return self._vals()[k]

    def __iter__(self):
        return iter(self._keys)

    def __len__(self):
        return len(self._keys)

    def __repr__(self):
        return f"StepLog({self._vals()!r})"


def _seed_mse(recon, target, diff, lam, loss_scale):
    return None, diff * (2.0 * lam * loss_scale / diff.numel())


def _seed_from(fn):
    def seed(recon, target, diff, lam, loss_scale):
        D, g = fn(recon, target)
        if g.shape != recon.shape or g.dtype != torch.float32:
            raise ValueError(f"distortion: the gradient must be fp32 of recon's shape {tuple(recon.shape)}, got {g.dtype} {tuple(g.shape)}")
        return D.reshape(()).float(), g * (lam * loss_scale)
    return seed


def msssim_distortion(recon, target):
    from . import metrics
    n = recon.shape[0]
    ms, g = metrics.ms_ssim_value_and_grad(recon, target, data_range=1.0, grad_out=torch.full((n,), -1.0 / n, dtype=torch.float32, device=recon.device))
    return 1.0 - ms.mean(), g


class TrainStep:
    def __init__(self, model, train_lambda: float = 2048.0, lr: float = 1e-4, loss_scale: float = 1024.0, clip: float = 2.0,
                 dynamic_scale: bool = True, growth_interval: int = 2000, graph: bool = False, graph_warmup: int = 2,
                 side_stream: bool = True, scale_update: str = "exact", freeze_gc: bool = True, distortion="mse", coder_fp32: bool = False):
        if distortion == "mse":
            self._seed = _seed_mse
        elif distortion == "ms-ssim":
# ... 153 lines not shown
```

Measured before the change: 49.55 frames/s.

## Reuse loop-filter reference features across P-frames via a per-image predicated ring

```diff
diff --git a/include/tdvc_hip.h b/include/tdvc_hip.h
--- a/include/tdvc_hip.h
+++ b/include/tdvc_hip.h
@@ -59,7 +59,10 @@
 
 int tdvc_set_predicate(const int* flag);
 int tdvc_last_launch_predicated(void);
+#define TDVC_MAX_PREDICATE_IMAGES 4
+int tdvc_set_predicate_images(const int* flags, int n);
 int tdvc_frame_changed(const tdvc_fmap* cur, tdvc_fmap* cache, int* flag, void* stream);
+int tdvc_frames_changed(const tdvc_fmap* cur, tdvc_fmap* cache, int* flags, unsigned force_mask, void* stream);
 
 
 int tdvc_conv_plan(int cin, int kh, int kw, int stride);
diff --git a/tdvc_amd/_lib.py b/tdvc_amd/_lib.py
--- a/tdvc_amd/_lib.py
+++ b/tdvc_amd/_lib.py
@@ -58,8 +58,10 @@
     "tdvc_last_conv_kernel": (C.c_char_p, []),
     "tdvc_prepare_device": (_i, []),
     "tdvc_set_predicate": (_i, [_P]),
+    "tdvc_set_predicate_images": (_i, [_P, _i]),
     "tdvc_last_launch_predicated": (_i, []),
     "tdvc_frame_changed": (_i, [_FM, _FM, _P, _P]),
+    "tdvc_frames_changed": (_i, [_FM, _FM, _P, C.c_uint, _P]),
     "tdvc_conv_plan": (_i, [_i, _i, _i, _i]),
     "tdvc_conv_packed_bytes": (_i64, [_i, _i, _i, _i]),
     "tdvc_pack_conv_weights": (_i, [_P, _i, _i, _i, _i, _i, _i, _P, _P, _i, _P]),
diff --git a/tdvc_amd/csrc/common.h b/tdvc_amd/csrc/common.h
--- a/tdvc_amd/csrc/common.h
+++ b/tdvc_amd/csrc/common.h
@@ -18,10 +18,23 @@
 
 const int* tdvc_launch_predicate();
 void tdvc_note_launch();
+const int* tdvc_launch_predicate_images(int N);
 #define TDVC_PREDICATE_RETURN(pred)                       \
   do {                                                    \
     if ((pred) != nullptr && *(pred) == 0) return;        \
   } while (0)
+
+struct TdvcActiveImages { unsigned list; int count; };
+__device__ __forceinline__ TdvcActiveImages tdvc_active_images(const int* flags, int nimg) {
+  TdvcActiveImages a = {0xE4u, nimg};
+  if (flags != nullptr) {
+    a.list = 0u; a.count = 0;
+    for (int i = 0; i < nimg; ++i)
+      if (flags[i] != 0) { a.list |= (unsigned)i << (2 * a.count); ++a.count; }
+  }
+  return a;
+}
+__device__ __forceinline__ int tdvc_active_image(const TdvcActiveImages& a, int j) { return (int)((a.list >> (2 * j)) & 3u); }
 
 #define TDVC_CHECK(cond, ...)            \
   do {                                   \
diff --git a/tdvc_amd/csrc/conv_c8.hip b/tdvc_amd/csrc/conv_c8.hip
--- a/tdvc_amd/csrc/conv_c8.hip
+++ b/tdvc_amd/csrc/conv_c8.hip
@@ -8,8 +8,14 @@
 constexpr int EW_C8 = 32 * 144;
 constexpr int LDS_C8 = 256 + NW_C8 * EW_C8;
 
-__global__ __launch_bounds__(NTHR_C8, 4) void conv_c8_kernel(const ConvParams p, int tiles_x, int total_tiles) {
+template <bool IMG>
+__global__ __launch_bounds__(NTHR_C8, 4) void conv_c8_kernel(const ConvParams p, int tiles_x, int total_tiles, const int* img, int nimg) {
   TDVC_PREDICATE_RETURN(p.pred);
+  TdvcActiveImages act = {0u, 0};
+  if constexpr (IMG) {
+    act = tdvc_active_images(img, nimg);
+    if (act.count == 0) return;
+  }
   extern __shared__ __attribute__((aligned(16))) unsigned char smem[];
   float* bias_s = reinterpret_cast<float*>(smem);
   const int tid = threadIdx.x, lane = tid & 63;
@@ -36,15 +42,20 @@
   const int nwaves = (int)gridDim.x * NW_C8;
   const int w0 = (int)blockIdx.x * NW_C8 + wave;
   const int per_img = tiles_x * p.Ho;
+  if constexpr (IMG) total_tiles = act.count * per_img;
   const half8 zero8 = {0, 0, 0, 0, 0, 0, 0, 0};
 
   auto load_b = [&](int tile, half8 (&b)[5]) {
-    const int n = tile / per_img, rem = tile - n * per_img;
+    const int ni = tile / per_img, rem = tile - ni * per_img;
+    const int n = IMG ? tdvc_active_image(act, ni) : ni;
     const int oy = rem / tiles_x, ox0 = (rem - oy * tiles_x) * 32;
     const half_t* xn = p.x + (long)n * p.x_sn;
+    int lv = lane;
+    if constexpr (IMG) asm volatile("" : "+v"(lv));
 #pragma unroll
     for (int s = 0; s < 5; ++s) {
-      const int iy = oy + tdy[s], ix = ox0 + r + tdx[s];
+      const int tv = min(2 * s + (lv >> 5), 8);
+      const int iy = oy + (IMG ? tv / 3 - 1 : tdy[s]), ix = ox0 + (IMG ? (lv & 31) + tv % 3 - 1 : r + tdx[s]);
       const bool ok = iy >= 0 && iy < p.H && ix >= 0 && ix < p.W;
       const half_t* src = xn + ((long)(ok ? iy : 0) * p.W + (ok ? ix : 0)) * p.x_sp;
       const half8 v = *reinterpret_cast<const half8*>(src);
@@ -68,7 +79,8 @@
     for (int s = 0; s < 5; ++s)
 #pragma unroll
       for (int mt = 0; mt < 2; ++mt) acc[mt][0] = __builtin_amdgcn_mfma_f32_32x32x16_f16(wa[mt][s], bcur[s], acc[mt][0], 0, 0, 0);
-    const int n = tile / per_img, rem = tile - n * per_img;
+    const int ni = tile / per_img, rem = tile - ni * per_img;
+    const int n = IMG ? tdvc_active_image(act, ni) : ni;
     const int oy = rem / tiles_x, ox0 = (rem - oy * tiles_x) * 32;
     {
       constexpr int EPS = 144;
@@ -115,6 +127,8 @@
   const long total = (long)N * p.Ho * tiles_x;
   int grid = (int)((total + NW_C8 - 1) / NW_C8);
   if (grid > 256 * 4) grid = 256 * 4;
-  hipLaunchKernelGGL(conv_c8_kernel, dim3(grid), dim3(NTHR_C8), LDS_C8, st, q, tiles_x, (int)total);
+  const int* img = q.pred ? nullptr : tdvc_launch_predicate_images(N);
+  if (img) hipLaunchKernelGGL(conv_c8_kernel<true>, dim3(grid), dim3(NTHR_C8), LDS_C8, st, q, tiles_x, (int)total, img, N);
+  else hipLaunchKernelGGL(conv_c8_kernel<false>, dim3(grid), dim3(NTHR_C8), LDS_C8, st, q, tiles_x, (int)total, nullptr, 0);
   return tdvc_launch_status("tdvc_conv2d(c8)");
 }
diff --git a/tdvc_amd/csrc/conv_common.h b/tdvc_amd/csrc/conv_common.h
--- a/tdvc_amd/csrc/conv_common.h
+++ b/tdvc_amd/csrc/conv_common.h
@@ -313,7 +313,7 @@
       opix[k] = ok[k] ? oy * p.Wo + ox : 0;
     }
     half8 r1[4], r2[4];
-    if (has1) {
+    if (has1 && !BCAST) {
 #pragma unroll
       for (int k = 0; k < 4; ++k) r1[k] = *reinterpret_cast<const half8*>(rb1 + (long)opix[k] * p.res.sp);
     }
@@ -350,9 +350,10 @@
       for (int k = 0; k < 4; ++k) {
         const half8 v = *reinterpret_cast<const half8*>(ew + (k * 8 + prow) * EPS + chunk * 16);
         half_t* yp = yb + (long)opix[k] * p.y.sp;
+        const half_t* sp = has1 ? rb1 + (long)opix[k] * p.res.sp : yp;
         half8 xs[4];
 #pragma unroll
-        for (int t = 0; t < 4; ++t) xs[t] = *reinterpret_cast<const half8*>(yp + t * 64);
+        for (int t = 0; t < 4; ++t) xs[t] = *reinterpret_cast<const half8*>(sp + t * 64);
 #pragma unroll
         for (int t = 0; t < 4; ++t) {
           half8 o;
diff --git a/tdvc_amd/csrc/conv_dispatch.hip b/tdvc_amd/csrc/conv_dispatch.hip
--- a/tdvc_amd/csrc/conv_dispatch.hip
+++ b/tdvc_amd/csrc/conv_dispatch.hip
@@ -72,7 +72,8 @@
 bool bcast_eligible(Pick& k, const ConvParams& p) {
   const tdvc_conv_desc* d = k.d;
   return d->bcast_T == 4 && d->kh == 1 && d->kw == 1 && d->stride == 1 && d->pad == 0 && d->cout == 64 && d->y.C == 64 && d->y.sp >= 4 * 64 &&
-         d->y.dtype == TDVC_F16 && d->out_mode == TDVC_OUT_NHWC && d->act == TDVC_ACT_NONE && !d->gdn && !d->res.p && !d->res2.p &&
+         d->y.dtype == TDVC_F16 && d->out_mode == TDVC_OUT_NHWC && d->act == TDVC_ACT_NONE && !d->gdn && !d->res2.p &&
+         (!d->res.p || (d->res.dtype == TDVC_F16 && d->res.C == 64 && d->res.sp >= 4 * 64 && d->res.N == d->y.N && d->res.H == d->y.H && d->res.W == d->y.W)) &&
          !d->square_input && !d->round_before_act && d->bias && d->bcast_slope >= 0.f && d->bcast_slope <= 1.f && conv_v5_eligible(d, k.Ho, k.Wo) &&
          convk::conv_is_lean(p);
 }
@@ -88,7 +89,7 @@
 
 const Entry kTable[] = {
     {"conv_mfma_v5(bcast)", convk::SW_V5, bcast_eligible, bcast_launch, [](const tdvc_conv_desc* d) { return d->bcast_T != 0; },
-     "tdvc_conv2d: bcast_T needs a plain 1x1 / stride 1 conv to 64 channels of >= 8192 pixels, y a 64-channel window of a buffer with >= 4 slices, bcast_T == 4"},
+     "tdvc_conv2d: bcast_T needs a plain 1x1 / stride 1 conv to 64 channels of >= 8192 pixels, y (and res, the optional source of the slices) a 64-channel window of a buffer with >= 4 slices, bcast_T == 4"},
     {"conv_row(s2d)", convk::SW_ROW, [](Pick& k, const ConvParams& p) { return k.d->s2d && row_eligible(k, p); },
      [](const Pick& k, const ConvParams& p, hipStream_t st) { return launch_conv_row(k.geo, p, k.N(), st); }, nullptr, nullptr},
     {"conv_mfma_v3(s2d)", convk::SW_V3, [](Pick& k, const ConvParams&) { return k.d->s2d && conv_v3_eligible(k.d, k.Ho, k.Wo); },
diff --git a/tdvc_amd/csrc/conv_pair.hip b/tdvc_amd/csrc/conv_pair.hip
--- a/tdvc_amd/csrc/conv_pair.hip
+++ b/tdvc_amd/csrc/conv_pair.hip
@@ -55,6 +55,8 @@
   float slope1, slope2;
   int experiment;
   const int* pred;
+  const int* img;
+  unsigned split[4];
 };
 
 __device__ __forceinline__ int swz(int q) { return (int)((0x62654210u >> (4 * ((q >> 1) & 7))) & 7u); }
@@ -89,6 +91,15 @@
 template <int NCB, int A1, int A2, bool ADDX, bool RES2, bool STAMP = false>
 __global__ __launch_bounds__(NTHR, 1) void conv_pair_kernel(const PairParams p, long long* stamps = nullptr, int stamp_cap = 0) {
   TDVC_PREDICATE_RETURN(p.pred);
+  const TdvcActiveImages act = tdvc_active_images(p.img, p.N);
+  if (act.count == 0) return;
+  int p_seg_rows = p.seg_rows, p_segs = p.segs, p_jobs = p.jobs;
+  if (p.img != nullptr) {
+    const unsigned sp = act.count == 1 ? p.split[0] : (act.count == 2 ? p.split[1] : (act.count == 3 ? p.split[2] : p.split[3]));
+    p_seg_rows = (int)(sp & 0xFFFFu);
+    p_segs = (int)(sp >> 16);
+    p_jobs = act.count * p.strips * p_segs;
+  }
   using G = PairGeo<NCB>;
   constexpr int PW = G::PW, ROWB = G::ROWB, TROWB = G::TROWB, SROW = G::SROW, XRING = G::XRING, PF = G::PF, X0 = G::X0, T0 = G::T0, S0 = G::S0;
   constexpr int NF = 6 * NCB;
@@ -134,12 +145,12 @@
   const int nwg = (int)gridDim.x, b = (int)blockIdx.x;
   int jfirst, jstep, jend;
   if ((nwg & 7) == 0) {
-    const int per = (p.jobs + 7) >> 3;
+    const int per = (p_jobs + 7) >> 3;
     jfirst = (b & 7) * per + (b >> 3);
     jstep = nwg >> 3;
-    jend = min(p.jobs, ((b & 7) + 1) * per);
+    jend = min(p_jobs, ((b & 7) + 1) * per);
   } else {
-    jfirst = b; jstep = nwg; jend = p.jobs;
+    jfirst = b; jstep = nwg; jend = p_jobs;
   }
 
   const half_t hs1 = (half_t)p.slope1, hs2 = (half_t)p.slope2;
@@ -151,10 +162,11 @@
   half8 r2v[NIT] = {};
 
   for (int job = jfirst; job < jend; job += jstep) {
-    const int n = job / (p.strips * p.segs);
-    const int rem = job - n * (p.strips * p.segs);
+    const int ni = job / (p.strips * p_segs);
+    const int rem = job - ni * (p.strips * p_segs);
+    const int n = p.img != nullptr ? tdvc_active_image(act, ni) : ni;
     const int seg = rem / p.strips, strip = rem - seg * p.strips;
-    const int c0 = strip * PW, ra = seg * p.seg_rows, rb = min(p.H, ra + p.seg_rows);
+    const int c0 = strip * PW, ra = seg * p_seg_rows, rb = min(p.H, ra + p_seg_rows);
     const int rows = rb - ra;
     const half_t* xn = p.x + (long)n * p.x_sn;
     half_t* yn = p.y + (long)n * p.y_sn;
@@ -465,20 +477,34 @@
   const int ncb = g_pair_geometry == 2 || g_pair_geometry == 4 ? g_pair_geometry : (waste(62) <= 1.12 * waste(30) ? 4 : 2);
   const int PWsel = 16 * ncb - 2;
   p.strips = (p.W + PWsel - 1) / PWsel;
-  const long base = (long)p.N * p.strips;
-  int best = 1;
-  double best_eff = 0.;
-  for (int sg = 1; sg <= 64 && (p.H + sg - 1) / sg >= 16; ++sg) {
-    const int sr = (p.H + sg - 1) / sg, nseg = (p.H + sr - 1) / sr;
-    const long jobs = base * nseg;
-    const double eff = (double)jobs / (double)(((jobs + 255) / 256) * 256) * sr / (sr + 5.0);
-    if (eff > best_eff + 1e-9) { best_eff = eff; best = sg; }
-  }
-  p.seg_rows = (p.H + best - 1) / best;
-  p.segs = (p.H + p.seg_rows - 1) / p.seg_rows;
-  p.jobs = (int)(base * p.segs);
-  const int grid = p.jobs < 256 ? p.jobs : 256;
+  auto split_for = [&](int nimg, int& seg_rows, int& segs) {
+    const long base = (long)nimg * p.strips;
+    int best = 1;
+    double best_eff = 0.;
+    for (int sg = 1; sg <= 64 && (p.H + sg - 1) / sg >= 16; ++sg) {
+      const int sr = (p.H + sg - 1) / sg, nseg = (p.H + sr - 1) / sr;
+      const long jobs = base * nseg;
+      const double eff = (double)jobs / (double)(((jobs + 255) / 256) * 256) * sr / (sr + 5.0);
+      if (eff > best_eff + 1e-9) { best_eff = eff; best = sg; }
+    }
+    seg_rows = (p.H + best - 1) / best;
+    segs = (p.H + seg_rows - 1) / seg_rows;
+    return (int)(base * segs);
+  };
+  p.jobs = split_for(p.N, p.seg_rows, p.segs);
+  int grid = p.jobs < 256 ? p.jobs : 256;
   p.pred = tdvc_launch_predicate();
+  p.img = nullptr;
+  memset(p.split, 0, sizeof(p.split));
+  if (!p.pred && p.N <= TDVC_MAX_PREDICATE_IMAGES && p.H < 65536 && (p.img = tdvc_launch_predicate_images(p.N)) != nullptr) {
+    for (int a = 1; a <= p.N; ++a) {
+      int sr, sg;
+      const int jobs = split_for(a, sr, sg);
+      p.split[a - 1] = (unsigned)sr | ((unsigned)sg << 16);
+      const int g = jobs < 256 ? jobs : 256;
+      if (g > grid) grid = g;
+    }
+  }
   auto go = [&](auto kern, int lds) -> int {
     hipError_t err = hipFuncSetAttribute(reinterpret_cast<const void*>(kern), hipFuncAttributeMaxDynamicSharedMemorySize, lds);
     if (err != hipSuccess) { tdvc_set_error("tdvc_conv_pair: hipFuncSetAttribute failed: %s", hipGetErrorString(err)); return (int)err; }
diff --git a/tdvc_amd/csrc/lib.cpp b/tdvc_amd/csrc/lib.cpp
--- a/tdvc_amd/csrc/lib.cpp
+++ b/tdvc_amd/csrc/lib.cpp
@@ -15,16 +15,32 @@
   va_end(ap);
 }
 
-extern "C" int tdvc_abi_version(void) { return 7; }
+extern "C" int tdvc_abi_version(void) { return 8; }
 extern "C" const char* tdvc_last_error(void) { return g_err; }
 
 static thread_local const int* g_pred = nullptr;
 static thread_local int g_pred_taken = 0, g_pred_last = 0;
+static thread_local const int* g_pred_img = nullptr;
+static thread_local int g_pred_img_n = 0;
 
 extern "C" int tdvc_set_predicate(const int* flag) {
   if (reinterpret_cast<uintptr_t>(flag) & 3) { tdvc_set_error("tdvc_set_predicate: flag must be 4-byte aligned"); return TDVC_EINVAL; }
+  if (flag && g_pred_img) { tdvc_set_error("tdvc_set_predicate: a per-image predicate is set (clear it first)"); return TDVC_EINVAL; }
   g_pred = flag;
   return TDVC_OK;
+}
+extern "C" int tdvc_set_predicate_images(const int* flags, int n) {
+  if (!flags || n == 0) { g_pred_img = nullptr; g_pred_img_n = 0; return TDVC_OK; }
+  if (reinterpret_cast<uintptr_t>(flags) & 3) { tdvc_set_error("tdvc_set_predicate_images: flags must be 4-byte aligned"); return TDVC_EINVAL; }
+  if (n < 1 || n > TDVC_MAX_PREDICATE_IMAGES) { tdvc_set_error("tdvc_set_predicate_images: 1 <= n <= %d images, got %d", TDVC_MAX_PREDICATE_IMAGES, n); return TDVC_EINVAL; }
+  if (g_pred) { tdvc_set_error("tdvc_set_predicate_images: a launch predicate is set (clear it first)"); return TDVC_EINVAL; }
+  g_pred_img = flags; g_pred_img_n = n;
+  return TDVC_OK;
+}
+const int* tdvc_launch_predicate_images(int N) {
+  if (!g_pred_img || N != g_pred_img_n) return nullptr;
+  g_pred_taken = 1;
+  return g_pred_img;
 }
 extern "C" int tdvc_last_launch_predicated(void) { return g_pred_last; }
 const int* tdvc_launch_predicate() {
diff --git a/tdvc_amd/csrc/pointwise.hip b/tdvc_amd/csrc/pointwise.hip
--- a/tdvc_amd/csrc/pointwise.hip
+++ b/tdvc_amd/csrc/pointwise.hip
@@ -482,6 +482,20 @@
   if (i >= words) return;
   *frame_word(cache, i) = *frame_word(cur, i);
 }
+__global__ __launch_bounds__(EW_BLOCK) void frames_compare_kernel(FMap cur, FMap cache, long words, long per_img, unsigned force_mask, int* flags) {
+  const long i = (long)blockIdx.x * blockDim.x + threadIdx.x;
+  if (i >= words) return;
+  const long n = i / per_img;
+  const u32x4 a = *frame_word(cur, i), b = *frame_word(cache, i);
+  const bool forced = i == n * per_img && ((force_mask >> n) & 1u) != 0u;
+  if (forced || ((a[0] ^ b[0]) | (a[1] ^ b[1]) | (a[2] ^ b[2]) | (a[3] ^ b[3])) != 0u) flags[n] = 1;
+}
+__global__ __launch_bounds__(EW_BLOCK) void frames_refresh_kernel(FMap cur, FMap cache, long words, long per_img, const int* flags) {
+  const long i = (long)blockIdx.x * blockDim.x + threadIdx.x;
+  if (i >= words) return;
+  if (flags[i / per_img] == 0) return;
+  *frame_word(cache, i) = *frame_word(cur, i);
+}
 
 __device__ __forceinline__ float block_sum(float v, float* sh) {
   const int tid = threadIdx.x;
@@ -818,6 +832,18 @@
   return tdvc_launch_status("tdvc_frame_changed");
 }
 
+extern "C" int tdvc_frames_changed(const tdvc_fmap* cur, tdvc_fmap* cache, int* flags, unsigned force_mask, void* stream) {
+  TDVC_CHECK(cur && cache && flags && fmap_ok16(*cur) && fmap_ok16(*cache) && same_geom(*cur, *cache) && cur->C == cache->C &&
+             cur->N <= TDVC_MAX_PREDICATE_IMAGES && (reinterpret_cast<uintptr_t>(flags) & 3) == 0,
+             "tdvc_frames_changed: fp16 maps of one geometry, at most %d images, and 4-byte aligned flags", TDVC_MAX_PREDICATE_IMAGES);
+  const hipError_t err = hipMemsetAsync(flags, 0, sizeof(int) * cur->N, ST(stream));
+  if (err != hipSuccess) { tdvc_set_error("tdvc_frames_changed: hipMemsetAsync failed: %s", hipGetErrorString(err)); return (int)err; }
+  const long per_img = (long)cur->H * cur->W * (cur->C / 8), words = per_img * cur->N;
+  hipLaunchKernelGGL(frames_compare_kernel, grid1d(words), dim3(EW_BLOCK), 0, ST(stream), to_dev(*cur), to_dev(*cache), words, per_img, force_mask, flags);
+  hipLaunchKernelGGL(frames_refresh_kernel, grid1d(words), dim3(EW_BLOCK), 0, ST(stream), to_dev(*cur), to_dev(*cache), words, per_img, flags);
+  return tdvc_launch_status("tdvc_frames_changed");
+}
+
 extern "C" int tdvc_patch_match(const float* pin, const float* pref, int N, int hp, int wp, int C, int32_t* idx, void* stream) {
   TDVC_CHECK(pin && pref && idx && N >= 1 && hp >= 1 && wp >= 1 && C >= 1 && C * 9 * 4 <= 60000, "tdvc_patch_match: bad arguments");
   const int nph = (hp + 3) / 3 + 1, npw = (wp + 3) / 3 + 1;
diff --git a/tdvc_amd/model/modules.py b/tdvc_amd/model/modules.py
--- a/tdvc_amd/model/modules.py
+++ b/tdvc_amd/model/modules.py
@@ -5,6 +5,7 @@
 
 from .. import ops
 from ..ops import ACT_LRELU, ACT_NONE, ACT_RELU, FM
+from .ring import SlotRing
 
 
 class PackCache:
@@ -267,6 +268,17 @@
 
 LOOPFILTER_PAIR = True
 LOOPFILTER_BCAST = True
+LOOPFILTER_REUSE = True
+LOOPFILTER_RING = 9
+
+
+class LoopFilterReuse:
+
+    __slots__ = ("key", "ring", "A", "S", "F", "flags", "usable", "log")
+
+    def __init__(self, key, slots):
+        self.key, self.ring, self.usable, self.log = key, SlotRing(slots), None, []
+        self.A = self.S = self.F = self.flags = None
 
 
 class LoopFilter(nn.Module, PackCache):
@@ -287,6 +299,85 @@
                      res=res_buf.as_slices(b, 4, 64) if res_buf is not None else None, **kw)
 
     def run(self, xt: FM, refs8: FM, out: FM) -> FM:
+        if (LOOPFILTER_REUSE and LOOPFILTER_PAIR and LOOPFILTER_BCAST and not self.training and ops.TAPE is None and ops.PROFILE is None
+                and not xt.f32 and not refs8.f32 and xt.H * xt.W >= 8192 and ops.conv_pair_supported(xt.as_slices(0, 4, 64))):
+            r = self._run_reuse(xt, refs8, out)
+            if r is not None:
+                return r
+        return self._run_plain(xt, refs8, out)
+
+    def reuse_state(self) -> LoopFilterReuse | None:
+        return self.__dict__.get("_packed", {}).get("lf_reuse")
+
+    def _run_reuse(self, xt: FM, refs8: FM, out: FM) -> FM | None:
+        B, H, W = xt.N, xt.H, xt.W
+        dev = xt.t.device
+        key = (dev.index, ops._stream().value, B, H, W)
+        cache = self.__dict__.setdefault("_packed", {})
+        st = cache.get("lf_reuse")
+        if st is None or st.key != key or st.ring.slots != LOOPFILTER_RING:
+            st = cache["lf_reuse"] = LoopFilterReuse(key, LOOPFILTER_RING)
+        if st.usable is False:
+            return None
+        try:
+            return self._reuse_call(st, xt, refs8, out)
+        except BaseException:
+            cache.pop("lf_reuse", None)
+            raise
+
+    def _reuse_call(self, st: LoopFilterReuse, xt: FM, refs8: FM, out: FM) -> FM | None:
+        B, H, W = xt.N, xt.H, xt.W
+        dev = xt.t.device
+        lr = dict(act=ACT_LRELU, slope=0.1)
+        R = st.ring.slots
+        if st.A is None:
+            st.A, st.S = FM.empty(B, H, W, 64 * R, device=dev), FM.empty(B, H, W, 64 * R, device=dev)
+            st.F = FM.empty(B * R, H, W, refs8.C, device=dev)
+            st.flags = torch.ones((B, 4), dtype=torch.int32, device=dev)
+            a3, a4, s4 = FM(st.A.t, st.A.off, 3, 64, 64), FM(st.A.t, st.A.off, 4, 64, 64), FM(st.S.t, st.S.off, 4, 64, 64)
+            if not (ops.conv_pair_supported(a3) and ops.conv_pair_supported(a4, s4)):
+                st.usable = False
+                st.A = st.S = st.F = st.flags = None
+                return None
+        p, force = st.ring.begin()
+        win = lambda buf, b, j0, n: FM(buf.t, buf.off + b * buf.sn + 64 * (p + j0), n, 64, 64)
+        l1 = self.layer1
+        p01, pc1 = pk_conv(self, "c01", self.conv01), pk_conv(self, "c1", self.conv1)
+        pp_a = self._pk("pair_c02_c1", lambda: ops.pack_conv_pair(self.conv02.weight, self.conv02.bias,
+                                                                   self.conv1.weight.view(64, 64, 3, 3), self.conv1.bias))
+        pp_b = self._pk("pair_b1_bs", lambda: ops.pack_conv_pair(l1.conv1.weight.view(64, 64, 3, 3), l1.conv1.bias,
+                                                                  l1.spatial_conv3d.weight.view(64, 64, 3, 3), l1.spatial_conv3d.bias))
+        log = []
+        for b in range(B):
+            frames = refs8.batch(4 * b + 1, 3)
+            ops.frames_changed(frames, st.F.batch(b * R + p, 3), st.flags[b, :3], force)
+            with ops.predicate_images(st.flags[b, :3]) as lg:
+                t = ops.conv(frames, p01, **lr)
+                ops.conv_pair(t, pp_a, out=win(st.A, b, 0, 3), act1=ACT_NONE, act2=ACT_LRELU, slope2=0.1, add_input=False)
+            log += lg
+            ops.conv(xt.as_slices(b, 4, 64).batch(3, 1), pc1, out=win(st.A, b, 3, 1), **lr)
+            with ops.predicate_images(st.flags[b, :4]) as lg:
+                ops.conv_pair(win(st.A, b, 0, 4), pp_b, out=win(st.S, b, 0, 4), act1=ACT_LRELU, slope1=0.1, act2=ACT_NONE, add_input=False)
+            log += lg
+        st.log = list(log)
+        if not all(log):
+            st.usable = False
+            st.A = st.S = st.F = st.flags = None
+            return None
+        st.usable = True
+        st.ring.commit()
+        s = FM.empty(B, H, W, 256, device=dev)
+        ops.conv(st.S.ch(64 * p, 192), pk_conv(self, "bt", l1.temporal_conv3d), out=s.ch(0, 64), bcast_T=4, bcast_slope=0.1,
+                 res=st.S.ch(64 * p, 64))
+        o = FM.empty(B, H, W, 256, device=dev)
+        pc3 = pk_conv(self, "b3", l1.conv3)
+        for b in range(B):
+            ops.conv(s.as_slices(b, 4, 64), pc3, out=o.as_slices(b, 4, 64), res=win(st.A, b, 0, 4))
+        sums = []
+        f = ops.conv(o, pk_conv(self, "ff", self.feat_fusion), chan_sum=sums, **lr)
+        return self.attn.run(f, out=out, res=xt.ch(192, 64), sums=sums)
+
+    def _run_plain(self, xt: FM, refs8: FM, out: FM) -> FM:
         B, H, W = xt.N, xt.H, xt.W
         dev = xt.t.device
         lr = dict(act=ACT_LRELU, slope=0.1)
diff --git a/tdvc_amd/model/ring.py b/tdvc_amd/model/ring.py
--- /dev/null
+++ b/tdvc_amd/model/ring.py
@@ -0,0 +1,33 @@
+from __future__ import annotations
+
+WINDOW = 4
+
+
+class SlotRing:
+    __slots__ = ("slots", "p", "valid", "_started")
+
+    def __init__(self, slots: int):
+        if slots < WINDOW:
+            raise ValueError(f"SlotRing: the window needs {WINDOW} slots, got {slots}")
+        self.slots = slots
+        self.p = 0
+        self.valid = [False] * slots
+        self._started = False
+
+    def begin(self) -> tuple[int, int]:
+        if self._started:
+            self.p += 1
+            if self.p > self.slots - WINDOW:
+                self.p = 0
+                self.valid = [False] * self.slots
+        self._started = True
+        mask = 0
+        for j in range(WINDOW - 1):
+            if not self.valid[self.p + j]:
+                mask |= 1 << j
+        return self.p, mask
+
+    def commit(self) -> None:
+        for j in range(WINDOW - 1):
+            self.valid[self.p + j] = True
+        self.valid[self.p + WINDOW - 1] = False
diff --git a/tdvc_amd/ops.py b/tdvc_amd/ops.py
--- a/tdvc_amd/ops.py
+++ b/tdvc_amd/ops.py
@@ -53,6 +53,27 @@
         return False
 
 
+class predicate_images:
+
+    def __init__(self, flags: torch.Tensor):
+        assert flags.dtype == torch.int32 and flags.is_cuda and flags.dim() == 1 and flags.is_contiguous() and 1 <= flags.numel() <= 4
+        self.flags = flags
+
+    def __enter__(self):
+        global _PRED_LOG
+        if _PRED_LOG is not None:
+            raise L.TdvcHipError("ops.predicate_images does not nest")
+        L.check(L.lib().tdvc_set_predicate_images(self.flags.data_ptr(), self.flags.numel()), "set_predicate_images")
+        _PRED_LOG = []
+        return _PRED_LOG
+
+    def __exit__(self, *exc):
+        global _PRED_LOG
+        _PRED_LOG = None
+        L.lib().tdvc_set_predicate_images(None, 0)
+        return False
+
+
 def _log_predicated(kernels=1):
     if _PRED_LOG is not None:
         _PRED_LOG.extend([bool(L.lib().tdvc_last_launch_predicated())] * kernels)
@@ -61,6 +82,12 @@
 def frame_changed(cur: FM, cache: FM, flag: torch.Tensor) -> None:
     dc, dk = cur.desc(), cache.desc()
     L.check(L.lib().tdvc_frame_changed(C.byref(dc), C.byref(dk), flag.data_ptr(), _stream()), "frame_changed")
+
+
+def frames_changed(cur: FM, cache: FM, flags: torch.Tensor, force_mask: int = 0) -> None:
+    assert flags.dtype == torch.int32 and flags.is_cuda and flags.is_contiguous() and flags.numel() >= cur.N
+    dc, dk = cur.desc(), cache.desc()
+    L.check(L.lib().tdvc_frames_changed(C.byref(dc), C.byref(dk), flags.data_ptr(), int(force_mask) & 0xF, _stream()), "frames_changed")
 
 
 def _rec(name, *args):
diff --git a/tdvc_amd/train.py b/tdvc_amd/train.py
--- a/tdvc_amd/train.py
+++ b/tdvc_amd/train.py
@@ -26,6 +26,7 @@
             continue
         pk = m.__dict__.get("_packed", {})
         pk.pop("iframe_reuse", None)
+        pk.pop("lf_reuse", None)
         pcs += [pc for pc in pk.values() if isinstance(pc, ops.PackedConv)]
         for key in [k for k, v in pk.items() if isinstance(v, ops.PackedConvPair)]:
             del pk[key]
```

New measurement: 51.28 frames/s (median of 6 runs). 1.03x the previous value.
